# DmitryUlyanov/deep-image-prior

Hardware: NVIDIA H100
Metric: optimisation iterations/sec (512x512 skip-net denoising, sum over independent images) (higher is better)
Workload: dtype fp32 storage; tf32 tensor-core multiplies with fp32 accumulate in the convs (cuDNN's default fp32 mode)

## Files before the change

### deep-image-prior_b200/csrc/conv_tc.cu

```cuda
#include "conv_tc.cuh"
#include "ptx.cuh"
#include "wgmma.cuh"
#include "kernels.cuh"

namespace dip {

static constexpr int kTileM = 128;
static constexpr int kABytes = kTileM * 128;
static constexpr int kChunkBytes = kTileM * 128;
static constexpr int kNumThreads = 256;
static constexpr int kAccStride = kAccS;

struct SmemCtl {
  uint64_t full[8];
  uint64_t empty[8];
  float bias[160];
};

__host__ __device__ constexpr int round32(int n) { return (n + 31) & ~31; }
__host__ __device__ constexpr int round1024(int n) { return (n + 1023) & ~1023; }

template <int NT>
__device__ __forceinline__ void tc_conv_epilogue(const TcConvParams& p, SmemCtl* ctl, uint8_t* staging,
                                                 float (&acc)[2][NT / 2], int x0, int y0, int opx, int opy, int n_off,
                                                 double& stat_s1, double& stat_s2, bool col_halves = false);
__device__ __forceinline__ void tc_conv_stats_flush(const TcConvParams& p, int n_off, double stat_s1, double stat_s2);

template <bool BF16, int NT>
__device__ __forceinline__ void tc_conv_consumer(const TcConvParams& p, SmemCtl* ctl,
                                                 uint8_t* stage_base, int stage_bytes, uint8_t* staging, int n_iters,
                                                 int tile0, int tile_stride, int num_tiles, int tiles_pp, int n_off) {
  const int lane = threadIdx.x & 31;
  float acc[2][NT / 2];
  int stage = 0;
  uint32_t phase = 0;
  double stat_s1 = 0.0, stat_s2 = 0.0;
  const uint32_t base_lo = desc_lo(smem_u32(stage_base));
  const uint32_t stage_step = static_cast<uint32_t>(stage_bytes) >> 4;
  constexpr uint32_t kBOff = static_cast<uint32_t>(kABytes) >> 4;
  constexpr uint32_t kHalfOff = (64u * 128u) >> 4;
  for (int it = 0; it < n_iters; ++it) {
    const int tile = tile0 + it * tile_stride;
    int tx = tile % p.tiles_x, ty = tile / p.tiles_x;
    int opx = 0, opy = 0;
    int kb_per_tile = p.kh * p.kw * p.kblocks;
    if (p.nphase > 0) {
      if (tile >= num_tiles) break;
      const int t = tile % tiles_pp;
      tx = t % p.tiles_x; ty = t / p.tiles_x;
      const TcConvParams::Phase& q = p.phs[tile / tiles_pp];
      opx = q.opx; opy = q.opy;
      kb_per_tile = q.kh * q.kw * p.kblocks;
    }
    const int x0 = tx * p.bw, y0 = ty * p.bh;
#pragma unroll
    for (int i = 0; i < NT / 2; ++i) { acc[0][i] = 0.f; acc[1][i] = 0.f; }
    int prev = -1;
    for (int kbt = 0; kbt < kb_per_tile; ++kbt) {
      mbar_wait(&ctl->full[stage], phase);
      const uint32_t a_lo = base_lo + stage * stage_step;
      const uint32_t b_lo = a_lo + kBOff;
      wgmma_fence();
#pragma unroll
      for (int k = 0; k < 4; ++k) {
        wgmma_ss<NT, BF16>(acc[0], desc_of(a_lo + 2 * k), desc_of(b_lo + 2 * k));
        wgmma_ss<NT, BF16>(acc[1], desc_of(a_lo + kHalfOff + 2 * k), desc_of(b_lo + 2 * k));
      }
      wgmma_commit();
      if (prev >= 0) {
        wgmma_wait<1>();
        if (lane == 0) mbar_arrive(&ctl->empty[prev]);
      }
      prev = stage;
      if (++stage == p.stages) { stage = 0; phase ^= 1; }
    }
    wgmma_wait<0>();
    if (prev >= 0 && lane == 0) mbar_arrive(&ctl->empty[prev]);
    tc_conv_epilogue<NT>(p, ctl, staging, acc, x0, y0, opx, opy, n_off, stat_s1, stat_s2);
  }
  tc_conv_stats_flush(p, n_off, stat_s1, stat_s2);
}

template <int NT>
__device__ __forceinline__ void tc_conv_epilogue(const TcConvParams& p, SmemCtl* ctl, uint8_t* staging,
                                                 float (&acc)[2][NT / 2], int x0, int y0, int opx, int opy, int n_off,
                                                 double& stat_s1, double& stat_s2, bool col_halves) {
  const int et = threadIdx.x - 128;
  const int w = et >> 5, lane = et & 31;
  const int bw_shift = 31 - __clz(p.bw);
  {
    if (et == 0) tma_store_wait_read0();
    named_bar_sync(1, 128);
#pragma unroll
    for (int h = 0; h < 2; ++h) {
#pragma unroll
      for (int j = 0; j < NT / 8; ++j) {
        const int col = 8 * j + 2 * (lane & 3);
        const int chunk = col >> 5;
        if (chunk < p.n_chunks) {
          const int q = (col & 31) >> 2, e = col & 3;
#pragma unroll
          for (int rr = 0; rr < 2; ++rr) {
            const int r64 = 16 * w + (lane >> 2) + 8 * rr;
            const int row = col_halves ? ((r64 >> 3) << 4) + 8 * h + (r64 & 7) : 64 * h + r64;
            float2 o;
            o.x = acc[h][4 * j + 2 * rr] + ctl->bias[col];
            o.y = acc[h][4 * j + 2 * rr + 1] + ctl->bias[col + 1];
            *reinterpret_cast<float2*>(staging + chunk * kChunkBytes + row * 128 + ((q ^ (row & 7)) << 4) + e * 4) = o;
          }
        }
      }
    }
    fence_proxy_async_smem();
    named_bar_sync(1, 128);
    if (et == 0) {
      if (p.nphase > 0)
        for (int j = 0; j < p.n_chunks; ++j) tma_store_5d(&p.tmD, staging + j * kChunkBytes, n_off + j * 32, opx, x0, opy, y0);
      else
        for (int j = 0; j < p.n_chunks; ++j) tma_store_3d(&p.tmD, staging + j * kChunkBytes, n_off + j * 32, x0, y0);
      tma_store_commit();
    }
    if (p.stats != nullptr && et < p.n_mma) {
      const int c = et;
      const int j = c >> 5, q = (c & 31) >> 2, e = c & 3;
      const uint8_t* cb = staging + j * kChunkBytes + e * 4;
      float a0 = 0.f, a1 = 0.f, b0 = 0.f, b1 = 0.f;
      if (x0 + p.bw <= p.out_w && y0 + p.bh <= p.out_h) {
#pragma unroll 8
        for (int m = 0; m < kTileM; m += 2) {
          const float x = *reinterpret_cast<const float*>(cb + m * 128 + ((q ^ (m & 7)) << 4));
          const float y = *reinterpret_cast<const float*>(cb + (m + 1) * 128 + ((q ^ ((m + 1) & 7)) << 4));
          a0 += x; b0 = fmaf(x, x, b0);
          a1 += y; b1 = fmaf(y, y, b1);
        }
      } else {
        for (int m = 0; m < kTileM; ++m) {
          const int py = m >> bw_shift, px = m & (p.bw - 1);
          if (x0 + px < p.out_w && y0 + py < p.out_h) {
            const float x = *reinterpret_cast<const float*>(cb + m * 128 + ((q ^ (m & 7)) << 4));
            a0 += x; b0 = fmaf(x, x, b0);
          }
        }
      }
      stat_s1 += static_cast<double>(a0 + a1);
      stat_s2 += static_cast<double>(b0 + b1);
    }
  }
}

__device__ __forceinline__ void tc_conv_stats_flush(const TcConvParams& p, int n_off, double stat_s1, double stat_s2) {
  const int et = threadIdx.x - 128;
  if (p.stats != nullptr && et < p.n_mma && n_off + et < p.stats_ld) {
    const int rep = (blockIdx.x % kAccR) * kAccLine;
    atomicAdd(&p.stats[(n_off + et) * kAccStride + rep], stat_s1);
    atomicAdd(&p.stats[(p.stats_ld + n_off + et) * kAccStride + rep], stat_s2);
  }
  if (et == 0) tma_store_wait_all0();
}

template <bool BF16>
__device__ __forceinline__ void tc_conv_body(const TcConvParams& p, uint8_t* smem_raw) {
  constexpr int KE = BF16 ? 64 : 32;
  uint8_t* smem = reinterpret_cast<uint8_t*>((reinterpret_cast<uintptr_t>(smem_raw) + 1023) & ~uintptr_t(1023));
  const int nt = round32(p.n_mma);
  const int b_bytes = p.n_mma * 128;
  const int stage_bytes = kABytes + round1024(nt * 128);
  uint8_t* stage_base = smem;
  uint8_t* staging = stage_base + p.stages * stage_bytes;
  SmemCtl* ctl = reinterpret_cast<SmemCtl*>(staging + p.n_chunks * kChunkBytes);

  const int warp = threadIdx.x >> 5;
  const int lane = threadIdx.x & 31;
  const int tiles_pp = p.tiles_x * p.tiles_y;
  const int num_tiles = p.nphase > 0 ? tiles_pp * p.nphase : tiles_pp;
  const int n_split = p.n_split < 1 ? 1 : p.n_split;
  const int n_part = blockIdx.x % n_split;
  const int n_off = n_part * p.n_mma;
  const int n_total = p.n_mma * n_split;
  const int tile_stride = static_cast<int>(gridDim.x) / n_split;
  const int n_iters = (num_tiles + tile_stride - 1) / tile_stride;
  const int tile0 = blockIdx.x / n_split;

  pdl_trigger();
  if (warp == 0 && lane == 0) {
    tma_prefetch_desc(&p.tmA);
    tma_prefetch_desc(&p.tmB);
    tma_prefetch_desc(&p.tmD);
  }
  if (warp == 1 && lane == 0) {
    for (int i = 0; i < p.stages; ++i) {
      mbar_init(&ctl->full[i], 1);
      mbar_init(&ctl->empty[i], 4);
    }
    fence_mbar_init();
  }
  pdl_wait();
  if (warp == 3) {
    for (int i = lane; i < 160; i += 32)
      ctl->bias[i] = (p.bias != nullptr && i < p.n_mma && (p.n_valid == 0 || n_off + i < p.n_valid)) ? p.bias[n_off + i] : 0.f;
  }
  __syncthreads();

  if (warp == 0) {
    int stage = 0;
    uint32_t phase = 0;
    for (int it = 0; it < n_iters; ++it) {
      const int tile = tile0 + it * tile_stride;
      int kh = p.kh, kw = p.kw, offx = p.offx, offy = p.offy, tap0 = 0;
      int x0 = (tile % p.tiles_x) * p.bw, y0 = (tile / p.tiles_x) * p.bh;
      if (p.nphase > 0) {
        if (tile >= num_tiles) break;
        const TcConvParams::Phase& q = p.phs[tile / tiles_pp];
        const int t = tile % tiles_pp;
        kh = q.kh; kw = q.kw; offx = q.offx; offy = q.offy; tap0 = q.tap0;
        x0 = (t % p.tiles_x) * p.bw; y0 = (t / p.tiles_x) * p.bh;
      }
      for (int r = 0; r < kh; ++r) {
        for (int s = 0; s < kw; ++s) {
          const int ix = offx + s, iy = offy + r;
          int cpx, cx, cpy, cy;
          if (p.stride == 1) {
            cpx = 0; cx = x0 + ix; cpy = 0; cy = y0 + iy;
          } else {
            cpx = ix & 1; cx = x0 + (ix >> 1); cpy = iy & 1; cy = y0 + (iy >> 1);
          }
          const int tap = tap0 + r * kw + s;
          for (int kb = 0; kb < p.kblocks; ++kb) {
            mbar_wait(&ctl->empty[stage], phase ^ 1);
            uint8_t* sa = stage_base + stage * stage_bytes;
            if (elect_one()) {
              mbar_expect_tx(&ctl->full[stage], kABytes + b_bytes);
              tma_load_5d(sa, &p.tmA, &ctl->full[stage], kb * KE, cpx, cx, cpy, cy);
              tma_load_2d(sa + kABytes, &p.tmB, &ctl->full[stage], kb * KE, tap * n_total + n_off);
            }
            __syncwarp();
            if (++stage == p.stages) { stage = 0; phase ^= 1; }
          }
        }
      }
    }
  } else if (warp >= 4) {
    switch (nt) {
      case 32: tc_conv_consumer<BF16, 32>(p, ctl, stage_base, stage_bytes, staging, n_iters, tile0, tile_stride, num_tiles, tiles_pp, n_off); break;
      case 64: tc_conv_consumer<BF16, 64>(p, ctl, stage_base, stage_bytes, staging, n_iters, tile0, tile_stride, num_tiles, tiles_pp, n_off); break;
      case 96: tc_conv_consumer<BF16, 96>(p, ctl, stage_base, stage_bytes, staging, n_iters, tile0, tile_stride, num_tiles, tiles_pp, n_off); break;
      case 128: tc_conv_consumer<BF16, 128>(p, ctl, stage_base, stage_bytes, staging, n_iters, tile0, tile_stride, num_tiles, tiles_pp, n_off); break;
      default: tc_conv_consumer<BF16, 160>(p, ctl, stage_base, stage_bytes, staging, n_iters, tile0, tile_stride, num_tiles, tiles_pp, n_off); break;
    }
  }
  __syncthreads();
}
__global__ void __launch_bounds__(kNumThreads, 1) tc_conv_kernel(const __grid_constant__ TcConvParams p) {
  extern __shared__ __align__(1024) uint8_t smem_raw[];
  tc_conv_body<false>(p, smem_raw);
}
__global__ void __launch_bounds__(kNumThreads, 1) tc_conv_kernel_bf16(const __grid_constant__ TcConvParams p) {
  extern __shared__ __align__(1024) uint8_t smem_raw[];
  tc_conv_body<true>(p, smem_raw);
}

__host__ __device__ constexpr int patch_nt(int n_mma) { return n_mma == 144 ? 144 : round32(n_mma); }
struct PatchCtl {
  uint64_t pfull[kPatchMaxKb];
  uint64_t pempty[kPatchMaxKb];
};

struct PatchWork {
  int tile0, tile_stride, n_iters, n_off, n_total;
};
__device__ __forceinline__ PatchWork patch_work(const TcConvParams& p) {
  const int n_split = p.n_split < 1 ? 1 : p.n_split;
  PatchWork w;
  const int num_tiles = p.tiles_x * p.tiles_y;
  w.tile_stride = static_cast<int>(gridDim.x) / n_split;
  w.tile0 = blockIdx.x / n_split;
  w.n_iters = (num_tiles - w.tile0 + w.tile_stride - 1) / w.tile_stride;
  w.n_off = static_cast<int>(blockIdx.x % n_split) * p.n_mma;
  w.n_total = p.n_mma * n_split;
  return w;
}
static constexpr int kPatchTaps = 9;

template <bool BF16, int NT>
__device__ __forceinline__ void tc_conv_patch_consumer(const TcConvParams& p, SmemCtl* ctl, PatchCtl* pc,
                                                       uint8_t* patch_base, uint8_t* b_base, int b_stage_bytes,
                                                       uint8_t* staging, const PatchWork& wk) {
  const int lane = threadIdx.x & 31;
  float acc[2][NT / 2];
  int stage = 0;
  uint32_t phase = 0, pphase = 0;
  double stat_s1 = 0.0, stat_s2 = 0.0;
  const uint32_t patch16 = smem_u32(patch_base) >> 4;
  const uint32_t b_lo0 = desc_lo(smem_u32(b_base));
  const uint32_t b_step = static_cast<uint32_t>(b_stage_bytes) >> 4;
  constexpr uint32_t kPlane16 = kPatchPlane >> 4, kSlot16 = kPatchBytes >> 4;
  const uint32_t row16 = p.bw + 2;
  const uint32_t half16 = p.bw == 8 ? 8 * row16 : 8;
  for (int it = 0; it < wk.n_iters; ++it) {
    const int tile = wk.tile0 + it * wk.tile_stride;
    const int x0 = (tile % p.tiles_x) * p.bw, y0 = (tile / p.tiles_x) * p.bh;
#pragma unroll
    for (int i = 0; i < NT / 2; ++i) { acc[0][i] = 0.f; acc[1][i] = 0.f; }
    int prev = -1;
    int prev_patch = -1;
#pragma unroll 1
    for (int tap = 0; tap < kPatchTaps; ++tap) {
      const int r = tap / 3, s = tap - 3 * (tap / 3);
#pragma unroll 1
      for (int kb = 0; kb < p.kblocks; ++kb) {
        if (tap == 0) mbar_wait(&pc->pfull[kb], pphase);
        mbar_wait(&ctl->full[stage], phase);
        const uint32_t b_lo = b_lo0 + stage * b_step;
        const uint32_t a16 = patch16 + kb * kSlot16 + r * row16 + s;
        wgmma_fence();
#pragma unroll
        for (int k = 0; k < 4; ++k) {
          wgmma_ss<NT, BF16>(acc[0], desc_noswz(a16 + 2 * k * kPlane16, kPlane16, row16), desc_of(b_lo + 2 * k));
          wgmma_ss<NT, BF16>(acc[1], desc_noswz(a16 + half16 + 2 * k * kPlane16, kPlane16, row16), desc_of(b_lo + 2 * k));
        }
        wgmma_commit();
        if (prev >= 0) {
          wgmma_wait<1>();
          if (lane == 0) {
            mbar_arrive(&ctl->empty[prev]);
            if (prev_patch >= 0) mbar_arrive(&pc->pempty[prev_patch]);
          }
        }
        prev = stage;
        prev_patch = tap == kPatchTaps - 1 ? kb : -1;
        if (++stage == p.stages) { stage = 0; phase ^= 1; }
      }
    }
    pphase ^= 1;
    wgmma_wait<0>();
    if (prev >= 0 && lane == 0) {
      mbar_arrive(&ctl->empty[prev]);
      if (prev_patch >= 0) mbar_arrive(&pc->pempty[prev_patch]);
    }
    tc_conv_epilogue<NT>(p, ctl, staging, acc, x0, y0, 0, 0, wk.n_off, stat_s1, stat_s2, p.bw == 16);
  }
  tc_conv_stats_flush(p, wk.n_off, stat_s1, stat_s2);
}

template <bool BF16>
__device__ __forceinline__ void tc_conv_patch_body(const TcConvParams& p, uint8_t* smem_raw) {
  constexpr int KE = BF16 ? 64 : 32;
  constexpr int KG = BF16 ? 8 : 4;
  uint8_t* smem = reinterpret_cast<uint8_t*>((reinterpret_cast<uintptr_t>(smem_raw) + 1023) & ~uintptr_t(1023));
  const int nt = patch_nt(p.n_mma);
  const int b_bytes = p.n_mma * 128;
  const int b_stage_bytes = round1024(nt * 128);
  uint8_t* b_base = smem;
  uint8_t* staging = b_base + p.stages * b_stage_bytes;
  uint8_t* patch_base = staging + p.n_chunks * kChunkBytes;
  SmemCtl* ctl = reinterpret_cast<SmemCtl*>(patch_base + p.kblocks * kPatchBytes);
  PatchCtl* pc = reinterpret_cast<PatchCtl*>(ctl + 1);

  const int warp = threadIdx.x >> 5;
  const int lane = threadIdx.x & 31;
  const PatchWork wk = patch_work(p);

  pdl_trigger();
  if (warp == 0 && lane == 0) {
    tma_prefetch_desc(&p.tmA);
    tma_prefetch_desc(&p.tmB);
    tma_prefetch_desc(&p.tmD);
  }
  if (warp == 1 && lane == 0) {
    for (int i = 0; i < p.stages; ++i) {
      mbar_init(&ctl->full[i], 1);
      mbar_init(&ctl->empty[i], 4);
    }
    for (int i = 0; i < p.kblocks; ++i) {
      mbar_init(&pc->pfull[i], 1);
      mbar_init(&pc->pempty[i], 4);
    }
    fence_mbar_init();
  }
  pdl_wait();
  if (warp == 3) {
    for (int i = lane; i < 160; i += 32)
      ctl->bias[i] = (p.bias != nullptr && i < p.n_mma && (p.n_valid == 0 || wk.n_off + i < p.n_valid)) ? p.bias[wk.n_off + i] : 0.f;
  }
  __syncthreads();

  if (warp == 0) {
    int stage = 0;
    uint32_t phase = 0, pphase = 0;
    for (int it = 0; it < wk.n_iters; ++it) {
      const int tile = wk.tile0 + it * wk.tile_stride;
      const int x0 = (tile % p.tiles_x) * p.bw, y0 = (tile / p.tiles_x) * p.bh;
      for (int tap = 0; tap < kPatchTaps; ++tap) {
        for (int kb = 0; kb < p.kblocks; ++kb) {
          if (tap == 0) {
            mbar_wait(&pc->pempty[kb], pphase ^ 1);
            if (elect_one()) {
              mbar_expect_tx(&pc->pfull[kb], kPatchBytes);
              tma_load_4d(patch_base + kb * kPatchBytes, &p.tmA, &pc->pfull[kb], 0, x0 + p.offx, y0 + p.offy, kb * (KE / KG));
            }
            __syncwarp();
          }
          mbar_wait(&ctl->empty[stage], phase ^ 1);
          if (elect_one()) {
            mbar_expect_tx(&ctl->full[stage], b_bytes);
            tma_load_2d(b_base + stage * b_stage_bytes, &p.tmB, &ctl->full[stage], kb * KE, tap * wk.n_total + wk.n_off);
          }
          __syncwarp();
          if (++stage == p.stages) { stage = 0; phase ^= 1; }
        }
      }
      pphase ^= 1;
    }
  } else if (warp >= 4) {
    switch (nt) {
      case 32: tc_conv_patch_consumer<BF16, 32>(p, ctl, pc, patch_base, b_base, b_stage_bytes, staging, wk); break;
      case 64: tc_conv_patch_consumer<BF16, 64>(p, ctl, pc, patch_base, b_base, b_stage_bytes, staging, wk); break;
      case 96: tc_conv_patch_consumer<BF16, 96>(p, ctl, pc, patch_base, b_base, b_stage_bytes, staging, wk); break;
      case 128: tc_conv_patch_consumer<BF16, 128>(p, ctl, pc, patch_base, b_base, b_stage_bytes, staging, wk); break;
      case 144: tc_conv_patch_consumer<BF16, 144>(p, ctl, pc, patch_base, b_base, b_stage_bytes, staging, wk); break;
      default: tc_conv_patch_consumer<BF16, 160>(p, ctl, pc, patch_base, b_base, b_stage_bytes, staging, wk); break;
    }
  }
  __syncthreads();
}
__global__ void __launch_bounds__(kNumThreads, 1) tc_conv_patch_kernel(const __grid_constant__ TcConvParams p) {
  extern __shared__ __align__(1024) uint8_t smem_raw[];
  tc_conv_patch_body<false>(p, smem_raw);
}
__global__ void __launch_bounds__(kNumThreads, 1) tc_conv_patch_kernel_bf16(const __grid_constant__ TcConvParams p) {
  extern __shared__ __align__(1024) uint8_t smem_raw[];
  tc_conv_patch_body<true>(p, smem_raw);
}

struct SmemCtlW {
  uint64_t full[8];
  uint64_t empty[8];
  uint64_t bt_full[2];
  uint64_t bt_empty[2];
};

__host__ __device__ constexpr int wgrad_tbuf_bytes(bool bf16, int n_cols) {
  return (bf16 ? kTileM * 128 : 0) + round1024(n_cols * 128);
}


template <int NT>
__device__ __forceinline__ void tc_wgrad_transposer(const TcWgradParams& p, SmemCtlW* ctl, uint32_t stage_base, int stage_bytes,
                                                    uint32_t bt_base, int items) {
  constexpr int kBt = wgrad_tbuf_bytes(false, NT);
  constexpr int kUnitsO = ((NT + 31) / 32) * 8;
  constexpr int kIters = (kUnitsO + 11) / 12;
  constexpr int y_bytes = 4 * kWgradKp * 128;
  const int tt = threadIdx.x - 32;
  const int lane = threadIdx.x & 31;
  const int b = tt & 7, b0 = b & 1, b1 = (b >> 1) & 1, b2 = b >> 2;
  uint32_t src[kIters], dst[kIters], sq[kIters], dq[kIters];
  bool ok[kIters];
#pragma unroll
  for (int it = 0; it < kIters; ++it) {
    const int o = (tt >> 3) + 12 * it;
    const int kk = (b1 ^ (o & 1)) | ((b2 ^ ((o >> 1) & 1)) << 1);
    const int c4 = (o >> 3) * 8 + b2 * 4 + b1 * 2 + ((o >> 2) & 1);
    ok[it] = o < kUnitsO && c4 < NT / 4;
    src[it] = y_bytes + (c4 >> 3) * (kWgradKp * 128) + (8 * kk + b0) * 128;
    sq[it] = (c4 & 7) ^ b0;
    dst[it] = c4 * 4 * 128;
    dq[it] = (2 * kk + b0) ^ ((c4 & 1) << 2);
  }
  int stage = 0, tb = 0;
  uint32_t phase = 0, tphase = 0;
  for (int item = blockIdx.x; item < items; item += gridDim.x) {
    const int ks = item % p.ksplits;
    const int blk0 = static_cast<int>((static_cast<long long>(p.px_blocks) * ks) / p.ksplits);
    const int blk1 = static_cast<int>((static_cast<long long>(p.px_blocks) * (ks + 1)) / p.ksplits);
    for (int blk = blk0; blk < blk1; ++blk) {
      mbar_wait(&ctl->full[stage], phase);
      mbar_wait(&ctl->bt_empty[tb], tphase ^ 1);
      const uint32_t sx = stage_base + stage * stage_bytes;
      const uint32_t bt = bt_base + tb * kBt;
#pragma unroll
      for (int it = 0; it < kIters; ++it) {
        if (ok[it]) {
          uint4 v[4];
#pragma unroll
          for (int i = 0; i < 4; ++i) v[i] = lds128(sx + src[it] + 256 * i + ((sq[it] ^ (2 * i)) << 4));
          sts128(bt + dst[it] + ((dq[it] ^ 0) << 4), v[0].x, v[1].x, v[2].x, v[3].x);
          sts128(bt + dst[it] + 128 + ((dq[it] ^ 1) << 4), v[0].y, v[1].y, v[2].y, v[3].y);
          sts128(bt + dst[it] + 256 + ((dq[it] ^ 2) << 4), v[0].z, v[1].z, v[2].z, v[3].z);
          sts128(bt + dst[it] + 384 + ((dq[it] ^ 3) << 4), v[0].w, v[1].w, v[2].w, v[3].w);
        }
      }
      fence_proxy_async_smem();
      mbar_arrive(&ctl->bt_full[tb]);
      __syncwarp();
      if (lane == 0) mbar_arrive(&ctl->empty[stage]);
      if (++stage == p.stages) { stage = 0; phase ^= 1; }
      tb ^= 1;
      if (tb == 0) tphase ^= 1;
    }
  }
}

template <int NT>
__device__ __forceinline__ void tc_wgrad_mma(const TcWgradParams& p, SmemCtlW* ctl, uint32_t stage_base, int stage_bytes,
                                             uint32_t bt_base, int items) {
  constexpr int kBt = wgrad_tbuf_bytes(false, NT);
  constexpr bool kDouble = NT <= 136;
  const int et = threadIdx.x - 128;
  const int w = et >> 5, lane = et & 31, g = lane >> 2, t = lane & 3;
  const int taps = p.kh * p.kw;
  uint32_t aoff[4];
#pragma unroll
  for (int r = 0; r < 4; ++r) {
    const int hi = r & 1, e = r >> 1;
    const int q = 4 * (w & 1) + (g >> 2) + 2 * hi, px = 2 * t + e;
    aoff[r] = (w >> 1) * (kWgradKp * 128) + px * 128 + ((q ^ px) << 4) + (g & 3) * 4;
  }
  auto load_a = [&](uint32_t (&f)[8][4], uint32_t sy) {
#pragma unroll
    for (int h = 0; h < 2; ++h)
#pragma unroll
      for (int kk = 0; kk < 4; ++kk)
#pragma unroll
        for (int r = 0; r < 4; ++r) f[4 * h + kk][r] = lds32(sy + aoff[r] + h * 2 * (kWgradKp * 128) + kk * 1024);
  };
  int stage = 0, tb = 0;
  uint32_t phase = 0, tphase = 0;
  bool pending = false;
  float acc[2][NT / 2];
  uint32_t fa[8][4], fb[8][4];
  auto step = [&](uint32_t (&cur)[8][4], uint32_t (&nxt)[8][4], bool more) {
    mbar_wait(&ctl->bt_full[tb], tphase);
    const uint32_t b_lo = desc_lo(bt_base + tb * kBt);
    wgmma_fence();
#pragma unroll
    for (int kk = 0; kk < 4; ++kk) {
      wgmma_rs<NT>(acc[0], cur[kk], desc_of(b_lo + 2 * kk));
      wgmma_rs<NT>(acc[1], cur[4 + kk], desc_of(b_lo + 2 * kk));
    }
    wgmma_commit();
    __syncwarp();
    if (lane == 0) mbar_arrive(&ctl->empty[stage]);
    if (++stage == p.stages) { stage = 0; phase ^= 1; }
    if constexpr (kDouble) wgmma_wait<1>(); else wgmma_wait<0>();
    if (pending && lane == 0) mbar_arrive(&ctl->bt_empty[tb ^ 1]);
    pending = true;
    tb ^= 1;
    if (tb == 0) tphase ^= 1;
    if (more) {
      mbar_wait(&ctl->full[stage], phase);
      load_a(nxt, stage_base + stage * stage_bytes);
    }
  };
  for (int item = blockIdx.x; item < items; item += gridDim.x) {
    const int tap = item / p.ksplits, ks = item % p.ksplits;
    const int blk0 = static_cast<int>((static_cast<long long>(p.px_blocks) * ks) / p.ksplits);
    const int blk1 = static_cast<int>((static_cast<long long>(p.px_blocks) * (ks + 1)) / p.ksplits);
#pragma unroll
    for (int i = 0; i < NT / 2; ++i) { acc[0][i] = 0.f; acc[1][i] = 0.f; }
    if (blk0 < blk1) {
      mbar_wait(&ctl->full[stage], phase);
      load_a(fa, stage_base + stage * stage_bytes);
    }
    for (int blk = blk0; blk < blk1; blk += 2) {
      step(fa, kDouble ? fb : fa, blk + 1 < blk1);
      if (blk + 1 == blk1) break;
      step(kDouble ? fb : fa, fa, blk + 2 < blk1);
    }
    wgmma_wait<0>();
    if (pending && lane == 0) mbar_arrive(&ctl->bt_empty[tb ^ 1]);
    pending = false;
    float* dst = p.partial + (static_cast<size_t>(ks) * taps + tap) * 128 * NT;
#pragma unroll
    for (int h = 0; h < 2; ++h) {
#pragma unroll
      for (int j = 0; j < NT / 8; ++j) {
        const int col = 8 * j + 2 * t;
#pragma unroll
        for (int rr = 0; rr < 2; ++rr) {
          const int n = 64 * h + 16 * w + g + 8 * rr;
          *reinterpret_cast<float2*>(dst + static_cast<size_t>(n) * NT + col) =
              make_float2(acc[h][4 * j + 2 * rr], acc[h][4 * j + 2 * rr + 1]);
        }
      }
    }
  }
}

template <int NT>
__device__ __forceinline__ void tc_wgrad_consumer_bf16(const TcWgradParams& p, SmemCtlW* ctl, uint8_t* smem, int stage_bytes,
                                                       uint8_t* tbase, int items) {
  constexpr int KE = 64;
  constexpr int E = 2;
  constexpr int kTA = kTileM * 128;
  constexpr int kTBuf = wgrad_tbuf_bytes(true, NT);
  constexpr int kRows = 128 + NT;
  const int et = threadIdx.x - 128;
  const int w = et >> 5, lane = et & 31;
  constexpr int chunk_bytes = kWgradKp * 128;
  constexpr int y_bytes = (128 / KE) * chunk_bytes;
  constexpr int groups = kWgradKp * E / 16;
  constexpr int nk = kWgradKp / 16;
  const int taps = p.kh * p.kw;
  int stage = 0, tb = 0;
  uint32_t phase = 0;
  float acc[2][NT / 2];
  for (int item = blockIdx.x; item < items; item += gridDim.x) {
    const int tap = item / p.ksplits, ks = item % p.ksplits;
    const int blk0 = static_cast<int>((static_cast<long long>(p.px_blocks) * ks) / p.ksplits);
    const int blk1 = static_cast<int>((static_cast<long long>(p.px_blocks) * (ks + 1)) / p.ksplits);
#pragma unroll
    for (int i = 0; i < NT / 2; ++i) { acc[0][i] = 0.f; acc[1][i] = 0.f; }
    for (int blk = blk0; blk < blk1; ++blk) {
      mbar_wait(&ctl->full[stage], phase);
      named_bar_sync(1, 128);
      const uint8_t* sy = smem + stage * stage_bytes;
      const uint8_t* sx = sy + y_bytes;
      uint8_t* ta = tbase + tb * kTBuf;
      uint8_t* tbb = ta + kTA;
      for (int i = et; i < kRows * groups; i += 128) {
        const int g = i / kRows, row = i % kRows;
        const bool is_y = row < 128;
        const int rs = is_y ? row : row - 128;
        const uint8_t* src = (is_y ? sy : sx) + (rs / KE) * chunk_bytes;
        const int cb = (rs % KE) * E;
        uint32_t v[4];
#pragma unroll
        for (int u = 0; u < 4; ++u) {
          const int px = g * 8 + 2 * u;
          const uint32_t lo = *reinterpret_cast<const uint16_t*>(src + px * 128 + ((((cb >> 4) ^ (px & 7)) << 4) | (cb & 15)));
          const uint32_t hi = *reinterpret_cast<const uint16_t*>(src + (px + 1) * 128 + ((((cb >> 4) ^ ((px + 1) & 7)) << 4) | (cb & 15)));
          v[u] = lo | (hi << 16);
        }
        uint8_t* dst = (is_y ? ta : tbb) + rs * 128 + ((g ^ (rs & 7)) << 4);
        *reinterpret_cast<uint4*>(dst) = make_uint4(v[0], v[1], v[2], v[3]);
      }
      fence_proxy_async_smem();
      named_bar_sync(1, 128);
      if (lane == 0) mbar_arrive(&ctl->empty[stage]);
      const uint32_t a_lo = desc_lo(smem_u32(ta)), b_lo = desc_lo(smem_u32(tbb));
      wgmma_fence();
#pragma unroll
      for (int k = 0; k < nk; ++k) {
        wgmma_ss<NT, true>(acc[0], desc_of(a_lo + 2 * k), desc_of(b_lo + 2 * k));
        wgmma_ss<NT, true>(acc[1], desc_of(a_lo + ((64u * 128u) >> 4) + 2 * k), desc_of(b_lo + 2 * k));
      }
      wgmma_commit();
      wgmma_wait<1>();
      tb ^= 1;
      if (++stage == p.stages) { stage = 0; phase ^= 1; }
    }
    wgmma_wait<0>();
    float* dst = p.partial + (static_cast<size_t>(ks) * taps + tap) * 128 * NT;
#pragma unroll
    for (int h = 0; h < 2; ++h) {
#pragma unroll
      for (int j = 0; j < NT / 8; ++j) {
        const int col = 8 * j + 2 * (lane & 3);
#pragma unroll
        for (int rr = 0; rr < 2; ++rr) {
          const int n = 64 * h + 16 * w + (lane >> 2) + 8 * rr;
          *reinterpret_cast<float2*>(dst + static_cast<size_t>(n) * NT + col) =
              make_float2(acc[h][4 * j + 2 * rr], acc[h][4 * j + 2 * rr + 1]);
        }
      }
    }
  }
}

template <bool BF16, int NT>
__device__ __forceinline__ void tc_wgrad_role(const TcWgradParams& p, SmemCtlW* ctl, uint8_t* smem, int stage_bytes,
                                              uint8_t* tbase, int items, int warp) {
  if constexpr (BF16) {
    if (warp >= 4) tc_wgrad_consumer_bf16<NT>(p, ctl, smem, stage_bytes, tbase, items);
  } else {
    if (warp >= 4) tc_wgrad_mma<NT>(p, ctl, smem_u32(smem), stage_bytes, smem_u32(tbase), items);
    else tc_wgrad_transposer<NT>(p, ctl, smem_u32(smem), stage_bytes, smem_u32(tbase), items);
  }
}

template <bool BF16>
__device__ __forceinline__ void tc_wgrad_body(const TcWgradParams& p, uint8_t* smem_raw) {
  uint8_t* smem = reinterpret_cast<uint8_t*>((reinterpret_cast<uintptr_t>(smem_raw) + 1023) & ~uintptr_t(1023));
  constexpr int KE = BF16 ? 64 : 32;
  constexpr int YCH = 128 / KE;
  constexpr int chunk_bytes = kWgradKp * 128;
  const int y_bytes = YCH * chunk_bytes;
  const int x_bytes = p.c_chunks * chunk_bytes;
  const int stage_bytes = y_bytes + x_bytes;
  uint8_t* tbase = smem + p.stages * stage_bytes;
  SmemCtlW* ctl = reinterpret_cast<SmemCtlW*>(tbase + 2 * wgrad_tbuf_bytes(BF16, p.n_cols));
  const int items = p.kh * p.kw * p.ksplits;

  const int warp = threadIdx.x >> 5;
  const int lane = threadIdx.x & 31;
  pdl_trigger();
  if (warp == 0 && lane == 0) {
    tma_prefetch_desc(&p.tmY);
    tma_prefetch_desc(&p.tmX);
  }
  if (warp == 1 && lane == 0) {
    for (int i = 0; i < p.stages; ++i) {
      mbar_init(&ctl->full[i], 1);
      mbar_init(&ctl->empty[i], BF16 ? 4 : 7);
    }
    for (int i = 0; i < 2; ++i) {
      mbar_init(&ctl->bt_full[i], 96);
      mbar_init(&ctl->bt_empty[i], 4);
    }
    fence_mbar_init();
  }
  pdl_wait();
  __syncthreads();

  if (warp == 0) {
    int stage = 0;
    uint32_t phase = 0;
    for (int item = blockIdx.x; item < items; item += gridDim.x) {
      const int tap = item / p.ksplits, ks = item % p.ksplits;
      const int r = tap / p.kw, s = tap % p.kw;
      const int blk0 = static_cast<int>((static_cast<long long>(p.px_blocks) * ks) / p.ksplits);
      const int blk1 = static_cast<int>((static_cast<long long>(p.px_blocks) * (ks + 1)) / p.ksplits);
      const int ix = p.offx + s, iy = p.offy + r;
      for (int blk = blk0; blk < blk1; ++blk) {
        const int y = blk / p.px_blocks_x;
        const int x0 = (blk % p.px_blocks_x) * kWgradKp;
        int cpx, cx, cpy, cy;
        if (p.stride == 1) {
          cpx = 0; cx = x0 + ix; cpy = 0; cy = y + iy;
        } else {
          cpx = ix & 1; cx = x0 + (ix >> 1); cpy = iy & 1; cy = y + (iy >> 1);
        }
        mbar_wait(&ctl->empty[stage], phase ^ 1);
        uint8_t* sy = smem + stage * stage_bytes;
        if (elect_one()) {
          mbar_expect_tx(&ctl->full[stage], stage_bytes);
          for (int j = 0; j < YCH; ++j) tma_load_3d(sy + j * chunk_bytes, &p.tmY, &ctl->full[stage], j * KE, x0, y);
          for (int j = 0; j < p.c_chunks; ++j)
            tma_load_5d(sy + y_bytes + j * chunk_bytes, &p.tmX, &ctl->full[stage], j * KE, cpx, cx, cpy, cy);
        }
        __syncwarp();
        if (++stage == p.stages) { stage = 0; phase ^= 1; }
      }
    }
  } else {
    switch (p.n_cols) {
      case 32: tc_wgrad_role<BF16, 32>(p, ctl, smem, stage_bytes, tbase, items, warp); break;
      case 64: tc_wgrad_role<BF16, 64>(p, ctl, smem, stage_bytes, tbase, items, warp); break;
      case 96: tc_wgrad_role<BF16, 96>(p, ctl, smem, stage_bytes, tbase, items, warp); break;
      case 128: tc_wgrad_role<BF16, 128>(p, ctl, smem, stage_bytes, tbase, items, warp); break;
      case 136: tc_wgrad_role<BF16, 136>(p, ctl, smem, stage_bytes, tbase, items, warp); break;
      default: tc_wgrad_role<BF16, 160>(p, ctl, smem, stage_bytes, tbase, items, warp); break;
    }
  }
  __syncthreads();
}
__global__ void __launch_bounds__(kNumThreads, 1) tc_wgrad_kernel(const __grid_constant__ TcWgradParams p) {
  extern __shared__ __align__(1024) uint8_t smem_raw[];
  tc_wgrad_body<false>(p, smem_raw);
}
__global__ void __launch_bounds__(kNumThreads, 1) tc_wgrad_kernel_bf16(const __grid_constant__ TcWgradParams p) {
  extern __shared__ __align__(1024) uint8_t smem_raw[];
  tc_wgrad_body<true>(p, smem_raw);
}

static constexpr size_t kMaxSmem = 232448;

size_t tc_conv_smem_bytes(const TcConvParams& p) {
  const size_t b_bytes = round1024((p.patch ? patch_nt(p.n_mma) : round32(p.n_mma)) * 128);
  if (p.patch)
    return 1024 + p.stages * b_bytes + static_cast<size_t>(p.n_chunks) * kChunkBytes +
           static_cast<size_t>(p.kblocks) * kPatchBytes + sizeof(SmemCtl) + sizeof(PatchCtl);
  return 1024 + p.stages * (kABytes + b_bytes) + static_cast<size_t>(p.n_chunks) * kChunkBytes + sizeof(SmemCtl);
}
size_t tc_wgrad_smem_bytes(const TcWgradParams& p) {
  const size_t chunk = static_cast<size_t>(kWgradKp) * 128;
  const size_t tbuf = wgrad_tbuf_bytes(p.bf16 != 0, p.n_cols);
  return 1024 + p.stages * ((p.bf16 ? 2 : 4) * chunk + static_cast<size_t>(p.c_chunks) * chunk) + 2 * tbuf + sizeof(SmemCtlW);
}

cudaError_t tc_kernels_init() {
  cudaError_t e = cudaFuncSetAttribute(tc_conv_kernel, cudaFuncAttributeMaxDynamicSharedMemorySize, (int)kMaxSmem);
  if (e != cudaSuccess) return e;
  e = cudaFuncSetAttribute(tc_conv_kernel_bf16, cudaFuncAttributeMaxDynamicSharedMemorySize, (int)kMaxSmem);
  if (e != cudaSuccess) return e;
  e = cudaFuncSetAttribute(tc_conv_patch_kernel, cudaFuncAttributeMaxDynamicSharedMemorySize, (int)kMaxSmem);
  if (e != cudaSuccess) return e;
  e = cudaFuncSetAttribute(tc_conv_patch_kernel_bf16, cudaFuncAttributeMaxDynamicSharedMemorySize, (int)kMaxSmem);
  if (e != cudaSuccess) return e;
  e = cudaFuncSetAttribute(tc_wgrad_kernel_bf16, cudaFuncAttributeMaxDynamicSharedMemorySize, (int)kMaxSmem);
  if (e != cudaSuccess) return e;
  return cudaFuncSetAttribute(tc_wgrad_kernel, cudaFuncAttributeMaxDynamicSharedMemorySize, (int)kMaxSmem);
}

static bool conv_params_ok(const TcConvParams& p) {
  return p.n_mma >= 1 && p.n_mma <= 160 && p.n_chunks == (p.n_mma + 31) / 32 && p.stages >= 1 && p.stages <= 8 &&
         p.kblocks >= 1 && p.nphase >= 0 && p.nphase <= 4 &&
         (p.bw & (p.bw - 1)) == 0 && p.bw * p.bh == kTileM &&
         (!p.patch || (((p.bw == 8 && p.bh == 16) || (p.bw == 16 && p.bh == 8)) && p.kblocks <= kPatchMaxKb && p.kh == 3 && p.kw == 3 && p.stride == 1 && p.nphase == 0));
}

cudaError_t tc_conv_launch(const TcConvParams& p, int num_sms, cudaStream_t s) {
  if (!conv_params_ok(p)) return cudaErrorInvalidValue;
  const int tiles = p.tiles_x * p.tiles_y * (p.nphase > 0 ? p.nphase : 1);
  int grid = tiles < num_sms ? tiles : num_sms;
  if (p.n_split > 1) {
    if (tiles * p.n_split > num_sms) return cudaErrorInvalidValue;
    grid = tiles * p.n_split;
  }
  const size_t smem = tc_conv_smem_bytes(p);
  if (smem > kMaxSmem) return cudaErrorInvalidValue;
  if (p.patch)
    return launch_k(p.bf16 ? tc_conv_patch_kernel_bf16 : tc_conv_patch_kernel, dim3(grid), dim3(kNumThreads), smem, s, 1, p);
  return launch_k(p.bf16 ? tc_conv_kernel_bf16 : tc_conv_kernel, dim3(grid), dim3(kNumThreads), smem, s, 1, p);
}

cudaError_t tc_wgrad_launch(const TcWgradParams& p, cudaStream_t s) {
  const size_t smem = tc_wgrad_smem_bytes(p);
  const bool cols_ok = p.n_cols == 32 || p.n_cols == 64 || p.n_cols == 96 || p.n_cols == 128 || p.n_cols == 136 ||
                       p.n_cols == 160;
  if (smem > kMaxSmem || !cols_ok || p.n_cols > p.c_chunks * (p.bf16 ? 64 : 32) || p.stages < 1 || p.stages > 8)
    return cudaErrorInvalidValue;
  return launch_k(p.bf16 ? tc_wgrad_kernel_bf16 : tc_wgrad_kernel, dim3(p.kh * p.kw * p.ksplits), dim3(kNumThreads), smem, s, 1, p);
}

}
```

### deep-image-prior_b200/csrc/conv_tc.cuh

```cuda
#pragma once
#include <cuda.h>
#include <cuda_runtime.h>
#include <stdint.h>

namespace dip {

struct TcConvParams {
  CUtensorMap tmA;
  CUtensorMap tmB;
  CUtensorMap tmD;
  int tiles_x, tiles_y;
  int bw, bh;
  int out_w, out_h;
  int kh, kw;
  int stride;
  int offx, offy;
  int bf16;
  int kblocks;
  int n_mma;
  int n_chunks;
  int stages;
  int n_split;
  int nphase;
  struct Phase { int kh, kw, offx, offy, tap0, opx, opy; } phs[4];
  int n_valid;
  const float* bias;
  double* stats;
  int stats_ld;
  int patch;
};
static constexpr int kPatchPlane = 180 * 16;
static constexpr int kPatchMaxKb = 8;
static constexpr int kPatchBytes = 8 * kPatchPlane;

static constexpr int kWgradKp = 32;
struct TcWgradParams {
  CUtensorMap tmY;
  CUtensorMap tmX;
  float* partial;
  int kh, kw, stride, offx, offy;
  int px_blocks_x;
  int px_blocks;
  int bf16;
  int c_chunks;
  int n_cols;
  int ksplits;
  int stages;
};

size_t tc_conv_smem_bytes(const TcConvParams& p);
size_t tc_wgrad_smem_bytes(const TcWgradParams& p);
cudaError_t tc_conv_launch(const TcConvParams& p, int num_sms, cudaStream_t s);
cudaError_t tc_wgrad_launch(const TcWgradParams& p, cudaStream_t s);
cudaError_t tc_kernels_init();

}
```

### deep-image-prior_b200/csrc/engine.cu

```cuda
#include <cuda.h>
#include <cuda_bf16.h>
#include <cuda_runtime.h>
#include <math.h>
#include <stdio.h>
#include <stdlib.h>
#include <string.h>

#include <initializer_list>
#include <map>
#include <string>
#include <vector>

#include "../../include/dip.h"
#include "conv_tc.cuh"
#include "kernels.cuh"

namespace dip {

static thread_local std::string g_err;
static int fail(const std::string& m) {
  g_err = m;
  return -1;
}
#define DIP_CUDA(expr)                                                                                   \
  do {                                                                                                   \
    cudaError_t _e = (expr);                                                                             \
    if (_e != cudaSuccess) return fail(std::string(#expr) + ": " + cudaGetErrorString(_e));              \
  } while (0)
#define DIP_CHECK(expr)        \
  do {                         \
    int _r = (expr);           \
    if (_r != 0) return _r;    \
  } while (0)

typedef CUresult (*PFN_encodeTiled)(CUtensorMap*, CUtensorMapDataType, cuuint32_t, void*, const cuuint64_t*,
                                    const cuuint64_t*, const cuuint32_t*, const cuuint32_t*, CUtensorMapInterleave,
                                    CUtensorMapSwizzle, CUtensorMapL2promotion, CUtensorMapFloatOOBfill);
static PFN_encodeTiled g_encode = nullptr;
static int g_num_sms = 0;
static unsigned long long g_inited_mask = 0;

static int engine_init() {
  int dev = 0;
  DIP_CUDA(cudaGetDevice(&dev));
  if (dev >= 64) return fail("dip: device ordinal >= 64 not supported");
  if (g_inited_mask & (1ull << dev)) return 0;
  cudaDeviceProp prop;
  DIP_CUDA(cudaGetDeviceProperties(&prop, dev));
  if (prop.major != 9 || prop.minor != 0)
    return fail("dip requires an sm_90 (H100) device; found sm_" + std::to_string(prop.major * 10 + prop.minor));
  g_num_sms = prop.multiProcessorCount;
  void* fn = nullptr;
  cudaDriverEntryPointQueryResult q;
  DIP_CUDA(cudaGetDriverEntryPoint("cuTensorMapEncodeTiled", &fn, cudaEnableDefault, &q));
  if (fn == nullptr || q != cudaDriverEntryPointSuccess) return fail("cuTensorMapEncodeTiled not available from the driver");
  g_encode = reinterpret_cast<PFN_encodeTiled>(fn);
  DIP_CUDA(tc_kernels_init());
  DIP_CUDA(down_kernels_init());
  g_inited_mask |= 1ull << dev;
  return 0;
}

static bool is_tc(int prec) { return prec == DIP_PRECISION_TF32 || prec == DIP_PRECISION_BF16; }

static int encode_map(CUtensorMap* m, const void* base, int rank, const cuuint64_t* dims, const cuuint64_t* strides_b,
                      const cuuint32_t* box, bool bf16 = false, bool swizzle = true) {
  cuuint32_t estr[5] = {1, 1, 1, 1, 1};
  CUresult r = g_encode(m, bf16 ? CU_TENSOR_MAP_DATA_TYPE_BFLOAT16 : CU_TENSOR_MAP_DATA_TYPE_FLOAT32, rank, const_cast<void*>(base), dims, strides_b, box, estr,
                        CU_TENSOR_MAP_INTERLEAVE_NONE, swizzle ? CU_TENSOR_MAP_SWIZZLE_128B : CU_TENSOR_MAP_SWIZZLE_NONE,
                        CU_TENSOR_MAP_L2_PROMOTION_L2_128B,
                        CU_TENSOR_MAP_FLOAT_OOB_FILL_NONE);
  if (r != CUDA_SUCCESS) {
    char buf[256];
    snprintf(buf, sizeof buf, "cuTensorMapEncodeTiled failed (%d): rank %d dims %llu %llu %llu box %u %u %u", (int)r, rank,
             (unsigned long long)dims[0], (unsigned long long)dims[1], (unsigned long long)(rank > 2 ? dims[2] : 0), box[0],
             box[1], rank > 2 ? box[2] : 0);
    return fail(buf);
  }
  return 0;
}
static int map_act5(CUtensorMap* m, const void* base, int rows, int cols, int ld, int c, int stride, int bw, int bh,
                    bool bf16 = false) {
  const cuuint64_t e = bf16 ? 2 : sizeof(float);
  cuuint64_t dims[5], str[4];
  if (stride == 1) {
    dims[0] = c; dims[1] = 1; dims[2] = cols; dims[3] = 1; dims[4] = rows;
    str[0] = ld * e; str[1] = ld * e; str[2] = (cuuint64_t)cols * ld * e; str[3] = (cuuint64_t)cols * ld * e;
  } else {
    dims[0] = c; dims[1] = 2; dims[2] = cols / 2; dims[3] = 2; dims[4] = rows / 2;
    str[0] = ld * e; str[1] = 2 * ld * e; str[2] = (cuuint64_t)cols * ld * e; str[3] = 2 * (cuuint64_t)cols * ld * e;
  }
  cuuint32_t box[5] = {bf16 ? 64u : 32u, 1, (cuuint32_t)bw, 1, (cuuint32_t)bh};
  return encode_map(m, base, 5, dims, str, box, bf16);
}
static int map_act3(CUtensorMap* m, const void* base, int rows, int cols, int ld, int c, int bw, int bh, bool bf16 = false) {
  const cuuint64_t e = bf16 ? 2 : sizeof(float);
  cuuint64_t dims[3] = {(cuuint64_t)c, (cuuint64_t)cols, (cuuint64_t)rows};
  cuuint64_t str[2] = {ld * e, (cuuint64_t)cols * ld * e};
  cuuint32_t box[3] = {bf16 ? 64u : 32u, (cuuint32_t)bw, (cuuint32_t)bh};
  return encode_map(m, base, 3, dims, str, box, bf16);
}
static int map_patch(CUtensorMap* m, const void* base, int rows, int cols, int ld, int c, int bw, int bh, bool bf16) {
  const cuuint64_t e = bf16 ? 2 : sizeof(float);
  const cuuint64_t g = 16 / e;
  cuuint64_t dims[4] = {g, (cuuint64_t)cols, (cuuint64_t)rows, (cuuint64_t)c / g};
  cuuint64_t str[3] = {ld * e, (cuuint64_t)cols * ld * e, 16};
  cuuint32_t box[4] = {(cuuint32_t)g, (cuuint32_t)bw + 2, (cuuint32_t)bh + 2, 8};
  return encode_map(m, base, 4, dims, str, box, bf16, false);
}
static int map_w2(CUtensorMap* m, const void* base, int rows_total, int kcols, int box_rows, bool bf16 = false) {
  const cuuint64_t e = bf16 ? 2 : sizeof(float);
  cuuint64_t dims[2] = {(cuuint64_t)kcols, (cuuint64_t)rows_total};
  cuuint64_t str[1] = {kcols * e};
  cuuint32_t box[2] = {bf16 ? 64u : 32u, (cuuint32_t)box_rows};
  return encode_map(m, base, 2, dims, str, box, bf16);
}

static void pick_tile(int w, int h, int* bw, int* bh) {
  const int cand[5][2] = {{128, 1}, {64, 2}, {32, 4}, {16, 8}, {8, 16}};
  long long best = -1;
  for (int i = 0; i < 5; ++i) {
    const long long cw = (w + cand[i][0] - 1) / cand[i][0] * cand[i][0];
    const long long ch = (h + cand[i][1] - 1) / cand[i][1] * cand[i][1];
    const long long cost = cw * ch * 64 + (cand[i][0] + cand[i][1]);
    if (best < 0 || cost < best) { best = cost; *bw = cand[i][0]; *bh = cand[i][1]; }
  }
}
static int round_up(int x, int m) { return (x + m - 1) / m * m; }
struct Timer {
  bool on = false;
  std::vector<cudaEvent_t> pool;
  size_t used = 0;
  struct Rec { int cls; double flops; size_t e0, e1; };
  std::vector<Rec> recs;
  size_t get(cudaStream_t s) {
    if (used == pool.size()) { cudaEvent_t e; cudaEventCreate(&e); pool.push_back(e); }
    cudaEventRecord(pool[used], s);
    return used++;
  }
  void reset() { used = 0; recs.clear(); }
};
struct Recorder {
  Timer* timer = nullptr;
  int n = 0;
};
enum HbmId { H_INPUT_PAD = 0, H_NOISE, H_SKINNY_FWD, H_BN_ACT_WRITE, H_BN_ACT_HEAD, H_CAT_STATS, H_CAT_WRITE, H_BN_BWD_REDUCE,
             H_BN_BWD_APPLY, H_CAT_BWD_REDUCE, H_CAT_BWD_APPLY, H_UPADJ, H_SKINNY_BWD, H_MSE, H_ADAM, H_HEAD_DLOGIT, H_DOWN_FWD,
             H_DOWN_BWD, H_PACK, H_WGRAD_REDUCE, H_TRACK_OUT, H_TRACK_DECIDE, H_ADAM_TRACK };
static constexpr int kUntimed = -1;
static int hbm(HbmId id, int sub) { return 16 + 8 * (int)id + sub; }
struct EnqScope {
  Timer* t; int cls; double flops; size_t e0 = 0; cudaStream_t s;
  EnqScope(Recorder* r, int cls_, double flops_, cudaStream_t s_)
      : t(r != nullptr && cls_ != kUntimed && r->timer->on ? r->timer : nullptr), cls(cls_), flops(flops_), s(s_) {
    if (r != nullptr) r->n++;
    if (t) e0 = t->get(s);
  }
  ~EnqScope() { if (t) { size_t e1 = t->get(s); t->recs.push_back({cls, flops, e0, e1}); } }
};
#define ENQ(rec, cls, flops, s, stmt)                                 \
  do {                                                                \
    EnqScope _es((rec), (cls), (double)(flops), (s));                 \
    stmt;                                                             \
  } while (0)

struct PackEntry {
  const float* w; float* dst_f; float* dst_d;
  int N, C, k, rot, n_rows, c_pad, c_rows;
  int Ctot, coff;
  int s2;
  int bf16;
  int c_pad16;
  int n_pad;
};
__constant__ int kS2Taps[9] = {2 * 3 + 2, 2 * 3 + 0, 0 * 3 + 2, 0 * 3 + 0,
                               2 * 3 + 1, 0 * 3 + 1,
                               1 * 3 + 2, 1 * 3 + 0,
                               1 * 3 + 1};
__global__ void k_pack_table(const PackEntry* __restrict__ tab) {
  pdl_enter();
  const PackEntry e = tab[blockIdx.y];
  const int taps = e.k * e.k;
  const int c_pad = e.bf16 ? e.c_pad16 : e.c_pad;
  __nv_bfloat16* const f16 = reinterpret_cast<__nv_bfloat16*>(e.dst_f);
  __nv_bfloat16* const d16 = reinterpret_cast<__nv_bfloat16*>(e.dst_d);
  const long long nf = e.dst_f != nullptr ? (long long)taps * e.n_rows * c_pad : 0;
  const long long nd = e.dst_d != nullptr ? (long long)taps * e.c_rows * e.n_pad : 0;
  for (long long i = (long long)blockIdx.x * blockDim.x + threadIdx.x; i < nf + nd; i += (long long)gridDim.x * blockDim.x) {
    if (i < nf) {
      const int c = (int)(i % c_pad), n = (int)((i / c_pad) % e.n_rows), tap = (int)(i / ((long long)c_pad * e.n_rows));
      float v = 0.f;
      if (n < e.N && c < e.C) v = e.w[((long long)n * e.Ctot + (c + e.coff + e.rot) % e.Ctot) * taps + tap];
      if (e.bf16) f16[i] = __float2bfloat16_rn(v); else e.dst_f[i] = v;
    } else {
      const long long j = i - nf;
      const int n = (int)(j % e.n_pad), c = (int)((j / e.n_pad) % e.c_rows), tapf = (int)(j / ((long long)e.n_pad * e.c_rows));
      const int tap = e.s2 ? kS2Taps[tapf] : taps - 1 - tapf;
      float v = 0.f;
      if (n < e.N && c < e.C) v = e.w[((long long)n * e.Ctot + (c + e.coff + e.rot) % e.Ctot) * taps + tap];
      if (e.bf16) d16[j] = __float2bfloat16_rn(v); else e.dst_d[j] = v;
    }
  }
}
struct UnpackEntry {
  const float* acc; float* dw;
  int N, C, taps, rot, cols, Ctot, coff, ks;
};
__global__ void k_wgrad_unpack_table(const UnpackEntry* __restrict__ tab) {
  pdl_enter();
  const UnpackEntry e = tab[blockIdx.y];
  const int total = e.N * e.C * e.taps;
  for (int i = blockIdx.x * blockDim.x + threadIdx.x; i < total; i += gridDim.x * blockDim.x) {
    const int tap = i % e.taps, c = (i / e.taps) % e.C, n = i / (e.taps * e.C);
    const size_t split = (size_t)e.taps * 128 * e.cols;
    const float* src = e.acc + ((size_t)tap * 128 + n) * e.cols + c;
    float v = 0.f;
    for (int k = 0; k < e.ks; ++k) v += src[k * split];
    e.dw[((size_t)n * e.Ctot + (c + e.coff + e.rot) % e.Ctot) * e.taps + tap] = v;
  }
}
static int pick_nsplit(int tiles, int n_rows) {
  int sp = 1;
  while (sp * 2 <= 4 && tiles * sp * 2 <= g_num_sms && n_rows % (32 * sp * 2) == 0) sp *= 2;
  return sp;
}
static void fit_stages(TcConvParams& p) {
  p.stages = p.patch ? 8 : 6;
  while (tc_conv_smem_bytes(p) > 232448 && p.stages > 2) p.stages--;
}
struct ConvOp {
  Recorder* rec = nullptr;
  double alg_flops() const { return 2.0 * out_h * out_w * (double)N * C * k * k; }
  int N = 128, C = 0, k = 1, stride = 1, rot = 0;
  int Np = 128;
  int n_pad = 128;
  int n_pad16 = 128;
  int Ctot = 0, coff = 0;
  bool do_fprop = true, do_wgrad = true;
  int dg_ld = 0;
  int c_pad = 0;
  int crows = 0;
  bool bf16 = false;
  int c_pad16 = 0;
  const uint16_t* in16 = nullptr; int in_ld16 = 0;
  const uint16_t* dy16 = nullptr;
  const float* in = nullptr; int in_rows = 0, in_cols = 0, in_ld = 0; int offx = 0, offy = 0;
  float* out = nullptr; int out_h = 0, out_w = 0;
  double* stats = nullptr;
  float* wp_f = nullptr; float* wp_d = nullptr;
  const float* dy = nullptr;
  bool has_dgrad = false;
  bool dg_s2 = false;
  float* dg_out = nullptr; int dg_out_h = 0, dg_out_w = 0; int dg_off = 0;
  float* partial = nullptr;
  const UnpackEntry* unpack = nullptr;
  int p_w = -1, p_b = -1;
  TcConvParams fp{}, dg{};
  TcWgradParams wg{};

  void set_shapes() {
    c_pad = round_up(C, 32);
    c_pad16 = round_up(C, 64);
    crows = round_up(C, 16);
    Np = round_up(N, 16); n_pad = round_up(N, 32); n_pad16 = round_up(N, 64);
    if (Ctot == 0) Ctot = C;
    if (dg_ld == 0) dg_ld = C;
  }
  size_t wp_f_elems() const { return (size_t)k * k * Np * c_pad; }
  size_t wp_d_elems() const { return (size_t)k * k * crows * n_pad; }
  int wg_cols() const { return C > 128 && C <= 136 ? 136 : c_pad; }
  int tc_ksplits() const {
    const int blocks = out_h * ((out_w + kWgradKp - 1) / kWgradKp);
    int ks = static_cast<int>(kNumSms) / (k * k);
    if (ks > blocks) ks = blocks;
    return ks < 1 ? 1 : ks;
  }
  int simt_ksplits() const { return out_h < 64 ? out_h : 64; }
  int part_ks(int prec) const { return is_tc(prec) ? tc_ksplits() : simt_ksplits(); }
  int part_cols(int prec) const { return is_tc(prec) ? wg_cols() : c_pad; }
  size_t partial_elems(int prec) const { return (size_t)part_ks(prec) * k * k * 128 * part_cols(prec); }
  PackEntry pack_entry(int prec, const float* w) const {
    PackEntry e{};
    e.w = w; e.dst_f = do_fprop ? wp_f : nullptr; e.dst_d = has_dgrad ? wp_d : nullptr;
    e.N = N; e.C = C; e.k = k; e.rot = rot; e.n_rows = Np; e.c_pad = c_pad; e.c_rows = crows;
    e.Ctot = Ctot; e.coff = coff; e.s2 = dg_s2 && is_tc(prec) ? 1 : 0;
    e.bf16 = bf16 ? 1 : 0; e.c_pad16 = c_pad16; e.n_pad = bf16 ? n_pad16 : n_pad;
    return e;
  }
  UnpackEntry unpack_entry(int prec, float* dw) const {
    return UnpackEntry{partial, dw, N, C, k * k, rot, part_cols(prec), Ctot, coff, part_ks(prec)};
  }

  int patch_form(TcConvParams& g, const void* act, int rows, int cols, int ld, int kc) {
    if ((g.bw != 8 && g.bw != 16) || kc % (bf16 ? 8 : 4) != 0 || g.kblocks > kPatchMaxKb) return 0;
    TcConvParams t = g;
    t.patch = 1;
    fit_stages(t);
    if (tc_conv_smem_bytes(t) > 232448) return 0;
    DIP_CHECK(map_patch(&t.tmA, act, rows, cols, ld, kc, g.bw, g.bh, bf16));
    g = t;
    return 0;
  }
  int build_tc() {
    int bw, bh;
    fp = TcConvParams{};
    if (do_fprop) {
      pick_tile(out_w, out_h, &bw, &bh);
      DIP_CHECK(bf16 ? map_act5(&fp.tmA, in16, in_rows, in_cols, in_ld16, C, stride, bw, bh, true)
                     : map_act5(&fp.tmA, in, in_rows, in_cols, in_ld, C, stride, bw, bh));
      fp.n_split = pick_nsplit(((out_w + bw - 1) / bw) * ((out_h + bh - 1) / bh), Np);
      DIP_CHECK(map_w2(&fp.tmB, wp_f, k * k * Np, bf16 ? c_pad16 : c_pad, Np / fp.n_split, bf16));
      DIP_CHECK(map_act3(&fp.tmD, out, out_h, out_w, N, N, bw, bh));
      fp.tiles_x = (out_w + bw - 1) / bw; fp.tiles_y = (out_h + bh - 1) / bh;
      fp.bw = bw; fp.bh = bh; fp.out_w = out_w; fp.out_h = out_h;
      fp.kh = fp.kw = k; fp.stride = stride; fp.offx = offx; fp.offy = offy;
      fp.bf16 = bf16 ? 1 : 0;
      fp.kblocks = bf16 ? c_pad16 / 64 : c_pad / 32;
      fp.n_mma = Np / fp.n_split; fp.n_chunks = (fp.n_mma + 31) / 32;
      fp.n_valid = N;
      fp.bias = nullptr; fp.stats = stats; fp.stats_ld = N;
      fit_stages(fp);
      if (k == 3 && stride == 1)
        DIP_CHECK(bf16 ? patch_form(fp, in16, in_rows, in_cols, in_ld16, C) : patch_form(fp, in, in_rows, in_cols, in_ld, C));
    }
    dg = TcConvParams{};
    if (has_dgrad) {
      const int gh = dg_s2 ? dg_out_h / 2 : dg_out_h, gw = dg_s2 ? dg_out_w / 2 : dg_out_w;
      pick_tile(gw, gh, &bw, &bh);
      DIP_CHECK(bf16 ? map_act5(&dg.tmA, dy16, out_h, out_w, N, N, 1, bw, bh, true)
                     : map_act5(&dg.tmA, dy, out_h, out_w, N, N, 1, bw, bh));
      dg.tiles_x = (gw + bw - 1) / bw; dg.tiles_y = (gh + bh - 1) / bh;
      dg.n_split = pick_nsplit((dg_s2 ? 4 : 1) * dg.tiles_x * dg.tiles_y, crows);
      DIP_CHECK(map_w2(&dg.tmB, wp_d, k * k * crows, bf16 ? n_pad16 : n_pad, crows / dg.n_split, bf16));
      DIP_CHECK(dg_s2 ? map_act5(&dg.tmD, dg_out, dg_out_h, dg_out_w, dg_ld, C, 2, bw, bh)
                      : map_act3(&dg.tmD, dg_out, dg_out_h, dg_out_w, dg_ld, C, bw, bh));
      dg.bw = bw; dg.bh = bh; dg.out_w = gw; dg.out_h = gh;
      dg.stride = 1;
      if (dg_s2) {
        dg.kh = dg.kw = 2; dg.offx = dg.offy = -1;
        dg.nphase = 4;
        int t0 = 0;
        for (int a = 0; a < 2; ++a)
          for (int b = 0; b < 2; ++b) {
            TcConvParams::Phase& q = dg.phs[a * 2 + b];
            q.kh = 2 - a; q.kw = 2 - b; q.offy = a == 0 ? -1 : 0; q.offx = b == 0 ? -1 : 0; q.tap0 = t0; q.opx = b; q.opy = a;
            t0 += q.kh * q.kw;
          }
      } else {
        dg.kh = dg.kw = k; dg.offx = dg.offy = dg_off;
      }
      dg.bf16 = bf16 ? 1 : 0;
      dg.kblocks = bf16 ? n_pad16 / 64 : n_pad / 32;
      dg.n_mma = crows / dg.n_split; dg.n_chunks = (dg.n_mma + 31) / 32;
      fit_stages(dg);
      if (!dg_s2 && k == 3)
        DIP_CHECK(bf16 ? patch_form(dg, dy16, out_h, out_w, N, N) : patch_form(dg, dy, out_h, out_w, N, N));
    }
    wg = TcWgradParams{};
    if (!do_wgrad) return 0;
    wg.bf16 = bf16 ? 1 : 0;
    DIP_CHECK(bf16 ? map_act3(&wg.tmY, dy16, out_h, out_w, N, N, kWgradKp, 1, true)
                   : map_act3(&wg.tmY, dy, out_h, out_w, N, N, kWgradKp, 1));
    DIP_CHECK(bf16 ? map_act5(&wg.tmX, in16, in_rows, in_cols, in_ld16, C, stride, kWgradKp, 1, true)
                   : map_act5(&wg.tmX, in, in_rows, in_cols, in_ld, C, stride, kWgradKp, 1));
    wg.partial = partial;
    wg.kh = wg.kw = k; wg.stride = stride; wg.offx = offx; wg.offy = offy;
    wg.px_blocks_x = (out_w + kWgradKp - 1) / kWgradKp;
    wg.px_blocks = out_h * wg.px_blocks_x;
    wg.c_chunks = bf16 ? c_pad16 / 64 : c_pad / 32;
    wg.n_cols = wg_cols();
    wg.ksplits = tc_ksplits();
    wg.stages = 6;
    while (tc_wgrad_smem_bytes(wg) > 232448 && wg.stages > 1) wg.stages--;
    if (tc_wgrad_smem_bytes(wg) > 232448) return fail("wgrad stage does not fit in shared memory");
    return 0;
  }

  int run_fprop(int prec, const float* bias, cudaStream_t s) {
    if (is_tc(prec)) {
      TcConvParams p = fp;
      p.bias = bias;
      ENQ(rec, 0, alg_flops(), s, DIP_CUDA(tc_conv_launch(p, g_num_sms, s)));
    } else {
      SimtConvArgs a{};
      a.A = in; a.a_h = in_rows; a.a_w = in_cols; a.a_ld = in_ld; a.a_c = C;
      a.Wp = wp_f; a.n_rows = Np; a.c_pad = c_pad;
      a.D = out; a.d_h = out_h; a.d_w = out_w; a.d_ld = N; a.d_c = N;
      a.kh = a.kw = k; a.stride = stride; a.offx = offx; a.offy = offy; a.bias = bias;
      ENQ(rec, kUntimed, 0, s, launch_simt_conv(a, s));
      if (stats != nullptr) ENQ(rec, kUntimed, 0, s, launch_channel_stats(out, N, N, out_h * out_w, stats, s));
      DIP_CUDA(cudaGetLastError());
    }
    return 0;
  }
  int run_dgrad(int prec, cudaStream_t s) {
    if (is_tc(prec)) {
      ENQ(rec, 1, alg_flops(), s, DIP_CUDA(tc_conv_launch(dg, g_num_sms, s)));
    } else {
      SimtConvArgs a{};
      a.A = dy; a.a_h = out_h; a.a_w = out_w; a.a_ld = N; a.a_c = N; a.dil = dg_s2 ? 2 : 1;
      a.Wp = wp_d; a.n_rows = crows; a.c_pad = n_pad;
      a.D = dg_out; a.d_h = dg_out_h; a.d_w = dg_out_w; a.d_ld = dg_ld; a.d_c = C;
      a.kh = a.kw = k; a.stride = 1; a.offx = a.offy = dg_off; a.bias = nullptr;
      ENQ(rec, kUntimed, 0, s, launch_simt_conv(a, s));
      DIP_CUDA(cudaGetLastError());
    }
    return 0;
  }
  int run_wgrad(int prec, cudaStream_t s) {
    static const bool dbg_skip = getenv("DIP_DBG_SKIP_WGRAD") != nullptr;
    if (dbg_skip) return 0;
    if (is_tc(prec)) {
      ENQ(rec, 2, alg_flops(), s, DIP_CUDA(tc_wgrad_launch(wg, s)));
    } else {
      SimtWgradArgs a{};
      a.dY = dy; a.h = out_h; a.w = out_w; a.dy_ld = N; a.n = N;
      a.X = in; a.x_h = in_rows; a.x_w = in_cols; a.x_ld = in_ld; a.x_c = C;
      a.kh = a.kw = k; a.stride = stride; a.offx = offx; a.offy = offy;
      a.partial = partial; a.c_pad = c_pad; a.ksplits = simt_ksplits();
      ENQ(rec, kUntimed, 0, s, launch_simt_wgrad(a, s));
    }
    if (unpack != nullptr)
      ENQ(rec, hbm(H_WGRAD_REDUCE, 0), ((double)part_ks(prec) + 1.0) * k * k * 128.0 * part_cols(prec) * sizeof(float), s,
          launch_k(k_wgrad_unpack_table, dim3(64, 1), dim3(256), 0, s, 1, unpack));
    DIP_CUDA(cudaGetLastError());
    return 0;
  }
};

struct CvtEntry {
  const double* src; float* dst; int n, rot;
  int row, row_ld;
};
__global__ void k_cvt_table(const CvtEntry* __restrict__ tab) {
  pdl_enter();
  const CvtEntry e = tab[blockIdx.x];
  for (int i = threadIdx.x; i < e.n; i += blockDim.x) {
    const int si = e.row > 0 ? (i / e.row) * e.row_ld + i % e.row : i;
    e.dst[(i + e.rot) % e.n] = (float)acc_get(e.src + (size_t)si * kAccS);
  }
}
struct RunEntry {
  const double* fwd; float* rm; float* rv; void* nb; int C, rot; float n; int nb_is_float;
};
__global__ void k_running_table(const RunEntry* __restrict__ tab) {
  pdl_enter();
  const RunEntry e = tab[blockIdx.x];
  if (e.rm == nullptr) return;
  for (int c = threadIdx.x; c < e.C; c += blockDim.x) {
    const int ct = (c + e.rot) % e.C;
    const double m = acc_get(e.fwd + c * kAccS) / e.n;
    double var = acc_get(e.fwd + (e.C + c) * kAccS) / e.n - m * m;
    if (var < 0) var = 0;
    const double unb = e.n > 1.f ? var * e.n / (e.n - 1.0) : var;
    e.rm[ct] = 0.9f * e.rm[ct] + 0.1f * (float)m;
    e.rv[ct] = 0.9f * e.rv[ct] + 0.1f * (float)unb;
  }
  if (threadIdx.x == 0 && e.nb != nullptr) {
    if (e.nb_is_float) *reinterpret_cast<float*>(e.nb) += 1.f; else *reinterpret_cast<long long*>(e.nb) += 1;
  }
}

struct Arena {
  uint8_t* base;
  size_t off = 0;
  template <typename T>
  T* get(size_t n) {
    off = (off + 255) & ~size_t(255);
    T* p = base ? reinterpret_cast<T*>(base + off) : nullptr;
    off += n * sizeof(T);
    return p;
  }
};
struct BufInfo {
  void* ptr; int rows, cols, ld, c;
};
struct BnLayer {
  int C = 0, rot = 0; float n = 1.f;
  double* fwd = nullptr; double* bwd = nullptr; double* dbias = nullptr;
  int p_gamma = -1, p_beta = -1, p_bias = -1, idx = -1;
};
struct Level {
  int H, W, h, w, Cin;
  int Cin_act;
  int bilinear;
  int nd = 128, nu = 128, ns = 0, cu = 128;
  float *rawF = nullptr, *dRawF = nullptr;
  uint16_t* dRawF16 = nullptr;
  float *Pin, *raw_s, *raw_d1, *P_d1, *raw_d2, *P_d2, *P_cat, *raw_u, *A_u, *raw_v, *U;
  uint16_t *Pin16 = nullptr, *P_d1_16 = nullptr, *P_d2_16 = nullptr, *P_cat16 = nullptr, *A_u16 = nullptr;
  uint16_t *dRaw_v16 = nullptr, *dRaw_u16 = nullptr, *dRaw_d2_16 = nullptr, *dRaw_d1_16 = nullptr, *dRaw_s16 = nullptr;
  int Pin_ld16 = 0, cat_ld16 = 0;
  float *dUp;
  float *dS;
  float *dRaw_v, *dA_u, *dRaw_u, *dP_cat, *dCat, *dRaw_s, *dRaw_d2, *dP_d1, *dRaw_d1, *dPin;
  BnLayer bn_s, bn_d1, bn_d2, bn_cat, bn_u, bn_v;
  int p_skip_w, p_skip_b;
  double* dw_s;
  ConvOp d1, d2, up, c11;
  ConvOp sk, up_a, up_b;
};

}

using namespace dip;

struct dip_plan {
  dip_net_desc desc;
  int H, W;
  int zero_pad = 0;
  int act_fun = DIP_ACT_LEAKY_RELU;
  bool dry = false;
  uint8_t* ws = nullptr;
  size_t ws_bytes = 0;
  std::vector<Level> lv;
  std::vector<long long> numel;
  std::vector<float*> params, grads;
  std::vector<void*> running;
  std::vector<BnLayer*> bns;
  std::vector<ConvOp*> convs;
  std::map<std::string, BufInfo> bufs;
  int p_head_w = -1, p_head_b = -1;
  double* dw_head = nullptr; double* db_head = nullptr; double* db_scratch = nullptr;
  float* out_saved = nullptr;
  double* acc_fwd = nullptr; size_t acc_fwd_n = 0;
  double* acc_bwd = nullptr; size_t acc_bwd_n = 0;
  float* partial = nullptr;
  float* zbuf = nullptr; float* dout = nullptr; float* dl4 = nullptr;
  static constexpr int kDownMaxK = 64;
  float* ds_kern = nullptr;
  float* ds_y = nullptr;
  float* ds_dy = nullptr;
  int ds_K = 0, ds_f = 1, ds_pad = 0, ds_Ho = 0, ds_Wo = 0;
  static constexpr int kLossRing = 65536;
  double* loss_ring = nullptr;
  int* it_dev = nullptr;
  struct GraphKey {
    const void *z0 = nullptr, *target = nullptr, *mask = nullptr, *out = nullptr, *slots = nullptr;
    unsigned long long adam_id = 0, adam_bind = 0;
    float sigma = 0.f; uint64_t seed = 0; double lr = 0.0;
    dip_track track{};
    bool operator==(const GraphKey& o) const {
      const dip_track &a = track, &b = o.track;
      return z0 == o.z0 && target == o.target && mask == o.mask && out == o.out && slots == o.slots && adam_id == o.adam_id &&
             adam_bind == o.adam_bind && sigma == o.sigma && seed == o.seed && lr == o.lr && a.gt == b.gt &&
             a.out_avg == b.out_avg && a.snapshot == b.snapshot && a.state == b.state && a.records == b.records &&
             a.exp_weight == b.exp_weight && a.show_every == b.show_every && a.backtrack_db == b.backtrack_db;
    }
  };
  GraphKey gkey{};
  cudaGraphExec_t gexec = nullptr;
  cudaGraphExec_t gfwd = nullptr, gbwd = nullptr;
  cudaStream_t gstream = nullptr;
  cudaEvent_t gev_in = nullptr, gev_out = nullptr;
  cudaStream_t wstream = nullptr;
  cudaStream_t sstream = nullptr;
  std::vector<cudaEvent_t> wev;
  size_t wev_used = 0;
  bool side_on = false;
  std::vector<dip::ConvOp*> deferred;
  struct { bool on = false; const float* z0 = nullptr; float sigma = 0.f; uint64_t seed = 0, offset = 0; const int* it_dev = nullptr; } fnoise;
  bool prepacked = false;
  PackEntry* d_pack = nullptr; CvtEntry* d_cvt = nullptr; RunEntry* d_run = nullptr; UnpackEntry* d_unpack = nullptr;
  int n_pack = 0, n_cvt = 0, n_run = 0, n_unpack = 0;
  float* wacc_base = nullptr; size_t wacc_bytes = 0;
  long long pack_max = 0;
  bool bound = false;
  int nbt_is_float = 0;
  int launches_fwd = 0, launches_bwd = 0;
  Timer timer;
  Recorder rec{&timer};
};

namespace dip {

static BnRef bn_ref(const dip_plan* P, const BnLayer& b) {
  BnRef r;
  r.fwd = b.fwd; r.gamma = P->params[b.p_gamma]; r.beta = P->params[b.p_beta];
  r.C = b.C; r.rot = b.rot; r.inv_n = 1.f / b.n;
  return r;
}

static int build_plan(dip_plan* P, Arena& A) {
  const dip_net_desc& d = P->desc;
  const int L = d.num_scales;
  if (L < 1 || L > 8) return fail("dip-b200: 1..8 scales supported");
  std::vector<int> ND(L), NU(L), NS(L);
  for (int l = 0; l < L; ++l) {
    ND[l] = d.channels > 0 ? d.channels : d.channels_down[l];
    NU[l] = d.channels > 0 ? d.channels : d.channels_up[l];
    NS[l] = d.channels > 0 ? d.skip_channels : d.channels_skip[l];
    for (int w : {ND[l], NU[l]})
      if (w < 8 || w > 128 || w % 8 != 0)
        return fail("dip-b200: num_channels_down / num_channels_up must be multiples of 8 in [8, 128] (128 in the BASELINE configurations)");
  }
  bool wide = true, uniform = true;
  for (int l = 0; l < L; ++l) {
    wide = wide && NS[l] == 128 && ND[l] == 128 && NU[l] == 128;
    uniform = uniform && ND[l] == 128 && NU[l] == 128 && NS[l] == NS[0];
  }
  for (int l = 0; l < L; ++l)
    if (!(wide || NS[l] == 0 || NS[l] == 4))
      return fail("dip-b200: num_channels_skip must be 0 or 4 per scale, or 128 at every scale of a 128-wide network");
  const int CS = NS[0];
  if (d.downsample_mode != 0 && d.downsample_mode != 1) return fail("dip-b200: downsample_mode must be 'stride' (0) or 'avg' (1)");
  const bool avg = d.downsample_mode == 1;
  auto psl = [&](int l) { return NS[l] > 0 ? 4 : 0; };
  if (d.in_channels < 1 || d.in_channels > 128) return fail("dip-b200: input depth must be in [1,128]");
  int cin_eng = 4;
  while (cin_eng < d.in_channels) cin_eng *= 2;
  if (d.out_channels < 1 || d.out_channels > 4) return fail("dip-b200: num_output_channels must be <= 4");
  if (P->H % (1 << L) || P->W % (1 << L)) return fail("dip-b200: H and W must be divisible by 2^num_scales");
  if ((P->H >> L) < 2 || (P->W >> L) < 2)
    return fail("dip-b200: H and W must be at least 2 * 2^num_scales (ReflectionPad2d(1) in front of the deepest 3x3 conv needs 2 "
                "pixels per side: torch raises for the reference's network as well)");
  const int prec = d.precision;
  if (prec != DIP_PRECISION_TF32 && prec != DIP_PRECISION_FP32 && prec != DIP_PRECISION_BF16) return fail("dip-b200: unknown precision");
  const bool bf = prec == DIP_PRECISION_BF16;
  P->lv.resize(L);
  int pidx = 0;
  std::vector<int> pre(L), post(L);
  {
    int idx = 0;
    for (int l = 0; l < L; ++l) { pre[l] = idx; idx += 8 + psl(l); }
    for (int l = L - 1; l >= 0; --l) { post[l] = idx; idx += 10; }
    P->p_head_w = idx; P->p_head_b = idx + 1;
    pidx = idx + 2;
  }
  P->numel.assign(pidx, 0);
  P->bns.clear(); P->convs.clear();
  size_t acc_f = 0, acc_b = 0;
  auto bn_init = [&](BnLayer& b, int C, int rot, int n, int pg, int pbias) {
    b.C = C; b.rot = rot; b.n = (float)n; b.p_gamma = pg; b.p_beta = pg + 1; b.p_bias = pbias;
    P->numel[pg] = C; P->numel[pg + 1] = C;
    acc_f += 2 * C; acc_b += 3 * C;
  };
  for (int l = 0; l < L; ++l) {
    Level& v = P->lv[l];
    v.H = P->H >> l; v.W = P->W >> l; v.h = v.H / 2; v.w = v.W / 2;
    v.nd = ND[l]; v.nu = NU[l]; v.ns = NS[l]; v.cu = l == L - 1 ? ND[l] : NU[l + 1];
    const int CS = v.ns, ps = psl(l);
    v.Cin = l == 0 ? cin_eng : ND[l - 1];
    v.Cin_act = l == 0 ? d.in_channels : ND[l - 1];
    v.bilinear = d.upsample_bilinear < 0 ? (d.upsample_mask >> l) & 1 : (d.upsample_bilinear != 0);
    const int b0 = pre[l], b1 = post[l];
    if (CS > 0) {
      v.p_skip_w = b0; v.p_skip_b = b0 + 1;
      P->numel[b0] = (long long)CS * v.Cin_act; P->numel[b0 + 1] = CS;
      bn_init(v.bn_s, CS, 0, v.H * v.W, b0 + 2, b0 + 1);
    } else {
      v.p_skip_w = v.p_skip_b = -1;
      v.bn_s = BnLayer{};
    }
    v.d1.N = v.nd; v.d1.C = v.Cin_act; v.d1.k = 3; v.d1.stride = 2; v.d1.p_w = b0 + ps; v.d1.p_b = b0 + ps + 1;
    P->numel[b0 + ps] = (long long)v.nd * v.Cin_act * 9; P->numel[b0 + ps + 1] = v.nd;
    bn_init(v.bn_d1, v.nd, 0, v.h * v.w, b0 + ps + 2, b0 + ps + 1);
    v.d2.N = v.nd; v.d2.C = v.nd; v.d2.k = 3; v.d2.stride = 1; v.d2.p_w = b0 + ps + 4; v.d2.p_b = b0 + ps + 5;
    P->numel[b0 + ps + 4] = (long long)v.nd * v.nd * 9; P->numel[b0 + ps + 5] = v.nd;
    bn_init(v.bn_d2, v.nd, 0, v.h * v.w, b0 + ps + 6, b0 + ps + 5);
    bn_init(v.bn_cat, v.cu + CS, CS, v.H * v.W, b1 + 0, -1);
    v.up.N = v.nu; v.up.C = v.cu + CS; v.up.k = 3; v.up.stride = 1; v.up.rot = CS; v.up.p_w = b1 + 2; v.up.p_b = b1 + 3;
    if (wide) {
      v.up.do_wgrad = false;
      v.sk.C = v.Cin_act; v.sk.k = 1; v.sk.stride = 1; v.sk.p_w = b0; v.sk.p_b = b0 + 1;
      for (ConvOp* h : {&v.up_a, &v.up_b}) {
        h->C = 128; h->Ctot = 128 + CS; h->k = 3; h->stride = 1; h->rot = CS; h->p_w = b1 + 2; h->p_b = b1 + 3;
        h->do_fprop = false; h->dg_ld = 128 + CS;
      }
      v.up_b.coff = 128;
    }
    P->numel[b1 + 2] = (long long)v.nu * (v.cu + CS) * 9; P->numel[b1 + 3] = v.nu;
    bn_init(v.bn_u, v.nu, 0, v.H * v.W, b1 + 4, b1 + 3);
    v.c11.N = v.nu; v.c11.C = v.nu; v.c11.k = 1; v.c11.stride = 1; v.c11.p_w = b1 + 6; v.c11.p_b = b1 + 7;
    P->numel[b1 + 6] = (long long)v.nu * v.nu; P->numel[b1 + 7] = v.nu;
    bn_init(v.bn_v, v.nu, 0, v.H * v.W, b1 + 8, b1 + 7);
  }
  const int NH = NU[0];
  P->numel[P->p_head_w] = (long long)d.out_channels * NH;
  P->numel[P->p_head_b] = d.out_channels;
  {
    std::vector<BnLayer*> a, b;
    for (int l = 0; l < L; ++l) { if (NS[l] > 0) a.push_back(&P->lv[l].bn_s); a.push_back(&P->lv[l].bn_d1); a.push_back(&P->lv[l].bn_d2); }
    for (int l = L - 1; l >= 0; --l) { a.push_back(&P->lv[l].bn_cat); a.push_back(&P->lv[l].bn_u); a.push_back(&P->lv[l].bn_v); }
    P->bns = a;
    for (size_t i = 0; i < P->bns.size(); ++i) P->bns[i]->idx = (int)i;
  }
  size_t skinny_acc = 0;
  for (int l = 0; l < L; ++l) skinny_acc += (size_t)NS[l] * P->lv[l].Cin;
  skinny_acc += (size_t)d.out_channels * NH + 8;
  P->acc_fwd_n = acc_f * kAccS;
  P->acc_bwd_n = (acc_b + skinny_acc) * kAccS;
  P->acc_fwd = A.get<double>(P->acc_fwd_n);
  P->acc_bwd = A.get<double>(P->acc_bwd_n);
  {
    double* f = P->acc_fwd; double* b = P->acc_bwd;
    for (BnLayer* bn : P->bns) {
      bn->fwd = f; f = f ? f + 2 * bn->C * kAccS : nullptr;
      bn->bwd = b; bn->dbias = b ? b + 2 * bn->C * kAccS : nullptr; b = b ? b + 3 * bn->C * kAccS : nullptr;
    }
    for (int l = 0; l < L; ++l) { P->lv[l].dw_s = b; b = b ? b + (size_t)NS[l] * P->lv[l].Cin * kAccS : nullptr; }
    P->dw_head = b; b = b ? b + (size_t)d.out_channels * NH * kAccS : nullptr;
    P->db_head = b;
    P->db_scratch = b ? b + 4 * kAccS : nullptr;
  }
  auto reg = [&](const std::string& name, void* p, int rows, int cols, int ld, int c) { P->bufs[name] = BufInfo{p, rows, cols, ld, c}; };
  for (int l = 0; l < L; ++l) {
    Level& v = P->lv[l];
    const std::string pf = "L" + std::to_string(l) + ".";
    auto f32 = [&](const char* name, int rows, int cols, int ld, int c) {
      float* p = A.get<float>((size_t)rows * cols * ld);
      reg(pf + name, p, rows, cols, ld, c);
      return p;
    };
    auto b16 = [&](const char* name, int rows, int cols, int ld, int c) {
      uint16_t* p = A.get<uint16_t>((size_t)rows * cols * ld);
      reg(pf + name, p, rows, cols, ld, c);
      return p;
    };
    const bool last = l == L - 1;
    const int CS = v.ns, nd = v.nd, nu = v.nu, CC = v.cu + v.ns;
    const bool d1_dgrad = l > 0 || d.input_grad != 0;
    if (l == 0) v.Pin = f32("Pin", v.H + 2, v.W + 2, v.Cin, v.Cin);
    else reg(pf + "Pin", v.Pin = P->lv[l - 1].P_d2, v.H + 2, v.W + 2, v.Cin, v.Cin);
    v.raw_s = f32("raw_s", v.H, v.W, CS, CS);
    v.raw_d1 = f32("raw_d1", v.h, v.w, nd, nd);
    v.P_d1 = f32("P_d1", v.h + 2, v.w + 2, nd, nd);
    v.raw_d2 = f32("raw_d2", v.h, v.w, nd, nd);
    v.P_d2 = last ? f32("P_d2", v.h, v.w, nd, nd) : f32("P_d2", v.h + 2, v.w + 2, nd, nd);
    v.P_cat = f32("P_cat", v.H + 2, v.W + 2, CC, CC);
    v.raw_u = f32("raw_u", v.H, v.W, nu, nu);
    v.A_u = f32("A_u", v.H, v.W, nu, nu);
    v.raw_v = f32("raw_v", v.H, v.W, nu, nu);
    v.U = (l > 0 || nu != 128) ? f32("U", v.H, v.W, nu, nu) : nullptr;
    v.dRaw_v = f32("dRaw_v", v.H, v.W, nu, nu);
    v.dA_u = f32("dA_u", v.H, v.W, nu, nu);
    v.dRaw_u = f32("dRaw_u", v.H, v.W, nu, nu);
    v.dP_cat = f32("dP_cat", v.H + 2, v.W + 2, CC, CC);
    v.dCat = f32("dCat", v.H, v.W, CC, CC);
    v.dRaw_s = f32("dRaw_s", v.H, v.W, CS, CS);
    v.dUp = f32("dUp", v.h, v.w, v.cu, v.cu);
    v.dRaw_d2 = f32("dRaw_d2", v.h, v.w, nd, nd);
    v.dP_d1 = f32("dP_d1", v.h + 2, v.w + 2, nd, nd);
    v.dRaw_d1 = f32("dRaw_d1", v.h, v.w, nd, nd);
    if (avg) {
      v.rawF = f32("rawF", v.H, v.W, nd, nd);
      if (bf) v.dRawF16 = b16("dRawF16", v.H, v.W, nd, nd);
      else v.dRawF = f32("dRawF", v.H, v.W, nd, nd);
    }
    v.dS = (CS > 0 && (l > 0 ? wide : d.input_grad != 0)) ? f32("dS", v.H, v.W, v.Cin, v.Cin) : nullptr;
    v.dPin = d1_dgrad ? f32("dPin", v.H + 2, v.W + 2, v.Cin, v.Cin_act) : nullptr;
    if (bf) {
      v.Pin_ld16 = round_up(v.Cin, 8); v.cat_ld16 = round_up(CC, 8);
      if (l == 0) v.Pin16 = b16("Pin16", v.H + 2, v.W + 2, v.Pin_ld16, v.Cin);
      else reg(pf + "Pin16", v.Pin16 = P->lv[l - 1].P_d2_16, v.H + 2, v.W + 2, v.Pin_ld16, v.Cin);
      v.P_d1_16 = b16("P_d1_16", v.h + 2, v.w + 2, nd, nd);
      v.P_d2_16 = last ? nullptr : b16("P_d2_16", v.h + 2, v.w + 2, nd, nd);
      v.P_cat16 = b16("P_cat16", v.H + 2, v.W + 2, v.cat_ld16, CC);
      v.A_u16 = b16("A_u16", v.H, v.W, nu, nu);
      v.dRaw_v16 = b16("dRaw_v16", v.H, v.W, nu, nu);
      v.dRaw_u16 = b16("dRaw_u16", v.H, v.W, nu, nu);
      v.dRaw_d2_16 = b16("dRaw_d2_16", v.h, v.w, nd, nd);
      v.dRaw_d1_16 = avg ? nullptr : b16("dRaw_d1_16", v.h, v.w, nd, nd);
      v.dRaw_s16 = wide ? b16("dRaw_s16", v.H, v.W, 128, 128) : nullptr;
    }
  }
  P->out_saved = A.get<float>((size_t)P->H * P->W * d.out_channels);
  P->zbuf = A.get<float>((size_t)P->H * P->W * d.in_channels);
  P->dout = A.get<float>((size_t)P->H * P->W * d.out_channels);
  P->dl4 = A.get<float>((size_t)P->H * P->W * 4);
  P->ds_kern = A.get<float>(dip_plan::kDownMaxK * dip_plan::kDownMaxK);
  P->ds_y = A.get<float>((size_t)P->H * P->W * d.out_channels);
  P->ds_dy = A.get<float>((size_t)P->H * P->W * d.out_channels);
  P->loss_ring = A.get<double>(dip_plan::kLossRing);
  P->it_dev = A.get<int>(4);
  size_t partial_max = 0;
  for (int l = 0; l < L; ++l) {
    Level& v = P->lv[l];
    ConvOp& a = v.d1;
    a.set_shapes();
    a.in = v.Pin; a.in_rows = v.H + 2; a.in_cols = v.W + 2; a.in_ld = v.Cin; a.offx = a.offy = 0;
    a.out = v.raw_d1; a.out_h = v.h; a.out_w = v.w; a.stats = v.bn_d1.fwd;
    a.has_dgrad = l > 0 || d.input_grad != 0;
    a.dg_ld = v.Cin;
    a.dg_s2 = true;
    a.dy = v.dRaw_d1; a.dy16 = v.dRaw_d1_16;
    a.dg_out = v.dPin; a.dg_out_h = v.H + 2; a.dg_out_w = v.W + 2; a.dg_off = -2;
    a.in16 = v.Pin16; a.in_ld16 = v.Pin_ld16;
    if (avg) {
      a.stride = 1; a.out = v.rawF; a.out_h = v.H; a.out_w = v.W; a.stats = nullptr;
      a.dg_s2 = false; a.dy = v.dRawF; a.dy16 = v.dRawF16;
    }
    ConvOp& b = v.d2;
    b.set_shapes();
    b.in = v.P_d1; b.in_rows = v.h + 2; b.in_cols = v.w + 2; b.in_ld = v.nd; b.offx = b.offy = 0;
    b.out = v.raw_d2; b.out_h = v.h; b.out_w = v.w; b.stats = v.bn_d2.fwd;
    b.has_dgrad = true;
    b.dy = v.dRaw_d2; b.dy16 = v.dRaw_d2_16;
    b.dg_out = v.dP_d1; b.dg_out_h = v.h + 2; b.dg_out_w = v.w + 2; b.dg_off = -2;
    b.in16 = v.P_d1_16; b.in_ld16 = v.nd;
    ConvOp& c = v.up;
    c.set_shapes();
    c.in = v.P_cat; c.in_rows = v.H + 2; c.in_cols = v.W + 2; c.in_ld = v.cu + v.ns; c.offx = c.offy = 0;
    c.out = v.raw_u; c.out_h = v.H; c.out_w = v.W; c.stats = v.bn_u.fwd;
    c.has_dgrad = !wide;
    c.dy = v.dRaw_u; c.dy16 = v.dRaw_u16;
    c.dg_out = v.dP_cat; c.dg_out_h = v.H + 2; c.dg_out_w = v.W + 2; c.dg_off = -2;
    c.in16 = v.P_cat16; c.in_ld16 = v.cat_ld16;
    ConvOp& e = v.c11;
    e.set_shapes();
    e.in = v.A_u; e.in_rows = v.H; e.in_cols = v.W; e.in_ld = v.nu; e.offx = e.offy = 0;
    e.out = v.raw_v; e.out_h = v.H; e.out_w = v.W; e.stats = v.bn_v.fwd;
    e.has_dgrad = true;
    e.dy = v.dRaw_v; e.dy16 = v.dRaw_v16;
    e.dg_out = v.dA_u; e.dg_out_h = v.H; e.dg_out_w = v.W; e.dg_off = 0;
    e.in16 = v.A_u16; e.in_ld16 = v.nu;
    std::vector<ConvOp*> ops = {&a, &b, &c, &e};
    if (wide) {
      ConvOp& k1 = v.sk;
      k1.set_shapes();
      k1.in = v.Pin; k1.in_rows = v.H + 2; k1.in_cols = v.W + 2; k1.in_ld = v.Cin; k1.offx = k1.offy = 1;
      k1.out = v.raw_s; k1.out_h = v.H; k1.out_w = v.W; k1.stats = v.bn_s.fwd;
      k1.has_dgrad = l > 0 || d.input_grad != 0;
      k1.dg_ld = v.Cin;
      k1.dy = v.dRaw_s; k1.dy16 = v.dRaw_s16;
      k1.dg_out = v.dS; k1.dg_out_h = v.H; k1.dg_out_w = v.W; k1.dg_off = 0;
      k1.in16 = v.Pin16; k1.in_ld16 = v.Pin_ld16;
      ops.push_back(&k1);
      for (ConvOp* h : {&v.up_a, &v.up_b}) {
        h->set_shapes();
        h->in = v.P_cat + h->coff; h->in_rows = v.H + 2; h->in_cols = v.W + 2; h->in_ld = 128 + CS; h->offx = h->offy = 0;
        h->out = v.raw_u; h->out_h = v.H; h->out_w = v.W; h->stats = nullptr;
        h->has_dgrad = true;
        h->dy = v.dRaw_u; h->dy16 = v.dRaw_u16;
        h->dg_out = v.dP_cat + h->coff; h->dg_out_h = v.H + 2; h->dg_out_w = v.W + 2; h->dg_off = -2;
        h->in16 = v.P_cat16 != nullptr ? v.P_cat16 + h->coff : nullptr; h->in_ld16 = v.cat_ld16;
        ops.push_back(h);
      }
    }
    for (ConvOp* op : ops) {
      op->wp_f = op->do_fprop ? A.get<float>(op->wp_f_elems()) : nullptr;
      op->wp_d = op->has_dgrad ? A.get<float>(op->wp_d_elems()) : nullptr;
      op->bf16 = bf;
      op->rec = &P->rec;
      const size_t pe = op->do_wgrad ? op->partial_elems(prec) : 0;
      if (pe > partial_max) partial_max = pe;
      P->convs.push_back(op);
    }
  }
  P->partial = is_tc(prec) ? nullptr : A.get<float>(partial_max);
  P->n_unpack = 0;
  for (ConvOp* op : P->convs) if (op->do_wgrad) P->n_unpack++;
  if (is_tc(prec)) {
    size_t tot = 0;
    for (ConvOp* op : P->convs) if (op->do_wgrad) tot += (op->partial_elems(prec) + 63) & ~size_t(63);
    P->wacc_base = A.get<float>(tot);
    P->wacc_bytes = tot * sizeof(float);
    if (P->wacc_base != nullptr) reg("wacc", P->wacc_base, 1, 1, (int)tot, (int)tot);
    size_t off = 0;
    for (ConvOp* op : P->convs) if (op->do_wgrad) { op->partial = P->wacc_base ? P->wacc_base + off : nullptr; off += (op->partial_elems(prec) + 63) & ~size_t(63); }
  }
  P->d_unpack = A.get<UnpackEntry>(P->n_unpack > 0 ? P->n_unpack : 1);
  if (!is_tc(prec) && !P->dry) {
    int i = 0;
    for (ConvOp* op : P->convs) if (op->do_wgrad) { op->partial = P->partial; op->unpack = P->d_unpack + i++; }
  }
  P->n_pack = (int)P->convs.size();
  P->n_cvt = (int)P->bns.size() * 3 + L + 2;
  P->n_run = (int)P->bns.size();
  P->d_pack = A.get<PackEntry>(P->n_pack);
  P->d_cvt = A.get<CvtEntry>(P->n_cvt);
  P->d_run = A.get<RunEntry>(P->n_run);
  if (P->dry) return 0;
  {
    int lo = 0, hi = 0;
    DIP_CUDA(cudaDeviceGetStreamPriorityRange(&lo, &hi));
    if (getenv("DIP_NO_PRIO") != nullptr) lo = hi = 0;
    DIP_CUDA(cudaStreamCreateWithPriority(&P->wstream, cudaStreamNonBlocking, lo));
    DIP_CUDA(cudaStreamCreateWithPriority(&P->sstream, cudaStreamNonBlocking, lo));
  }
  if (is_tc(prec))
    for (ConvOp* op : P->convs) DIP_CHECK(op->build_tc());
  P->pack_max = 0;
  for (ConvOp* op : P->convs) {
    const long long n = (op->do_fprop ? (long long)op->wp_f_elems() : 0) + (op->has_dgrad ? (long long)op->wp_d_elems() : 0);
    if (n > P->pack_max) P->pack_max = n;
  }
  return 0;
}

static int upload_tables(dip_plan* P) {
  std::vector<PackEntry> pk;
  for (ConvOp* op : P->convs) pk.push_back(op->pack_entry(P->desc.precision, P->params[op->p_w]));
  DIP_CUDA(cudaMemcpy(P->d_pack, pk.data(), pk.size() * sizeof(PackEntry), cudaMemcpyHostToDevice));
  if (P->n_unpack > 0) {
    std::vector<UnpackEntry> up;
    for (ConvOp* op : P->convs)
      if (op->do_wgrad) up.push_back(op->unpack_entry(P->desc.precision, P->grads[op->p_w]));
    if ((int)up.size() != P->n_unpack) return fail("internal: unpack table size mismatch");
    DIP_CUDA(cudaMemcpy(P->d_unpack, up.data(), up.size() * sizeof(UnpackEntry), cudaMemcpyHostToDevice));
  }
  std::vector<CvtEntry> cv;
  for (BnLayer* b : P->bns) {
    cv.push_back(CvtEntry{b->bwd + b->C * kAccS, P->grads[b->p_gamma], b->C, b->rot});
    cv.push_back(CvtEntry{b->bwd, P->grads[b->p_beta], b->C, b->rot});
    if (b->p_bias >= 0) cv.push_back(CvtEntry{b->dbias, P->grads[b->p_bias], b->C, 0});
    else cv.push_back(CvtEntry{b->dbias, nullptr, 0, 0});
  }
  for (size_t l = 0; l < P->lv.size(); ++l) {
    if (P->lv[l].ns == 128 || P->lv[l].ns == 0) cv.push_back(CvtEntry{P->lv[l].dw_s, nullptr, 0, 0});
    else cv.push_back(CvtEntry{P->lv[l].dw_s, P->grads[P->lv[l].p_skip_w], (int)P->numel[P->lv[l].p_skip_w], 0,
                               P->lv[l].Cin_act, P->lv[l].Cin});
  }
  cv.push_back(CvtEntry{P->dw_head, P->grads[P->p_head_w], (int)P->numel[P->p_head_w], 0});
  cv.push_back(CvtEntry{P->db_head, P->grads[P->p_head_b], (int)P->numel[P->p_head_b], 0});
  if ((int)cv.size() != P->n_cvt) return fail("internal: cvt table size mismatch");
  DIP_CUDA(cudaMemcpy(P->d_cvt, cv.data(), cv.size() * sizeof(CvtEntry), cudaMemcpyHostToDevice));
  std::vector<RunEntry> rn;
  for (BnLayer* b : P->bns) {
    RunEntry e{};
    e.fwd = b->fwd; e.C = b->C; e.rot = b->rot; e.n = b->n;
    if (!P->running.empty()) {
      e.rm = (float*)P->running[3 * b->idx]; e.rv = (float*)P->running[3 * b->idx + 1]; e.nb = P->running[3 * b->idx + 2];
      e.nb_is_float = P->nbt_is_float;
    }
    rn.push_back(e);
  }
  DIP_CUDA(cudaMemcpy(P->d_run, rn.data(), rn.size() * sizeof(RunEntry), cudaMemcpyHostToDevice));
  return 0;
}

static void stream_edge(dip_plan* P, cudaStream_t from, cudaStream_t to) {
  if (P->wev_used == P->wev.size()) {
    cudaEvent_t e;
    cudaEventCreateWithFlags(&e, cudaEventDisableTiming);
    P->wev.push_back(e);
  }
  cudaEvent_t e = P->wev[P->wev_used++];
  cudaEventRecord(e, from);
  cudaStreamWaitEvent(to, e, 0);
}
static cudaStream_t fork_side(dip_plan* P, cudaStream_t s) {
  if (!P->side_on) return s;
  stream_edge(P, s, P->wstream);
  return P->wstream;
}
static void join_side(dip_plan* P, cudaStream_t s) {
  if (P->side_on) stream_edge(P, P->wstream, s);
}
static bool skip_stream_on(const dip_plan* P) {
  static const bool off = getenv("DIP_NO_SKIPSTREAM") != nullptr;
  return P->side_on && !off;
}
static cudaStream_t fork_skip(dip_plan* P, cudaStream_t s) {
  if (!skip_stream_on(P)) return s;
  stream_edge(P, s, P->sstream);
  return P->sstream;
}
static void join_skip(dip_plan* P, cudaStream_t s) {
  if (skip_stream_on(P)) stream_edge(P, P->sstream, s);
}

static CatArgs cat_args(const dip_plan* P, const Level& v, const float* Usrc) {
  CatArgs a;
  a.U = Usrc; a.raw_s = v.raw_s;
  if (v.ns > 0) a.bn_s = bn_ref(P, v.bn_s);
  else a.bn_s = BnRef{nullptr, nullptr, nullptr, 0, 0, 0.f};
  a.Cu = v.cu; a.Cs = v.ns; a.H = v.H; a.W = v.W; a.bilinear = v.bilinear;
  return a;
}
static const float* level_usrc(const dip_plan* P, int l) {
  const int L = (int)P->lv.size();
  return l == L - 1 ? P->lv[l].P_d2 : P->lv[l + 1].U;
}

static int fwd_level(dip_plan* P, int l, cudaStream_t s) {
  Level& v = P->lv[l];
  const int prec = P->desc.precision;
  const int CS = v.ns, nd = v.nd, nu = v.nu;
  const bool last = l == (int)P->lv.size() - 1;
  const float* pin_interior = v.Pin + ((size_t)(v.W + 2) + 1) * v.Cin;
  const bool bf = prec == DIP_PRECISION_BF16;
  if (CS > 0) {
    cudaStream_t ks = fork_skip(P, s);
    if (CS == 128)
      DIP_CHECK(v.sk.run_fprop(prec, P->params[v.p_skip_b], ks));
    else
      ENQ(&P->rec, hbm(H_SKINNY_FWD, 0), (double)v.H * v.W * (v.Cin_act + CS) * sizeof(float), ks,
          launch_skinny_fwd(pin_interior, v.Cin, v.W + 2, P->params[v.p_skip_w], P->params[v.p_skip_b], v.Cin, CS, v.H, v.W, v.raw_s, 0,
                            v.bn_s.fwd, ks, v.Cin_act));
  }
  DIP_CHECK(v.d1.run_fprop(prec, P->params[v.d1.p_b], s));
  if (v.rawF != nullptr) {
    ENQ(&P->rec, kUntimed, 0, s, launch_avgpool2(v.rawF, v.h, v.w, nd, v.raw_d1, s));
    ENQ(&P->rec, kUntimed, 0, s, launch_channel_stats(v.raw_d1, nd, nd, v.h * v.w, v.bn_d1.fwd, s));
  }
  ENQ(&P->rec, hbm(H_BN_ACT_WRITE, 1), (double)nd * ((double)v.h * v.w + (double)(v.h + 2) * (v.w + 2)) * sizeof(float), s,
      launch_bn_act_write(v.raw_d1, nd, bn_ref(P, v.bn_d1), v.h, v.w, bf ? nullptr : v.P_d1, nd, 1, 1, P->act_fun, s, Twin{v.P_d1_16, nd},
                          P->zero_pad));
  DIP_CHECK(v.d2.run_fprop(prec, P->params[v.d2.p_b], s));
  ENQ(&P->rec, hbm(H_BN_ACT_WRITE, last ? 0 : 1),
      (double)nd * ((double)v.h * v.w + (last ? (double)v.h * v.w : (double)(v.h + 2) * (v.w + 2))) * sizeof(float), s,
      launch_bn_act_write(v.raw_d2, nd, bn_ref(P, v.bn_d2), v.h, v.w, (bf && !last && P->lv[l + 1].ns != 4) ? nullptr : v.P_d2, nd, last ? 0 : 1, 1, P->act_fun, s,
                          Twin{last ? nullptr : v.P_d2_16, nd}, P->zero_pad));
  if (!last) DIP_CHECK(fwd_level(P, l + 1, s));
  if (CS > 0) join_skip(P, s);
  CatArgs ca = cat_args(P, v, level_usrc(P, l));
  const double cat_in = ((double)v.cu * v.h * v.w + (double)CS * v.H * v.W) * sizeof(float);
  ENQ(&P->rec, hbm(H_CAT_STATS, v.bilinear), cat_in, s, launch_cat_stats(ca, v.bn_cat.fwd, P->act_fun, s));
  ENQ(&P->rec, hbm(H_CAT_WRITE, v.bilinear), cat_in + ((double)v.cu + CS) * (v.H + 2) * (v.W + 2) * sizeof(float), s,
      launch_cat_write(ca, bn_ref(P, v.bn_cat), v.P_cat, P->act_fun, s, Twin{v.P_cat16, v.cat_ld16}, P->zero_pad));
  DIP_CHECK(v.up.run_fprop(prec, P->params[v.up.p_b], s));
  ENQ(&P->rec, hbm(H_BN_ACT_WRITE, 0), 2.0 * nu * v.H * v.W * sizeof(float), s,
      launch_bn_act_write(v.raw_u, nu, bn_ref(P, v.bn_u), v.H, v.W, bf ? nullptr : v.A_u, nu, 0, 1, P->act_fun, s, Twin{v.A_u16, nu}));
  DIP_CHECK(v.c11.run_fprop(prec, P->params[v.c11.p_b], s));
  if (l > 0 || nu != 128) {
    ENQ(&P->rec, hbm(H_BN_ACT_WRITE, 0), 2.0 * nu * v.H * v.W * sizeof(float), s,
        launch_bn_act_write(v.raw_v, nu, bn_ref(P, v.bn_v), v.H, v.W, v.U, nu, 0, 1, P->act_fun, s));
    if (l == 0) {
      ENQ(&P->rec, hbm(H_SKINNY_FWD, 1), ((double)nu + P->desc.out_channels) * v.H * v.W * sizeof(float), s,
          launch_skinny_fwd(v.U, nu, v.W, P->params[P->p_head_w], P->params[P->p_head_b], nu, P->desc.out_channels, v.H, v.W,
                            P->out_saved, P->desc.need_sigmoid != 0 ? 1 : 2, nullptr, s));
    }
  } else {
    HeadRef hd{P->params[P->p_head_w], P->params[P->p_head_b], P->desc.out_channels, P->out_saved, P->desc.need_sigmoid != 0};
    ENQ(&P->rec, hbm(H_BN_ACT_HEAD, 0), (128.0 + P->desc.out_channels) * v.H * v.W * sizeof(float), s,
        launch_bn_act_head(v.raw_v, bn_ref(P, v.bn_v), v.H, v.W, hd, P->act_fun, s));
  }
  DIP_CUDA(cudaGetLastError());
  return 0;
}

static void plan_pack(dip_plan* P, cudaStream_t s) {
  dim3 grid((unsigned)((P->pack_max + 255) / 256 < 64 ? (P->pack_max + 255) / 256 : 64), P->n_pack);
  double bytes = 0;
  for (ConvOp* op : P->convs)
    bytes += ((double)op->N * op->C * op->k * op->k + (op->do_fprop ? (double)op->wp_f_elems() : 0.0) + (op->has_dgrad ? (double)op->wp_d_elems() : 0.0)) * sizeof(float);
  ENQ(&P->rec, hbm(H_PACK, 0), bytes, s, launch_k(k_pack_table, dim3(grid), dim3(256), 0, s, 1, P->d_pack));
}

static int plan_forward(dip_plan* P, const float* z, const float* noise, float sigma, float* out, cudaStream_t s) {
  if (!P->bound) return fail("dip_forward: parameters not bound (call dip_plan_bind)");
  P->side_on = getenv("DIP_NO_SIDE") == nullptr;
  if (!P->prepacked) { P->wev_used = 0; P->rec.n = 0; }
  ENQ(&P->rec, kUntimed, 0, s, DIP_CUDA(cudaMemsetAsync(P->acc_fwd, 0, P->acc_fwd_n * sizeof(double), s)));
  if (!P->prepacked) plan_pack(P, fork_side(P, s));
  P->prepacked = false;
  Level& v0 = P->lv[0];
  if (P->fnoise.on)
    ENQ(&P->rec, hbm(H_NOISE, 1), ((double)v0.Cin_act * v0.H * v0.W + (double)v0.Cin * (v0.H + 2) * (v0.W + 2)) * sizeof(float), s,
        launch_noise_pad(P->fnoise.z0, P->fnoise.sigma, P->fnoise.seed, P->fnoise.offset, P->fnoise.it_dev, v0.Pin, v0.Cin,
                         v0.H, v0.W, v0.Cin_act, s, Twin{v0.Pin16, v0.Pin_ld16}, P->zero_pad));
  else
    ENQ(&P->rec, hbm(H_INPUT_PAD, noise != nullptr),
        ((noise != nullptr ? 2.0 : 1.0) * v0.Cin_act * v0.H * v0.W + (double)v0.Cin * (v0.H + 2) * (v0.W + 2)) * sizeof(float), s,
        launch_input_pad(z, noise, sigma, v0.Pin, v0.Cin, v0.H, v0.W, s, v0.Cin_act, Twin{v0.Pin16, v0.Pin_ld16}, P->zero_pad));
  join_side(P, s);
  DIP_CHECK(fwd_level(P, 0, s));
  if (out != nullptr && out != P->out_saved)
    ENQ(&P->rec, kUntimed, 0, s,
        DIP_CUDA(cudaMemcpyAsync(out, P->out_saved, (size_t)v0.H * v0.W * P->desc.out_channels * sizeof(float), cudaMemcpyDeviceToDevice, s)));
  ENQ(&P->rec, kUntimed, 0, s, launch_k(k_running_table, dim3(P->n_run), dim3(160), 0, s, 1, P->d_run));
  DIP_CUDA(cudaGetLastError());
  P->launches_fwd = P->rec.n;
  return 0;
}

static int bn_bwd(dip_plan* P, const float* raw, int ld_raw, BnLayer& b, int act, GradSrc src, int H, int W, float* draw,
                  cudaStream_t s, uint16_t* draw16 = nullptr) {
  if (draw16 != nullptr) draw = nullptr;
  if (src.kind == 1) src.zero_pad = P->zero_pad;
  BnRef r = bn_ref(P, b);
  const double px = (double)H * W, C4 = b.C * sizeof(float);
  double gsrc = px * C4;
  if (src.kind == 1) gsrc = (src.zero_pad ? px : (double)(H + 2) * (W + 2)) * C4 + (src.ds != nullptr ? px * 4 * sizeof(float) : 0.0) + (src.add != nullptr ? px * C4 : 0.0);
  else if (src.kind == 2) gsrc = 4.0 * px * C4;
  else if (src.kind == 3) gsrc = px * 4 * sizeof(float);
  ENQ(&P->rec, hbm(H_BN_BWD_REDUCE, src.kind), px * C4 + gsrc, s, launch_bn_bwd_reduce(raw, ld_raw, r, act, P->act_fun, src, H, W, b.bwd, s));
  ENQ(&P->rec, hbm(H_BN_BWD_APPLY, src.kind), px * C4 + gsrc + px * C4, s,
      launch_bn_bwd_apply(raw, ld_raw, r, act, P->act_fun, src, H, W, b.bwd, draw, b.dbias, s, Twin{draw16, b.C}));
  return 0;
}
static GradSrc src_plain(const float* g, int ld, int coff) { GradSrc s{}; s.kind = 0; s.g = g; s.ld = ld; s.coff = coff; return s; }
static GradSrc src_fold(const float* gp, int ld, const float* ds, const float* w2, int n2) {
  GradSrc s{}; s.kind = 1; s.g = gp; s.ld = ld; s.coff = 0; s.ds = ds; s.w2 = w2; s.n2 = n2; return s;
}
static GradSrc src_upadj(const float* d, int ld, int bilinear) { GradSrc s{}; s.kind = 2; s.g = d; s.ld = ld; s.coff = 0; s.bilinear = bilinear; return s; }

static constexpr int kDeferLevel = 2;
static int flush_deferred(dip_plan* P, int prec, cudaStream_t s) {
  if (P->deferred.empty()) return 0;
  cudaStream_t ws = fork_side(P, s);
  for (ConvOp* op : P->deferred) DIP_CHECK(op->run_wgrad(prec, ws));
  P->deferred.clear();
  return 0;
}
static int conv_backward(dip_plan* P, ConvOp& op, bool dgrad, int prec, cudaStream_t s, int level = 99) {
  if (P->side_on && level < kDeferLevel && (int)P->lv.size() > kDeferLevel) {
    if (dgrad) DIP_CHECK(op.run_dgrad(prec, s));
    P->deferred.push_back(&op);
    return 0;
  }
  cudaStream_t ws = fork_side(P, s);
  if (dgrad) DIP_CHECK(op.run_dgrad(prec, s));
  return op.run_wgrad(prec, ws);
}

static int bwd_level(dip_plan* P, int l, GradSrc src_v, cudaStream_t s) {
  Level& v = P->lv[l];
  const int prec = P->desc.precision;
  const int CS = v.ns, nd = v.nd, nu = v.nu;
  const int CC = v.cu + CS;
  const bool last = l == (int)P->lv.size() - 1;
  DIP_CHECK(bn_bwd(P, v.raw_v, nu, v.bn_v, 1, src_v, v.H, v.W, v.dRaw_v, s, v.dRaw_v16));
  if (l == kDeferLevel) DIP_CHECK(flush_deferred(P, prec, s));
  DIP_CHECK(conv_backward(P, v.c11, true, prec, s, l));
  DIP_CHECK(bn_bwd(P, v.raw_u, nu, v.bn_u, 1, src_plain(v.dA_u, nu, 0), v.H, v.W, v.dRaw_u, s, v.dRaw_u16));
  if (CS == 128) {
    cudaStream_t ws = fork_side(P, s);
    DIP_CHECK(v.up_a.run_dgrad(prec, s));
    DIP_CHECK(v.up_b.run_dgrad(prec, s));
    DIP_CHECK(v.up_a.run_wgrad(prec, ws));
    DIP_CHECK(v.up_b.run_wgrad(prec, ws));
  } else {
    DIP_CHECK(conv_backward(P, v.up, true, prec, s, l));
  }
  BnRef rc = bn_ref(P, v.bn_cat);
  const double catb = ((double)v.H * v.W + (P->zero_pad ? (double)v.H * v.W : (double)(v.H + 2) * (v.W + 2))) * CC * sizeof(float);
  ENQ(&P->rec, hbm(H_CAT_BWD_REDUCE, 0), catb, s, launch_cat_bwd_reduce(v.P_cat, rc, v.dP_cat, CC, v.H, v.W, v.bn_cat.bwd, s, P->zero_pad));
  ENQ(&P->rec, hbm(H_CAT_BWD_APPLY, 0), catb + (double)v.H * v.W * CC * sizeof(float), s,
      launch_cat_bwd_apply(v.P_cat, rc, v.dP_cat, CC, v.H, v.W, v.bn_cat.bwd, v.dCat, s, P->zero_pad));
  cudaStream_t ks = fork_skip(P, s);
  ENQ(&P->rec, hbm(H_UPADJ, v.bilinear), (double)v.cu * ((double)v.H * v.W + (double)v.h * v.w) * sizeof(float), s,
      launch_upadj(v.dCat, CC, 0, v.h, v.w, v.cu, v.bilinear, v.dUp, s));
  if (CS > 0) DIP_CHECK(bn_bwd(P, v.raw_s, CS, v.bn_s, 1, src_plain(v.dCat, CC, v.cu), v.H, v.W, v.dRaw_s, ks, v.dRaw_s16));
  if (CS == 0) {
  } else if (CS == 128) {
    DIP_CHECK(v.sk.run_wgrad(prec, fork_side(P, ks)));
    if (l > 0 || P->desc.input_grad) DIP_CHECK(v.sk.run_dgrad(prec, ks));
  } else {
    const float* pin_interior = v.Pin + ((size_t)(v.W + 2) + 1) * v.Cin;
    ENQ(&P->rec, hbm(H_SKINNY_BWD, 0), (double)v.H * v.W * (v.Cin_act + CS) * sizeof(float), ks,
        launch_skinny_bwd(pin_interior, v.Cin, v.W + 2, P->params[v.p_skip_w], v.Cin, CS, v.H, v.W, v.dRaw_s, nullptr, 0,
                          (l == 0 && P->desc.input_grad) ? v.dS : nullptr, v.dw_s, nullptr , ks, v.Cin_act));
  }
  GradSrc src_d2;
  if (!last) {
    DIP_CHECK(bwd_level(P, l + 1, src_plain(v.dUp, v.cu, 0), s));
    join_skip(P, s);
    Level& n = P->lv[l + 1];
    if (n.ns == 128) { src_d2 = src_fold(n.dPin, nd, nullptr, nullptr, 0); src_d2.add = n.dS; src_d2.ld_add = nd; }
    else if (n.ns == 0) src_d2 = src_fold(n.dPin, nd, nullptr, nullptr, 0);
    else src_d2 = src_fold(n.dPin, nd, n.dRaw_s, P->params[n.p_skip_w], n.ns);
  } else {
    src_d2 = src_plain(v.dUp, v.cu, 0);
  }
  DIP_CHECK(bn_bwd(P, v.raw_d2, nd, v.bn_d2, 1, src_d2, v.h, v.w, v.dRaw_d2, s, v.dRaw_d2_16));
  DIP_CHECK(conv_backward(P, v.d2, true, prec, s));
  const bool d1_dgrad = l > 0 || P->desc.input_grad != 0;
  const bool avg = v.rawF != nullptr;
  DIP_CHECK(bn_bwd(P, v.raw_d1, nd, v.bn_d1, 1, src_fold(v.dP_d1, nd, nullptr, nullptr, 0), v.h, v.w, v.dRaw_d1, s,
                   avg ? nullptr : v.dRaw_d1_16));
  if (avg)
    ENQ(&P->rec, kUntimed, 0, s,
        launch_avgpool2_bwd(v.dRaw_d1, v.h, v.w, nd, prec == DIP_PRECISION_BF16 ? nullptr : v.dRawF, s, Twin{v.dRawF16, nd}));
  DIP_CHECK(conv_backward(P, v.d1, d1_dgrad, prec, s));
  DIP_CUDA(cudaGetLastError());
  return 0;
}

static int plan_backward(dip_plan* P, const float* dout, cudaStream_t s) {
  if (!P->bound) return fail("dip_backward: parameters not bound");
  P->rec.n = 0;
  P->deferred.clear();
  ENQ(&P->rec, kUntimed, 0, s, DIP_CUDA(cudaMemsetAsync(P->acc_bwd, 0, P->acc_bwd_n * sizeof(double), s)));
  P->side_on = getenv("DIP_NO_SIDE") == nullptr;
  Level& v0 = P->lv[0];
  GradSrc sh{};
  ENQ(&P->rec, hbm(H_HEAD_DLOGIT, 0), (2.0 * P->desc.out_channels + 4.0) * P->H * P->W * sizeof(float), s,
      launch_head_dlogit(dout, P->out_saved, P->desc.out_channels, P->H * P->W, P->dl4, s, P->desc.need_sigmoid != 0));
  sh.kind = 3; sh.dl4 = P->dl4; sh.wh = P->params[P->p_head_w]; sh.nh = P->desc.out_channels;
  sh.dwh = P->dw_head; sh.dbh = P->db_head;
  DIP_CHECK(bwd_level(P, 0, sh, s));
  DIP_CHECK(flush_deferred(P, P->desc.precision, s));
  join_side(P, s);
  join_skip(P, s);
  ENQ(&P->rec, kUntimed, 0, s, launch_k(k_cvt_table, dim3(P->n_cvt), dim3(128), 0, s, 1, P->d_cvt));
  if (is_tc(P->desc.precision) && P->n_unpack > 0)
    ENQ(&P->rec, hbm(H_WGRAD_REDUCE, 1), 2.0 * (double)P->wacc_bytes, s,
        launch_k(k_wgrad_unpack_table, dim3(64, P->n_unpack), dim3(256), 0, s, 1, P->d_unpack));
  DIP_CUDA(cudaGetLastError());
  P->launches_bwd = P->rec.n;
  return 0;
}

}

struct dip_adam {
  int n = 0;
  std::vector<long long> numel;
  int nblocks = 0;
  float** d_p = nullptr; const float** d_g = nullptr; float** d_m = nullptr; float** d_v = nullptr;
  int* d_blk_tensor = nullptr; int* d_blk_start = nullptr; int* d_numel = nullptr;
  long long* d_off = nullptr;
  bool bound = false;
  unsigned long long id = 0;
  unsigned long long bind_gen = 0;
};
static unsigned long long g_adam_serial = 0;

static void drop_graphs(dip_plan* P) {
  for (cudaGraphExec_t* g : {&P->gexec, &P->gfwd, &P->gbwd})
    if (*g != nullptr) { cudaGraphExecDestroy(*g); *g = nullptr; }
}
static bool graphs_enabled(const dip_plan* P) { return !P->timer.on && getenv("DIP_NO_GRAPH") == nullptr; }
static int ensure_gstream(dip_plan* P) {
  if (P->gstream == nullptr) {
    int lo = 0, hi = 0;
    DIP_CUDA(cudaDeviceGetStreamPriorityRange(&lo, &hi));
    if (getenv("DIP_NO_PRIO") != nullptr) hi = 0;
    DIP_CUDA(cudaStreamCreateWithPriority(&P->gstream, cudaStreamNonBlocking, hi));
    DIP_CUDA(cudaEventCreateWithFlags(&P->gev_in, cudaEventDisableTiming));
    DIP_CUDA(cudaEventCreateWithFlags(&P->gev_out, cudaEventDisableTiming));
  }
  return 0;
}
template <class Body>
static int capture_graph(cudaStream_t gs, cudaGraphExec_t* exec, Body body) {
  cudaGraph_t graph = nullptr;
  DIP_CUDA(cudaStreamBeginCapture(gs, cudaStreamCaptureModeThreadLocal));
  const int rc = body(gs);
  cudaError_t ce = cudaStreamEndCapture(gs, &graph);
  if (rc != 0) { if (graph) cudaGraphDestroy(graph); return rc; }
  if (ce != cudaSuccess) return fail(std::string("cudaStreamEndCapture: ") + cudaGetErrorString(ce));
  ce = cudaGraphInstantiate(exec, graph, 0);
  cudaGraphDestroy(graph);
  if (ce != cudaSuccess) { *exec = nullptr; return fail(std::string("cudaGraphInstantiate: ") + cudaGetErrorString(ce)); }
  return 0;
}
template <class Body>
static int replay_graph(dip_plan* P, cudaGraphExec_t* exec, cudaStream_t s, Body body) {
  DIP_CHECK(ensure_gstream(P));
  cudaStream_t gs = P->gstream;
  DIP_CUDA(cudaEventRecord(P->gev_in, s));
  DIP_CUDA(cudaStreamWaitEvent(gs, P->gev_in, 0));
  if (*exec == nullptr) DIP_CHECK(capture_graph(gs, exec, body));
  DIP_CUDA(cudaGraphLaunch(*exec, gs));
  DIP_CUDA(cudaEventRecord(P->gev_out, gs));
  DIP_CUDA(cudaStreamWaitEvent(s, P->gev_out, 0));
  return 0;
}

extern "C" {

const char* dip_last_error(void) { return g_err.c_str(); }
int dip_version(void) { return 100; }

static_assert(DIP_ACT_LEAKY_RELU == kActLeakyRelu && DIP_ACT_SWISH == kActSwish && DIP_ACT_ELU == kActElu &&
                  DIP_ACT_NONE == kActNone, "the plan's act_fun is passed to the kernels as their kAct* kind");
static int apply_opts(dip_plan* P, const dip_plan_opts* opts) {
  const int pad = opts != nullptr ? opts->pad_mode : DIP_PAD_REFLECTION;
  if (pad != DIP_PAD_REFLECTION && pad != DIP_PAD_ZERO)
    return fail("dip-b200: pad_mode must be DIP_PAD_REFLECTION (0) or DIP_PAD_ZERO (1), got " + std::to_string(pad));
  const int act = opts != nullptr ? opts->act_fun : DIP_ACT_LEAKY_RELU;
  if (act < DIP_ACT_LEAKY_RELU || act > DIP_ACT_NONE)
    return fail("dip-b200: act_fun must be DIP_ACT_LEAKY_RELU (0), DIP_ACT_SWISH (1), DIP_ACT_ELU (2) or DIP_ACT_NONE (3), got " +
                std::to_string(act));
  P->zero_pad = pad == DIP_PAD_ZERO;
  P->act_fun = act;
  return 0;
}

size_t dip_plan_workspace_bytes_opts(const dip_net_desc* desc, int H, int W, const dip_plan_opts* opts) {
  dip_plan P;
  P.desc = *desc; P.H = H; P.W = W; P.dry = true;
  if (apply_opts(&P, opts) != 0) return 0;
  Arena A{nullptr};
  if (build_plan(&P, A) != 0) return 0;
  return A.off + 4096;
}
size_t dip_plan_workspace_bytes(const dip_net_desc* desc, int H, int W) { return dip_plan_workspace_bytes_opts(desc, H, W, nullptr); }

int dip_plan_create_opts(const dip_net_desc* desc, int H, int W, const dip_plan_opts* opts, void* workspace,
                         size_t workspace_bytes, dip_plan** out) {
  DIP_CHECK(engine_init());
  const size_t need = dip_plan_workspace_bytes_opts(desc, H, W, opts);
  if (need == 0) return -1;
  if (workspace == nullptr || workspace_bytes < need) return fail("dip_plan_create: workspace too small");
  if (reinterpret_cast<uintptr_t>(workspace) % 256 != 0) return fail("dip_plan_create: workspace must be 256-byte aligned");
  dip_plan* P = new dip_plan();
  P->desc = *desc; P->H = H; P->W = W; P->ws = (uint8_t*)workspace; P->ws_bytes = workspace_bytes;
  apply_opts(P, opts);
  Arena A{(uint8_t*)workspace};
  if (build_plan(P, A) != 0) { delete P; return -1; }
  *out = P;
  return 0;
}
int dip_plan_create(const dip_net_desc* desc, int H, int W, void* workspace, size_t workspace_bytes, dip_plan** out) {
  return dip_plan_create_opts(desc, H, W, nullptr, workspace, workspace_bytes, out);
}
void dip_plan_destroy(dip_plan* plan) {
  if (plan == nullptr) return;
  if (plan->gexec) cudaGraphExecDestroy(plan->gexec);
  if (plan->gfwd) cudaGraphExecDestroy(plan->gfwd);
  if (plan->gbwd) cudaGraphExecDestroy(plan->gbwd);
  if (plan->gstream) cudaStreamDestroy(plan->gstream);
  if (plan->gev_in) cudaEventDestroy(plan->gev_in);
  if (plan->gev_out) cudaEventDestroy(plan->gev_out);
  for (cudaEvent_t e : plan->timer.pool) cudaEventDestroy(e);
  for (cudaEvent_t e : plan->wev) cudaEventDestroy(e);
  if (plan->wstream) cudaStreamDestroy(plan->wstream);
  if (plan->sstream) cudaStreamDestroy(plan->sstream);
  delete plan;
}
int dip_plan_num_params(const dip_plan* plan) { return (int)plan->numel.size(); }
int dip_plan_num_bn(const dip_plan* plan) { return (int)plan->bns.size(); }
long long dip_plan_param_numel(const dip_plan* plan, int index) {
  if (index < 0 || index >= (int)plan->numel.size()) return -1;
  return plan->numel[index];
}
int dip_plan_bind(dip_plan* P, void* const* params, void* const* grads, void* const* bn_running, int nbt_is_float) {
  drop_graphs(P);
  P->nbt_is_float = nbt_is_float;
  const int n = (int)P->numel.size();
  P->params.resize(n); P->grads.resize(n);
  for (int i = 0; i < n; ++i) {
    if (params[i] == nullptr || grads[i] == nullptr) return fail("dip_plan_bind: null parameter/gradient pointer");
    P->params[i] = (float*)params[i]; P->grads[i] = (float*)grads[i];
  }
  P->running.clear();
  if (bn_running != nullptr) P->running.assign(bn_running, bn_running + 3 * P->bns.size());
  DIP_CHECK(upload_tables(P));
  P->bound = true;
  return 0;
}
int dip_forward(dip_plan* P, const void* z, const void* noise, float sigma, void* out, dip_stream_t stream) {
  cudaStream_t s = (cudaStream_t)stream;
  if (!P->bound) return fail("dip_forward: parameters not bound (call dip_plan_bind)");
  if (noise != nullptr || !graphs_enabled(P))
    return plan_forward(P, (const float*)z, (const float*)noise, sigma, (float*)out, s);
  const size_t nz = (size_t)P->H * P->W * P->desc.in_channels * sizeof(float);
  DIP_CUDA(cudaMemcpyAsync(P->zbuf, z, nz, cudaMemcpyDeviceToDevice, s));
  DIP_CHECK(replay_graph(P, &P->gfwd, s, [&](cudaStream_t gs) { return plan_forward(P, P->zbuf, nullptr, 0.f, nullptr, gs); }));
  if (out != nullptr && out != P->out_saved)
    DIP_CUDA(cudaMemcpyAsync(out, P->out_saved, (size_t)P->H * P->W * P->desc.out_channels * sizeof(float), cudaMemcpyDeviceToDevice, s));
  return 0;
}
int dip_backward(dip_plan* P, const void* dout, dip_stream_t stream) {
  cudaStream_t s = (cudaStream_t)stream;
  if (!P->bound) return fail("dip_backward: parameters not bound");
  if (!graphs_enabled(P)) return plan_backward(P, (const float*)dout, s);
  if (dout != P->dout)
    DIP_CUDA(cudaMemcpyAsync(P->dout, dout, (size_t)P->H * P->W * P->desc.out_channels * sizeof(float), cudaMemcpyDeviceToDevice, s));
  return replay_graph(P, &P->gbwd, s, [&](cudaStream_t gs) { return plan_backward(P, P->dout, gs); });
}
int dip_loss_mse(const void* out, const void* target, const void* mask, int channels, int hw, double* loss, void* dout,
                 dip_stream_t stream) {
  launch_mse((const float*)out, (const float*)target, (const float*)mask, channels, hw, loss, (float*)dout, nullptr, (cudaStream_t)stream);
  DIP_CUDA(cudaGetLastError());
  return 0;
}
int dip_noise_perturb(const void* z0, void* z, float sigma, uint64_t seed, uint64_t offset, size_t n, dip_stream_t stream) {
  if (n % 4 != 0) return fail("dip_noise_perturb: n must be a multiple of 4");
  launch_noise((const float*)z0, (float*)z, sigma, seed, offset, nullptr, n, (cudaStream_t)stream);
  DIP_CUDA(cudaGetLastError());
  return 0;
}

int dip_lanczos_down_fwd(const void* x, int C, int H, int W, const void* kern, int K, int factor, int pad, void* y,
                         dip_stream_t stream) {
  DIP_CHECK(engine_init());
  if (K < 1 || factor < 1 || pad < 0) return fail("dip_lanczos_down_fwd: bad K / factor / pad");
  if (down_out_size(H, K, factor, pad) < 1 || down_out_size(W, K, factor, pad) < 1)
    return fail("dip_lanczos_down_fwd: image smaller than the filter");
  DIP_CUDA(launch_down_fwd((const float*)x, C, H, W, (const float*)kern, K, factor, pad, (float*)y, (cudaStream_t)stream));
  return 0;
}
int dip_lanczos_down_bwd(const void* dy, int C, int H, int W, const void* kern, int K, int factor, int pad, void* dx,
                         dip_stream_t stream) {
  DIP_CHECK(engine_init());
  if (K < 1 || factor < 1 || pad < 0) return fail("dip_lanczos_down_bwd: bad K / factor / pad");
  if (down_out_size(H, K, factor, pad) < 1 || down_out_size(W, K, factor, pad) < 1)
    return fail("dip_lanczos_down_bwd: image smaller than the filter");
  DIP_CUDA(launch_down_bwd((const float*)dy, C, H, W, (const float*)kern, K, factor, pad, (float*)dx, (cudaStream_t)stream));
  return 0;
}
int dip_lanczos_down_out_size(int n, int K, int factor, int pad) { return down_out_size(n, K, factor, pad); }

int dip_plan_set_downsampler(dip_plan* P, const float* kern_host, int K, int factor, int pad) {
  if (P->gexec != nullptr) { cudaGraphExecDestroy(P->gexec); P->gexec = nullptr; }
  if (kern_host == nullptr || K == 0) { P->ds_K = 0; return 0; }
  if (K < 1 || K > dip_plan::kDownMaxK || factor < 1 || pad < 0) return fail("dip_plan_set_downsampler: bad K / factor / pad");
  const int Ho = down_out_size(P->H, K, factor, pad), Wo = down_out_size(P->W, K, factor, pad);
  if (Ho < 1 || Wo < 1 || Ho > P->H || Wo > P->W) return fail("dip_plan_set_downsampler: unsupported output size");
  DIP_CUDA(cudaMemcpy(P->ds_kern, kern_host, (size_t)K * K * sizeof(float), cudaMemcpyHostToDevice));
  P->ds_K = K; P->ds_f = factor; P->ds_pad = pad; P->ds_Ho = Ho; P->ds_Wo = Wo;
  return 0;
}

int dip_adam_create(int ntensors, const long long* numel, dip_adam** out) {
  dip_adam* a = new dip_adam();
  a->id = ++g_adam_serial;
  a->n = ntensors;
  a->numel.assign(numel, numel + ntensors);
  std::vector<int> bt, bs, ne;
  std::vector<long long> off;
  const int chunk = adam_chunk();
  for (int t = 0; t < ntensors; ++t) {
    off.push_back(t == 0 ? 0 : off.back() + numel[t - 1]);
    ne.push_back((int)numel[t]);
    for (long long st = 0; st < numel[t]; st += chunk) { bt.push_back(t); bs.push_back((int)st); }
  }
  a->nblocks = (int)bt.size();
  DIP_CUDA(cudaMalloc(&a->d_p, ntensors * sizeof(void*)));
  DIP_CUDA(cudaMalloc(&a->d_g, ntensors * sizeof(void*)));
  DIP_CUDA(cudaMalloc(&a->d_m, ntensors * sizeof(void*)));
  DIP_CUDA(cudaMalloc(&a->d_v, ntensors * sizeof(void*)));
  DIP_CUDA(cudaMalloc(&a->d_blk_tensor, bt.size() * sizeof(int)));
  DIP_CUDA(cudaMalloc(&a->d_blk_start, bs.size() * sizeof(int)));
  DIP_CUDA(cudaMalloc(&a->d_numel, ne.size() * sizeof(int)));
  DIP_CUDA(cudaMalloc(&a->d_off, off.size() * sizeof(long long)));
  DIP_CUDA(cudaMemcpy(a->d_blk_tensor, bt.data(), bt.size() * sizeof(int), cudaMemcpyHostToDevice));
  DIP_CUDA(cudaMemcpy(a->d_blk_start, bs.data(), bs.size() * sizeof(int), cudaMemcpyHostToDevice));
  DIP_CUDA(cudaMemcpy(a->d_numel, ne.data(), ne.size() * sizeof(int), cudaMemcpyHostToDevice));
  DIP_CUDA(cudaMemcpy(a->d_off, off.data(), off.size() * sizeof(long long), cudaMemcpyHostToDevice));
  *out = a;
  return 0;
}
void dip_adam_destroy(dip_adam* a) {
  if (!a) return;
  cudaFree(a->d_p); cudaFree(a->d_g); cudaFree(a->d_m); cudaFree(a->d_v);
  cudaFree(a->d_blk_tensor); cudaFree(a->d_blk_start); cudaFree(a->d_numel); cudaFree(a->d_off);
  delete a;
}
int dip_adam_bind(dip_adam* a, void* const* p, void* const* g, void* const* m, void* const* v) {
  DIP_CUDA(cudaMemcpy(a->d_p, p, a->n * sizeof(void*), cudaMemcpyHostToDevice));
  DIP_CUDA(cudaMemcpy(a->d_g, g, a->n * sizeof(void*), cudaMemcpyHostToDevice));
  DIP_CUDA(cudaMemcpy(a->d_m, m, a->n * sizeof(void*), cudaMemcpyHostToDevice));
  DIP_CUDA(cudaMemcpy(a->d_v, v, a->n * sizeof(void*), cudaMemcpyHostToDevice));
  a->bound = true;
  a->bind_gen++;
  return 0;
}
int dip_adam_step(dip_adam* a, double lr, double beta1, double beta2, double eps, int step, dip_stream_t stream) {
  if (!a->bound) return fail("dip_adam_step: not bound");
  if (step < 1) return fail("dip_adam_step: step must be >= 1");
  AdamTable t{a->d_p, a->d_g, a->d_m, a->d_v, a->d_blk_tensor, a->d_blk_start, a->d_numel, a->nblocks};
  launch_adam(t, lr, beta1, beta2, eps, step, nullptr, (cudaStream_t)stream);
  DIP_CUDA(cudaGetLastError());
  return 0;
}

static int run_body(dip_plan* P, dip_adam* adam, const float* z0, const float* target, const float* mask, float sigma,
                    uint64_t seed, int step_base, double lr, float* out, double* loss_slot, const dip_track* track, int* it_dev,
                    cudaStream_t s) {
  const size_t nz = (size_t)P->H * P->W * P->desc.in_channels;
  const int hw = P->H * P->W;
  const float* zin = z0;
  Recorder runner{&P->timer};
  P->side_on = getenv("DIP_NO_SIDE") == nullptr;
  P->wev_used = 0;
  if (P->side_on && P->bound) {
    P->rec.n = 0;
    plan_pack(P, fork_side(P, s));
    P->prepacked = true;
  }
  if (sigma > 0.f && P->W % 4 != 0) {
    ENQ(&runner, hbm(H_NOISE, 0), 2.0 * nz * sizeof(float), s, launch_noise(z0, P->zbuf, sigma, seed, (uint64_t)step_base, it_dev, nz, s));
    zin = P->zbuf;
  } else if (sigma > 0.f) {
    P->fnoise.on = true; P->fnoise.z0 = z0; P->fnoise.sigma = sigma; P->fnoise.seed = seed; P->fnoise.offset = (uint64_t)step_base;
    P->fnoise.it_dev = it_dev;
  }
  const int frc = plan_forward(P, zin, nullptr, 0.f, out, s);
  P->fnoise.on = false;
  DIP_CHECK(frc);
  const int* slot_idx = it_dev != nullptr ? it_dev + 1 : nullptr;
  if (P->ds_K > 0) {
    const int co = P->desc.out_channels;
    ENQ(&runner, hbm(H_DOWN_FWD, 0), (double)co * ((double)P->H * P->W + (double)P->ds_Ho * P->ds_Wo) * sizeof(float), s,
        DIP_CUDA(launch_down_fwd(P->out_saved, co, P->H, P->W, P->ds_kern, P->ds_K, P->ds_f, P->ds_pad, P->ds_y, s)));
    launch_mse(P->ds_y, target, mask, co, P->ds_Ho * P->ds_Wo, loss_slot, P->ds_dy, slot_idx, s);
    ENQ(&runner, hbm(H_DOWN_BWD, 0), (double)co * ((double)P->H * P->W + (double)P->ds_Ho * P->ds_Wo) * sizeof(float), s,
        DIP_CUDA(launch_down_bwd(P->ds_dy, co, P->H, P->W, P->ds_kern, P->ds_K, P->ds_f, P->ds_pad, P->dout, s)));
  } else {
    ENQ(&runner, hbm(H_MSE, mask != nullptr), (3.0 * P->desc.out_channels + (mask != nullptr ? 1.0 : 0.0)) * hw * sizeof(float), s,
        launch_mse(P->out_saved, target, mask, P->desc.out_channels, hw, loss_slot, P->dout, slot_idx, s));
  }
  TrackState* tstate = track != nullptr ? (TrackState*)track->state : nullptr;
  if (track != nullptr) {
    const int n = P->desc.out_channels * hw;
    const bool gt = track->gt != nullptr;
    ENQ(&runner, hbm(H_TRACK_OUT, gt), (gt ? 4.0 : 3.0) * n * sizeof(float), s,
        launch_track_out(P->out_saved, (const float*)track->gt, (float*)track->out_avg, tstate, (float)track->exp_weight,
                         (float)(1.0 - track->exp_weight), n, track->records, slot_idx, s));
    ENQ(&runner, hbm(H_TRACK_DECIDE, 0), (kTrackRecord + 1.0) * sizeof(double) + 2.0 * sizeof(TrackState), s,
        launch_track_decide(loss_slot, track->records, tstate, track->show_every, track->backtrack_db, gt, slot_idx, s));
  }
  DIP_CHECK(plan_backward(P, P->dout, s));
  if (!adam->bound) return fail("dip_run_iterations: adam not bound");
  AdamTable t{adam->d_p, adam->d_g, adam->d_m, adam->d_v, adam->d_blk_tensor, adam->d_blk_start, adam->d_numel, adam->nblocks};
  {
    double np_ = 0; for (long long n : adam->numel) np_ += (double)n;
    if (track == nullptr)
      ENQ(&runner, hbm(H_ADAM, 0), 7.0 * np_ * sizeof(float), s, launch_adam(t, lr, 0.9, 0.999, 1e-8, step_base + 1, it_dev, s));
    else
      ENQ(&runner, hbm(H_ADAM_TRACK, 0), 8.0 * np_ * sizeof(float), s,
          launch_adam_track(t, lr, 0.9, 0.999, 1e-8, step_base + 1, it_dev, AdamTrack{tstate, (float*)track->snapshot, adam->d_off}, s));
  }
  if (it_dev != nullptr) launch_advance(it_dev, s);
  DIP_CUDA(cudaGetLastError());
  return 0;
}

size_t dip_track_state_bytes(void) { return sizeof(TrackState); }

static int check_track(const dip_track* t) {
  if (!(t->exp_weight >= 0.0 && t->exp_weight < 1.0))
    return fail("dip_run_iterations_tracked: exp_weight must be in [0, 1), got " + std::to_string(t->exp_weight));
  if (t->show_every < 0) return fail("dip_run_iterations_tracked: show_every must be >= 0, got " + std::to_string(t->show_every));
  if (t->backtrack_db != t->backtrack_db) return fail("dip_run_iterations_tracked: backtrack_db is NaN");
  if (t->out_avg == nullptr) return fail("dip_run_iterations_tracked: out_avg is NULL");
  if (t->snapshot == nullptr) return fail("dip_run_iterations_tracked: snapshot is NULL");
  if (t->state == nullptr) return fail("dip_run_iterations_tracked: state is NULL");
  if (t->records == nullptr) return fail("dip_run_iterations_tracked: records is NULL");
  return 0;
}

int dip_run_iterations_tracked(dip_plan* P, dip_adam* adam, const void* z0, const void* target, const void* mask, float sigma,
                               uint64_t seed, int step0, int iters, double lr, void* out, double* loss_hist,
                               const dip_track* track, dip_stream_t stream) {
  cudaStream_t s = (cudaStream_t)stream;
  if (track != nullptr) DIP_CHECK(check_track(track));
  if (iters <= 0) return 0;
  const bool use_graph = !P->timer.on && getenv("DIP_NO_GRAPH") == nullptr;
  if (!use_graph) {
    for (int i = 0; i < iters; ++i) {
      double* lp = loss_hist != nullptr ? loss_hist + i : P->loss_ring;
      DIP_CUDA(cudaMemsetAsync(lp, 0, sizeof(double), s));
      dip_track ti;
      if (track != nullptr) {
        ti = *track;
        ti.records = track->records + (size_t)kTrackRecord * i;
        DIP_CUDA(cudaMemsetAsync(ti.records, 0, kTrackRecord * sizeof(double), s));
      }
      DIP_CHECK(run_body(P, adam, (const float*)z0, (const float*)target, (const float*)mask, sigma, seed, step0 + i, lr,
                         (float*)out, lp, track != nullptr ? &ti : nullptr, nullptr, s));
    }
    return 0;
  }
  if (loss_hist == nullptr && iters > dip_plan::kLossRing) {
    for (int done = 0; done < iters; done += dip_plan::kLossRing) {
      const int n = iters - done < dip_plan::kLossRing ? iters - done : dip_plan::kLossRing;
      dip_track tc;
      if (track != nullptr) { tc = *track; tc.records = track->records + (size_t)kTrackRecord * done; }
      DIP_CHECK(dip_run_iterations_tracked(P, adam, z0, target, mask, sigma, seed, step0 + done, n, lr, out, nullptr,
                                           track != nullptr ? &tc : nullptr, stream));
    }
    return 0;
  }
  DIP_CHECK(ensure_gstream(P));
  cudaStream_t gs = P->gstream;
  DIP_CUDA(cudaEventRecord(P->gev_in, s));
  DIP_CUDA(cudaStreamWaitEvent(gs, P->gev_in, 0));
  double* slots = loss_hist != nullptr ? loss_hist : P->loss_ring;
  dip_plan::GraphKey key;
  key.z0 = z0; key.target = target; key.mask = mask; key.out = out; key.slots = slots;
  key.adam_id = adam->id; key.adam_bind = adam->bind_gen; key.sigma = sigma; key.seed = seed; key.lr = lr;
  if (track != nullptr) key.track = *track;
  if (P->gexec == nullptr || !(key == P->gkey)) {
    if (P->gexec != nullptr) { cudaGraphExecDestroy(P->gexec); P->gexec = nullptr; }
    DIP_CHECK(capture_graph(gs, &P->gexec, [&](cudaStream_t cs) {
      return run_body(P, adam, (const float*)z0, (const float*)target, (const float*)mask, sigma, seed, 0, lr, (float*)out, slots,
                      track, P->it_dev, cs);
    }));
    P->gkey = key;
  }
  const int init[2] = {step0, 0};
  DIP_CUDA(cudaMemcpyAsync(P->it_dev, init, sizeof init, cudaMemcpyHostToDevice, gs));
  DIP_CUDA(cudaMemsetAsync(slots, 0, (size_t)iters * sizeof(double), gs));
  if (track != nullptr) DIP_CUDA(cudaMemsetAsync(track->records, 0, (size_t)iters * kTrackRecord * sizeof(double), gs));
  for (int i = 0; i < iters; ++i) DIP_CUDA(cudaGraphLaunch(P->gexec, gs));
  DIP_CUDA(cudaEventRecord(P->gev_out, gs));
  DIP_CUDA(cudaStreamWaitEvent(s, P->gev_out, 0));
  return 0;
}

int dip_run_iterations(dip_plan* P, dip_adam* adam, const void* z0, const void* target, const void* mask, float sigma,
                       uint64_t seed, int step0, int iters, double lr, void* out, double* loss_hist, dip_stream_t stream) {
  return dip_run_iterations_tracked(P, adam, z0, target, mask, sigma, seed, step0, iters, lr, out, loss_hist, nullptr, stream);
}

int dip_input_grad(dip_plan* P, void* dz, dip_stream_t stream) {
  if (!P->desc.input_grad) return fail("dip_input_grad: the plan was created without input_grad");
  Level& v = P->lv[0];
  launch_input_grad(v.dPin, v.ns > 0 ? v.dS : nullptr, v.Cin, v.Cin_act, v.H, v.W, (float*)dz, (cudaStream_t)stream, P->zero_pad);
  DIP_CUDA(cudaGetLastError());
  return 0;
}

int dip_plan_buffer(const dip_plan* plan, const char* name, void** ptr, int* dims4) {
  auto it = plan->bufs.find(name);
  if (it == plan->bufs.end()) return fail(std::string("dip_plan_buffer: unknown buffer ") + name);
  *ptr = it->second.ptr;
  dims4[0] = it->second.rows; dims4[1] = it->second.cols; dims4[2] = it->second.ld; dims4[3] = it->second.c;
  return 0;
}
int dip_plan_set_timing(dip_plan* plan, int enable) {
  plan->timer.on = enable != 0;
  plan->timer.reset();
  return 0;
}
int dip_plan_get_timing(dip_plan* plan, double* ms3, double* flops3, int* launches3) {
  for (int i = 0; i < 3; ++i) { ms3[i] = 0; flops3[i] = 0; launches3[i] = 0; }
  for (const Timer::Rec& r : plan->timer.recs) {
    DIP_CUDA(cudaEventSynchronize(plan->timer.pool[r.e1]));
    float ms = 0.f;
    DIP_CUDA(cudaEventElapsedTime(&ms, plan->timer.pool[r.e0], plan->timer.pool[r.e1]));
    if (r.cls > 2) continue;
    ms3[r.cls] += ms; flops3[r.cls] += r.flops; launches3[r.cls] += 1;
  }
  plan->timer.reset();
  return 0;
}
int dip_plan_get_timing_records(dip_plan* plan, int max_records, int* cls, double* flops, double* ms) {
  int n = 0;
  for (const Timer::Rec& r : plan->timer.recs) {
    if (n >= max_records) break;
    DIP_CUDA(cudaEventSynchronize(plan->timer.pool[r.e1]));
    float t = 0.f;
    DIP_CUDA(cudaEventElapsedTime(&t, plan->timer.pool[r.e0], plan->timer.pool[r.e1]));
    cls[n] = r.cls; flops[n] = r.flops; ms[n] = t;
    ++n;
  }
  plan->timer.reset();
  return n;
}
int dip_plan_num_launches(const dip_plan* plan, int* fwd, int* bwd) {
  *fwd = plan->launches_fwd; *bwd = plan->launches_bwd;
  return 0;
}

size_t dip_op_scratch_bytes(void) { return (size_t)96 << 20; }

static int op_setup(const char* name, ConvOp& op, int prec, const float* w, float* dw, void* scratch, cudaStream_t s) {
  DIP_CHECK(engine_init());
  const int max_c = op.do_fprop ? 256 : 160;
  if (op.N != 128) return fail(std::string(name) + ": N must be 128");
  if (op.C % 4 != 0 || op.C > max_c)
    return fail(std::string(name) + ": C must be a multiple of 4 and <= " + std::to_string(max_c));
  op.bf16 = prec == DIP_PRECISION_BF16;
  op.set_shapes();
  const bool pack = op.do_fprop || op.has_dgrad;
  const bool cast_dy = op.bf16 && (op.has_dgrad || op.do_wgrad), cast_in = op.bf16 && (op.do_fprop || op.do_wgrad);
  if (cast_in) op.in_ld16 = round_up(op.in_ld, 8);
  Arena A{(uint8_t*)scratch};
  op.wp_f = op.do_fprop ? A.get<float>(op.wp_f_elems()) : nullptr;
  op.wp_d = op.has_dgrad ? A.get<float>(op.wp_d_elems()) : nullptr;
  PackEntry* d_pack = pack ? A.get<PackEntry>(1) : nullptr;
  UnpackEntry* d_unpack = op.do_wgrad ? A.get<UnpackEntry>(1) : nullptr;
  op.partial = op.do_wgrad ? A.get<float>(op.partial_elems(prec)) : nullptr;
  const long long dy_px = (long long)op.out_h * op.out_w, in_px = (long long)op.in_rows * op.in_cols;
  uint16_t* dy16 = cast_dy ? A.get<uint16_t>(dy_px * op.N) : nullptr;
  uint16_t* in16 = cast_in ? A.get<uint16_t>(in_px * op.in_ld16) : nullptr;
  if (A.off > dip_op_scratch_bytes())
    return fail(std::string(name) + ": the operands need " + std::to_string((A.off + (1 << 20) - 1) >> 20) +
                " MB of scratch, more than dip_op_scratch_bytes() = " + std::to_string(dip_op_scratch_bytes() >> 20) + " MB");
  if (pack) {
    const PackEntry e = op.pack_entry(prec, w);
    DIP_CUDA(cudaMemcpyAsync(d_pack, &e, sizeof e, cudaMemcpyHostToDevice, s));
    launch_k(k_pack_table, dim3(64, 1), dim3(256), 0, s, 1, (const PackEntry*)d_pack);
  }
  if (op.do_wgrad) {
    const UnpackEntry e = op.unpack_entry(prec, dw);
    DIP_CUDA(cudaMemcpyAsync(d_unpack, &e, sizeof e, cudaMemcpyHostToDevice, s));
    op.unpack = d_unpack;
  }
  if (cast_dy) launch_cast_bf16(op.dy, op.N, op.N, dy_px, Twin{dy16, op.N}, s);
  if (cast_in) launch_cast_bf16(op.in, op.in_ld, op.in_ld, in_px, Twin{in16, op.in_ld16}, s);
  op.dy16 = dy16; op.in16 = in16;
  DIP_CUDA(cudaGetLastError());
  return is_tc(prec) ? op.build_tc() : 0;
}

int dip_op_conv_fprop(const void* a, int a_h, int a_w, int a_c, const void* w, const void* bias, int N, int C, int k, int stride,
                      int offx, int offy, int rot, void* d, int d_h, int d_w, double* stats, int precision, void* scratch,
                      dip_stream_t stream) {
  cudaStream_t s = (cudaStream_t)stream;
  ConvOp op;
  op.N = N; op.C = C; op.k = k; op.stride = stride; op.rot = rot;
  op.do_fprop = true; op.has_dgrad = false; op.do_wgrad = false;
  op.in = (const float*)a; op.in_rows = a_h; op.in_cols = a_w; op.in_ld = a_c; op.offx = offx; op.offy = offy;
  op.out = (float*)d; op.out_h = d_h; op.out_w = d_w; op.stats = stats;
  DIP_CHECK(op_setup("dip_op_conv_fprop", op, precision, (const float*)w, nullptr, scratch, s));
  return op.run_fprop(precision, (const float*)bias, s);
}
int dip_op_conv_dgrad(const void* dy, int dy_h, int dy_w, const void* w, int N, int C, int k, int rot, void* dx, int dx_h, int dx_w,
                      int precision, void* scratch, dip_stream_t stream) {
  cudaStream_t s = (cudaStream_t)stream;
  ConvOp op;
  op.N = N; op.C = C; op.k = k; op.rot = rot;
  op.do_fprop = false; op.has_dgrad = true; op.do_wgrad = false;
  op.dy = (const float*)dy; op.out_h = dy_h; op.out_w = dy_w;
  op.dg_out = (float*)dx; op.dg_out_h = dx_h; op.dg_out_w = dx_w; op.dg_off = -(k - 1);
  DIP_CHECK(op_setup("dip_op_conv_dgrad", op, precision, (const float*)w, nullptr, scratch, s));
  return op.run_dgrad(precision, s);
}
int dip_op_conv_dgrad_s2(const void* dy, int dy_h, int dy_w, const void* w, int N, int C, int rot, void* dx, int precision,
                         void* scratch, dip_stream_t stream) {
  cudaStream_t s = (cudaStream_t)stream;
  ConvOp op;
  op.N = N; op.C = C; op.k = 3; op.stride = 2; op.rot = rot;
  op.do_fprop = false; op.has_dgrad = true; op.do_wgrad = false;
  op.dg_s2 = true;
  op.dy = (const float*)dy; op.out_h = dy_h; op.out_w = dy_w;
  op.dg_out = (float*)dx; op.dg_out_h = 2 * dy_h + 2; op.dg_out_w = 2 * dy_w + 2; op.dg_off = -2;
  DIP_CHECK(op_setup("dip_op_conv_dgrad_s2", op, precision, (const float*)w, nullptr, scratch, s));
  return op.run_dgrad(precision, s);
}
int dip_op_conv_wgrad(const void* dy, int dy_h, int dy_w, const void* a, int a_h, int a_w, int a_c, int N, int C, int k, int stride,
                      int offx, int offy, int rot, void* dw, int precision, void* scratch, dip_stream_t stream) {
  cudaStream_t s = (cudaStream_t)stream;
  ConvOp op;
  op.N = N; op.C = C; op.k = k; op.stride = stride; op.rot = rot;
  op.do_fprop = false; op.has_dgrad = false; op.do_wgrad = true;
  op.in = (const float*)a; op.in_rows = a_h; op.in_cols = a_w; op.in_ld = a_c; op.offx = offx; op.offy = offy;
  op.dy = (const float*)dy; op.out_h = dy_h; op.out_w = dy_w;
  DIP_CHECK(op_setup("dip_op_conv_wgrad", op, precision, nullptr, (float*)dw, scratch, s));
  return op.run_wgrad(precision, s);
}

}
```

### deep-image-prior_b200/csrc/wgmma.cuh

```cuda
#pragma once
#include <stdint.h>

namespace dip {

__device__ __forceinline__ void wgmma_tf32_n32(float (&d)[16], uint64_t a, uint64_t b) {
  asm volatile("{\n\t.reg .pred p;\n\tsetp.ne.b32 p, %18, 0;\n\t"
               "wgmma.mma_async.sync.aligned.m64n32k8.f32.tf32.tf32 {%0, %1, %2, %3, %4, %5, %6, %7, %8, %9, %10, %11, %12, %13, %14, %15}, %16, %17, p, 1, 1;\n\t}\n"
               : "+f"(d[0]), "+f"(d[1]), "+f"(d[2]), "+f"(d[3]), "+f"(d[4]), "+f"(d[5]), "+f"(d[6]), "+f"(d[7]), "+f"(d[8]), "+f"(d[9]), "+f"(d[10]), "+f"(d[11]), "+f"(d[12]), "+f"(d[13]), "+f"(d[14]), "+f"(d[15])
               : "l"(a), "l"(b), "r"(1) : "memory");
}
__device__ __forceinline__ void wgmma_tf32_n64(float (&d)[32], uint64_t a, uint64_t b) {
  asm volatile("{\n\t.reg .pred p;\n\tsetp.ne.b32 p, %34, 0;\n\t"
               "wgmma.mma_async.sync.aligned.m64n64k8.f32.tf32.tf32 {%0, %1, %2, %3, %4, %5, %6, %7, %8, %9, %10, %11, %12, %13, %14, %15, %16, %17, %18, %19, %20, %21, %22, %23, %24, %25, %26, %27, %28, %29, %30, %31}, %32, %33, p, 1, 1;\n\t}\n"
               : "+f"(d[0]), "+f"(d[1]), "+f"(d[2]), "+f"(d[3]), "+f"(d[4]), "+f"(d[5]), "+f"(d[6]), "+f"(d[7]), "+f"(d[8]), "+f"(d[9]), "+f"(d[10]), "+f"(d[11]), "+f"(d[12]), "+f"(d[13]), "+f"(d[14]), "+f"(d[15]), "+f"(d[16]), "+f"(d[17]), "+f"(d[18]), "+f"(d[19]), "+f"(d[20]), "+f"(d[21]), "+f"(d[22]), "+f"(d[23]), "+f"(d[24]), "+f"(d[25]), "+f"(d[26]), "+f"(d[27]), "+f"(d[28]), "+f"(d[29]), "+f"(d[30]), "+f"(d[31])
               : "l"(a), "l"(b), "r"(1) : "memory");
}
__device__ __forceinline__ void wgmma_tf32_n96(float (&d)[48], uint64_t a, uint64_t b) {
  asm volatile("{\n\t.reg .pred p;\n\tsetp.ne.b32 p, %50, 0;\n\t"
               "wgmma.mma_async.sync.aligned.m64n96k8.f32.tf32.tf32 {%0, %1, %2, %3, %4, %5, %6, %7, %8, %9, %10, %11, %12, %13, %14, %15, %16, %17, %18, %19, %20, %21, %22, %23, %24, %25, %26, %27, %28, %29, %30, %31, %32, %33, %34, %35, %36, %37, %38, %39, %40, %41, %42, %43, %44, %45, %46, %47}, %48, %49, p, 1, 1;\n\t}\n"
               : "+f"(d[0]), "+f"(d[1]), "+f"(d[2]), "+f"(d[3]), "+f"(d[4]), "+f"(d[5]), "+f"(d[6]), "+f"(d[7]), "+f"(d[8]), "+f"(d[9]), "+f"(d[10]), "+f"(d[11]), "+f"(d[12]), "+f"(d[13]), "+f"(d[14]), "+f"(d[15]), "+f"(d[16]), "+f"(d[17]), "+f"(d[18]), "+f"(d[19]), "+f"(d[20]), "+f"(d[21]), "+f"(d[22]), "+f"(d[23]), "+f"(d[24]), "+f"(d[25]), "+f"(d[26]), "+f"(d[27]), "+f"(d[28]), "+f"(d[29]), "+f"(d[30]), "+f"(d[31]), "+f"(d[32]), "+f"(d[33]), "+f"(d[34]), "+f"(d[35]), "+f"(d[36]), "+f"(d[37]), "+f"(d[38]), "+f"(d[39]), "+f"(d[40]), "+f"(d[41]), "+f"(d[42]), "+f"(d[43]), "+f"(d[44]), "+f"(d[45]), "+f"(d[46]), "+f"(d[47])
               : "l"(a), "l"(b), "r"(1) : "memory");
}
__device__ __forceinline__ void wgmma_tf32_n128(float (&d)[64], uint64_t a, uint64_t b) {
  asm volatile("{\n\t.reg .pred p;\n\tsetp.ne.b32 p, %66, 0;\n\t"
               "wgmma.mma_async.sync.aligned.m64n128k8.f32.tf32.tf32 {%0, %1, %2, %3, %4, %5, %6, %7, %8, %9, %10, %11, %12, %13, %14, %15, %16, %17, %18, %19, %20, %21, %22, %23, %24, %25, %26, %27, %28, %29, %30, %31, %32, %33, %34, %35, %36, %37, %38, %39, %40, %41, %42, %43, %44, %45, %46, %47, %48, %49, %50, %51, %52, %53, %54, %55, %56, %57, %58, %59, %60, %61, %62, %63}, %64, %65, p, 1, 1;\n\t}\n"
               : "+f"(d[0]), "+f"(d[1]), "+f"(d[2]), "+f"(d[3]), "+f"(d[4]), "+f"(d[5]), "+f"(d[6]), "+f"(d[7]), "+f"(d[8]), "+f"(d[9]), "+f"(d[10]), "+f"(d[11]), "+f"(d[12]), "+f"(d[13]), "+f"(d[14]), "+f"(d[15]), "+f"(d[16]), "+f"(d[17]), "+f"(d[18]), "+f"(d[19]), "+f"(d[20]), "+f"(d[21]), "+f"(d[22]), "+f"(d[23]), "+f"(d[24]), "+f"(d[25]), "+f"(d[26]), "+f"(d[27]), "+f"(d[28]), "+f"(d[29]), "+f"(d[30]), "+f"(d[31]), "+f"(d[32]), "+f"(d[33]), "+f"(d[34]), "+f"(d[35]), "+f"(d[36]), "+f"(d[37]), "+f"(d[38]), "+f"(d[39]), "+f"(d[40]), "+f"(d[41]), "+f"(d[42]), "+f"(d[43]), "+f"(d[44]), "+f"(d[45]), "+f"(d[46]), "+f"(d[47]), "+f"(d[48]), "+f"(d[49]), "+f"(d[50]), "+f"(d[51]), "+f"(d[52]), "+f"(d[53]), "+f"(d[54]), "+f"(d[55]), "+f"(d[56]), "+f"(d[57]), "+f"(d[58]), "+f"(d[59]), "+f"(d[60]), "+f"(d[61]), "+f"(d[62]), "+f"(d[63])
               : "l"(a), "l"(b), "r"(1) : "memory");
}
__device__ __forceinline__ void wgmma_tf32_n144(float (&d)[72], uint64_t a, uint64_t b) {
  asm volatile("{\n\t.reg .pred p;\n\tsetp.ne.b32 p, %74, 0;\n\t"
               "wgmma.mma_async.sync.aligned.m64n144k8.f32.tf32.tf32 {%0, %1, %2, %3, %4, %5, %6, %7, %8, %9, %10, %11, %12, %13, %14, %15, %16, %17, %18, %19, %20, %21, %22, %23, %24, %25, %26, %27, %28, %29, %30, %31, %32, %33, %34, %35, %36, %37, %38, %39, %40, %41, %42, %43, %44, %45, %46, %47, %48, %49, %50, %51, %52, %53, %54, %55, %56, %57, %58, %59, %60, %61, %62, %63, %64, %65, %66, %67, %68, %69, %70, %71}, %72, %73, p, 1, 1;\n\t}\n"
               : "+f"(d[0]), "+f"(d[1]), "+f"(d[2]), "+f"(d[3]), "+f"(d[4]), "+f"(d[5]), "+f"(d[6]), "+f"(d[7]), "+f"(d[8]), "+f"(d[9]), "+f"(d[10]), "+f"(d[11]), "+f"(d[12]), "+f"(d[13]), "+f"(d[14]), "+f"(d[15]), "+f"(d[16]), "+f"(d[17]), "+f"(d[18]), "+f"(d[19]), "+f"(d[20]), "+f"(d[21]), "+f"(d[22]), "+f"(d[23]), "+f"(d[24]), "+f"(d[25]), "+f"(d[26]), "+f"(d[27]), "+f"(d[28]), "+f"(d[29]), "+f"(d[30]), "+f"(d[31]), "+f"(d[32]), "+f"(d[33]), "+f"(d[34]), "+f"(d[35]), "+f"(d[36]), "+f"(d[37]), "+f"(d[38]), "+f"(d[39]), "+f"(d[40]), "+f"(d[41]), "+f"(d[42]), "+f"(d[43]), "+f"(d[44]), "+f"(d[45]), "+f"(d[46]), "+f"(d[47]), "+f"(d[48]), "+f"(d[49]), "+f"(d[50]), "+f"(d[51]), "+f"(d[52]), "+f"(d[53]), "+f"(d[54]), "+f"(d[55]), "+f"(d[56]), "+f"(d[57]), "+f"(d[58]), "+f"(d[59]), "+f"(d[60]), "+f"(d[61]), "+f"(d[62]), "+f"(d[63]), "+f"(d[64]), "+f"(d[65]), "+f"(d[66]), "+f"(d[67]), "+f"(d[68]), "+f"(d[69]), "+f"(d[70]), "+f"(d[71])
               : "l"(a), "l"(b), "r"(1) : "memory");
}
__device__ __forceinline__ void wgmma_tf32_n160(float (&d)[80], uint64_t a, uint64_t b) {
  asm volatile("{\n\t.reg .pred p;\n\tsetp.ne.b32 p, %82, 0;\n\t"
               "wgmma.mma_async.sync.aligned.m64n160k8.f32.tf32.tf32 {%0, %1, %2, %3, %4, %5, %6, %7, %8, %9, %10, %11, %12, %13, %14, %15, %16, %17, %18, %19, %20, %21, %22, %23, %24, %25, %26, %27, %28, %29, %30, %31, %32, %33, %34, %35, %36, %37, %38, %39, %40, %41, %42, %43, %44, %45, %46, %47, %48, %49, %50, %51, %52, %53, %54, %55, %56, %57, %58, %59, %60, %61, %62, %63, %64, %65, %66, %67, %68, %69, %70, %71, %72, %73, %74, %75, %76, %77, %78, %79}, %80, %81, p, 1, 1;\n\t}\n"
               : "+f"(d[0]), "+f"(d[1]), "+f"(d[2]), "+f"(d[3]), "+f"(d[4]), "+f"(d[5]), "+f"(d[6]), "+f"(d[7]), "+f"(d[8]), "+f"(d[9]), "+f"(d[10]), "+f"(d[11]), "+f"(d[12]), "+f"(d[13]), "+f"(d[14]), "+f"(d[15]), "+f"(d[16]), "+f"(d[17]), "+f"(d[18]), "+f"(d[19]), "+f"(d[20]), "+f"(d[21]), "+f"(d[22]), "+f"(d[23]), "+f"(d[24]), "+f"(d[25]), "+f"(d[26]), "+f"(d[27]), "+f"(d[28]), "+f"(d[29]), "+f"(d[30]), "+f"(d[31]), "+f"(d[32]), "+f"(d[33]), "+f"(d[34]), "+f"(d[35]), "+f"(d[36]), "+f"(d[37]), "+f"(d[38]), "+f"(d[39]), "+f"(d[40]), "+f"(d[41]), "+f"(d[42]), "+f"(d[43]), "+f"(d[44]), "+f"(d[45]), "+f"(d[46]), "+f"(d[47]), "+f"(d[48]), "+f"(d[49]), "+f"(d[50]), "+f"(d[51]), "+f"(d[52]), "+f"(d[53]), "+f"(d[54]), "+f"(d[55]), "+f"(d[56]), "+f"(d[57]), "+f"(d[58]), "+f"(d[59]), "+f"(d[60]), "+f"(d[61]), "+f"(d[62]), "+f"(d[63]), "+f"(d[64]), "+f"(d[65]), "+f"(d[66]), "+f"(d[67]), "+f"(d[68]), "+f"(d[69]), "+f"(d[70]), "+f"(d[71]), "+f"(d[72]), "+f"(d[73]), "+f"(d[74]), "+f"(d[75]), "+f"(d[76]), "+f"(d[77]), "+f"(d[78]), "+f"(d[79])
               : "l"(a), "l"(b), "r"(1) : "memory");
}
__device__ __forceinline__ void wgmma_bf16_n32(float (&d)[16], uint64_t a, uint64_t b) {
  asm volatile("{\n\t.reg .pred p;\n\tsetp.ne.b32 p, %18, 0;\n\t"
               "wgmma.mma_async.sync.aligned.m64n32k16.f32.bf16.bf16 {%0, %1, %2, %3, %4, %5, %6, %7, %8, %9, %10, %11, %12, %13, %14, %15}, %16, %17, p, 1, 1, 0, 0;\n\t}\n"
               : "+f"(d[0]), "+f"(d[1]), "+f"(d[2]), "+f"(d[3]), "+f"(d[4]), "+f"(d[5]), "+f"(d[6]), "+f"(d[7]), "+f"(d[8]), "+f"(d[9]), "+f"(d[10]), "+f"(d[11]), "+f"(d[12]), "+f"(d[13]), "+f"(d[14]), "+f"(d[15])
               : "l"(a), "l"(b), "r"(1) : "memory");
}
__device__ __forceinline__ void wgmma_bf16_n64(float (&d)[32], uint64_t a, uint64_t b) {
  asm volatile("{\n\t.reg .pred p;\n\tsetp.ne.b32 p, %34, 0;\n\t"
               "wgmma.mma_async.sync.aligned.m64n64k16.f32.bf16.bf16 {%0, %1, %2, %3, %4, %5, %6, %7, %8, %9, %10, %11, %12, %13, %14, %15, %16, %17, %18, %19, %20, %21, %22, %23, %24, %25, %26, %27, %28, %29, %30, %31}, %32, %33, p, 1, 1, 0, 0;\n\t}\n"
               : "+f"(d[0]), "+f"(d[1]), "+f"(d[2]), "+f"(d[3]), "+f"(d[4]), "+f"(d[5]), "+f"(d[6]), "+f"(d[7]), "+f"(d[8]), "+f"(d[9]), "+f"(d[10]), "+f"(d[11]), "+f"(d[12]), "+f"(d[13]), "+f"(d[14]), "+f"(d[15]), "+f"(d[16]), "+f"(d[17]), "+f"(d[18]), "+f"(d[19]), "+f"(d[20]), "+f"(d[21]), "+f"(d[22]), "+f"(d[23]), "+f"(d[24]), "+f"(d[25]), "+f"(d[26]), "+f"(d[27]), "+f"(d[28]), "+f"(d[29]), "+f"(d[30]), "+f"(d[31])
               : "l"(a), "l"(b), "r"(1) : "memory");
}
__device__ __forceinline__ void wgmma_bf16_n96(float (&d)[48], uint64_t a, uint64_t b) {
  asm volatile("{\n\t.reg .pred p;\n\tsetp.ne.b32 p, %50, 0;\n\t"
               "wgmma.mma_async.sync.aligned.m64n96k16.f32.bf16.bf16 {%0, %1, %2, %3, %4, %5, %6, %7, %8, %9, %10, %11, %12, %13, %14, %15, %16, %17, %18, %19, %20, %21, %22, %23, %24, %25, %26, %27, %28, %29, %30, %31, %32, %33, %34, %35, %36, %37, %38, %39, %40, %41, %42, %43, %44, %45, %46, %47}, %48, %49, p, 1, 1, 0, 0;\n\t}\n"
               : "+f"(d[0]), "+f"(d[1]), "+f"(d[2]), "+f"(d[3]), "+f"(d[4]), "+f"(d[5]), "+f"(d[6]), "+f"(d[7]), "+f"(d[8]), "+f"(d[9]), "+f"(d[10]), "+f"(d[11]), "+f"(d[12]), "+f"(d[13]), "+f"(d[14]), "+f"(d[15]), "+f"(d[16]), "+f"(d[17]), "+f"(d[18]), "+f"(d[19]), "+f"(d[20]), "+f"(d[21]), "+f"(d[22]), "+f"(d[23]), "+f"(d[24]), "+f"(d[25]), "+f"(d[26]), "+f"(d[27]), "+f"(d[28]), "+f"(d[29]), "+f"(d[30]), "+f"(d[31]), "+f"(d[32]), "+f"(d[33]), "+f"(d[34]), "+f"(d[35]), "+f"(d[36]), "+f"(d[37]), "+f"(d[38]), "+f"(d[39]), "+f"(d[40]), "+f"(d[41]), "+f"(d[42]), "+f"(d[43]), "+f"(d[44]), "+f"(d[45]), "+f"(d[46]), "+f"(d[47])
               : "l"(a), "l"(b), "r"(1) : "memory");
}
__device__ __forceinline__ void wgmma_bf16_n128(float (&d)[64], uint64_t a, uint64_t b) {
  asm volatile("{\n\t.reg .pred p;\n\tsetp.ne.b32 p, %66, 0;\n\t"
               "wgmma.mma_async.sync.aligned.m64n128k16.f32.bf16.bf16 {%0, %1, %2, %3, %4, %5, %6, %7, %8, %9, %10, %11, %12, %13, %14, %15, %16, %17, %18, %19, %20, %21, %22, %23, %24, %25, %26, %27, %28, %29, %30, %31, %32, %33, %34, %35, %36, %37, %38, %39, %40, %41, %42, %43, %44, %45, %46, %47, %48, %49, %50, %51, %52, %53, %54, %55, %56, %57, %58, %59, %60, %61, %62, %63}, %64, %65, p, 1, 1, 0, 0;\n\t}\n"
               : "+f"(d[0]), "+f"(d[1]), "+f"(d[2]), "+f"(d[3]), "+f"(d[4]), "+f"(d[5]), "+f"(d[6]), "+f"(d[7]), "+f"(d[8]), "+f"(d[9]), "+f"(d[10]), "+f"(d[11]), "+f"(d[12]), "+f"(d[13]), "+f"(d[14]), "+f"(d[15]), "+f"(d[16]), "+f"(d[17]), "+f"(d[18]), "+f"(d[19]), "+f"(d[20]), "+f"(d[21]), "+f"(d[22]), "+f"(d[23]), "+f"(d[24]), "+f"(d[25]), "+f"(d[26]), "+f"(d[27]), "+f"(d[28]), "+f"(d[29]), "+f"(d[30]), "+f"(d[31]), "+f"(d[32]), "+f"(d[33]), "+f"(d[34]), "+f"(d[35]), "+f"(d[36]), "+f"(d[37]), "+f"(d[38]), "+f"(d[39]), "+f"(d[40]), "+f"(d[41]), "+f"(d[42]), "+f"(d[43]), "+f"(d[44]), "+f"(d[45]), "+f"(d[46]), "+f"(d[47]), "+f"(d[48]), "+f"(d[49]), "+f"(d[50]), "+f"(d[51]), "+f"(d[52]), "+f"(d[53]), "+f"(d[54]), "+f"(d[55]), "+f"(d[56]), "+f"(d[57]), "+f"(d[58]), "+f"(d[59]), "+f"(d[60]), "+f"(d[61]), "+f"(d[62]), "+f"(d[63])
               : "l"(a), "l"(b), "r"(1) : "memory");
}
__device__ __forceinline__ void wgmma_bf16_n136(float (&d)[68], uint64_t a, uint64_t b) {
  asm volatile("{\n\t.reg .pred p;\n\tsetp.ne.b32 p, %70, 0;\n\t"
               "wgmma.mma_async.sync.aligned.m64n136k16.f32.bf16.bf16 {%0, %1, %2, %3, %4, %5, %6, %7, %8, %9, %10, %11, %12, %13, %14, %15, %16, %17, %18, %19, %20, %21, %22, %23, %24, %25, %26, %27, %28, %29, %30, %31, %32, %33, %34, %35, %36, %37, %38, %39, %40, %41, %42, %43, %44, %45, %46, %47, %48, %49, %50, %51, %52, %53, %54, %55, %56, %57, %58, %59, %60, %61, %62, %63, %64, %65, %66, %67}, %68, %69, p, 1, 1, 0, 0;\n\t}\n"
               : "+f"(d[0]), "+f"(d[1]), "+f"(d[2]), "+f"(d[3]), "+f"(d[4]), "+f"(d[5]), "+f"(d[6]), "+f"(d[7]), "+f"(d[8]), "+f"(d[9]), "+f"(d[10]), "+f"(d[11]), "+f"(d[12]), "+f"(d[13]), "+f"(d[14]), "+f"(d[15]), "+f"(d[16]), "+f"(d[17]), "+f"(d[18]), "+f"(d[19]), "+f"(d[20]), "+f"(d[21]), "+f"(d[22]), "+f"(d[23]), "+f"(d[24]), "+f"(d[25]), "+f"(d[26]), "+f"(d[27]), "+f"(d[28]), "+f"(d[29]), "+f"(d[30]), "+f"(d[31]), "+f"(d[32]), "+f"(d[33]), "+f"(d[34]), "+f"(d[35]), "+f"(d[36]), "+f"(d[37]), "+f"(d[38]), "+f"(d[39]), "+f"(d[40]), "+f"(d[41]), "+f"(d[42]), "+f"(d[43]), "+f"(d[44]), "+f"(d[45]), "+f"(d[46]), "+f"(d[47]), "+f"(d[48]), "+f"(d[49]), "+f"(d[50]), "+f"(d[51]), "+f"(d[52]), "+f"(d[53]), "+f"(d[54]), "+f"(d[55]), "+f"(d[56]), "+f"(d[57]), "+f"(d[58]), "+f"(d[59]), "+f"(d[60]), "+f"(d[61]), "+f"(d[62]), "+f"(d[63]), "+f"(d[64]), "+f"(d[65]), "+f"(d[66]), "+f"(d[67])
               : "l"(a), "l"(b), "r"(1) : "memory");
}
__device__ __forceinline__ void wgmma_bf16_n144(float (&d)[72], uint64_t a, uint64_t b) {
  asm volatile("{\n\t.reg .pred p;\n\tsetp.ne.b32 p, %74, 0;\n\t"
               "wgmma.mma_async.sync.aligned.m64n144k16.f32.bf16.bf16 {%0, %1, %2, %3, %4, %5, %6, %7, %8, %9, %10, %11, %12, %13, %14, %15, %16, %17, %18, %19, %20, %21, %22, %23, %24, %25, %26, %27, %28, %29, %30, %31, %32, %33, %34, %35, %36, %37, %38, %39, %40, %41, %42, %43, %44, %45, %46, %47, %48, %49, %50, %51, %52, %53, %54, %55, %56, %57, %58, %59, %60, %61, %62, %63, %64, %65, %66, %67, %68, %69, %70, %71}, %72, %73, p, 1, 1, 0, 0;\n\t}\n"
               : "+f"(d[0]), "+f"(d[1]), "+f"(d[2]), "+f"(d[3]), "+f"(d[4]), "+f"(d[5]), "+f"(d[6]), "+f"(d[7]), "+f"(d[8]), "+f"(d[9]), "+f"(d[10]), "+f"(d[11]), "+f"(d[12]), "+f"(d[13]), "+f"(d[14]), "+f"(d[15]), "+f"(d[16]), "+f"(d[17]), "+f"(d[18]), "+f"(d[19]), "+f"(d[20]), "+f"(d[21]), "+f"(d[22]), "+f"(d[23]), "+f"(d[24]), "+f"(d[25]), "+f"(d[26]), "+f"(d[27]), "+f"(d[28]), "+f"(d[29]), "+f"(d[30]), "+f"(d[31]), "+f"(d[32]), "+f"(d[33]), "+f"(d[34]), "+f"(d[35]), "+f"(d[36]), "+f"(d[37]), "+f"(d[38]), "+f"(d[39]), "+f"(d[40]), "+f"(d[41]), "+f"(d[42]), "+f"(d[43]), "+f"(d[44]), "+f"(d[45]), "+f"(d[46]), "+f"(d[47]), "+f"(d[48]), "+f"(d[49]), "+f"(d[50]), "+f"(d[51]), "+f"(d[52]), "+f"(d[53]), "+f"(d[54]), "+f"(d[55]), "+f"(d[56]), "+f"(d[57]), "+f"(d[58]), "+f"(d[59]), "+f"(d[60]), "+f"(d[61]), "+f"(d[62]), "+f"(d[63]), "+f"(d[64]), "+f"(d[65]), "+f"(d[66]), "+f"(d[67]), "+f"(d[68]), "+f"(d[69]), "+f"(d[70]), "+f"(d[71])
               : "l"(a), "l"(b), "r"(1) : "memory");
}
__device__ __forceinline__ void wgmma_bf16_n160(float (&d)[80], uint64_t a, uint64_t b) {
  asm volatile("{\n\t.reg .pred p;\n\tsetp.ne.b32 p, %82, 0;\n\t"
               "wgmma.mma_async.sync.aligned.m64n160k16.f32.bf16.bf16 {%0, %1, %2, %3, %4, %5, %6, %7, %8, %9, %10, %11, %12, %13, %14, %15, %16, %17, %18, %19, %20, %21, %22, %23, %24, %25, %26, %27, %28, %29, %30, %31, %32, %33, %34, %35, %36, %37, %38, %39, %40, %41, %42, %43, %44, %45, %46, %47, %48, %49, %50, %51, %52, %53, %54, %55, %56, %57, %58, %59, %60, %61, %62, %63, %64, %65, %66, %67, %68, %69, %70, %71, %72, %73, %74, %75, %76, %77, %78, %79}, %80, %81, p, 1, 1, 0, 0;\n\t}\n"
               : "+f"(d[0]), "+f"(d[1]), "+f"(d[2]), "+f"(d[3]), "+f"(d[4]), "+f"(d[5]), "+f"(d[6]), "+f"(d[7]), "+f"(d[8]), "+f"(d[9]), "+f"(d[10]), "+f"(d[11]), "+f"(d[12]), "+f"(d[13]), "+f"(d[14]), "+f"(d[15]), "+f"(d[16]), "+f"(d[17]), "+f"(d[18]), "+f"(d[19]), "+f"(d[20]), "+f"(d[21]), "+f"(d[22]), "+f"(d[23]), "+f"(d[24]), "+f"(d[25]), "+f"(d[26]), "+f"(d[27]), "+f"(d[28]), "+f"(d[29]), "+f"(d[30]), "+f"(d[31]), "+f"(d[32]), "+f"(d[33]), "+f"(d[34]), "+f"(d[35]), "+f"(d[36]), "+f"(d[37]), "+f"(d[38]), "+f"(d[39]), "+f"(d[40]), "+f"(d[41]), "+f"(d[42]), "+f"(d[43]), "+f"(d[44]), "+f"(d[45]), "+f"(d[46]), "+f"(d[47]), "+f"(d[48]), "+f"(d[49]), "+f"(d[50]), "+f"(d[51]), "+f"(d[52]), "+f"(d[53]), "+f"(d[54]), "+f"(d[55]), "+f"(d[56]), "+f"(d[57]), "+f"(d[58]), "+f"(d[59]), "+f"(d[60]), "+f"(d[61]), "+f"(d[62]), "+f"(d[63]), "+f"(d[64]), "+f"(d[65]), "+f"(d[66]), "+f"(d[67]), "+f"(d[68]), "+f"(d[69]), "+f"(d[70]), "+f"(d[71]), "+f"(d[72]), "+f"(d[73]), "+f"(d[74]), "+f"(d[75]), "+f"(d[76]), "+f"(d[77]), "+f"(d[78]), "+f"(d[79])
               : "l"(a), "l"(b), "r"(1) : "memory");
}

__device__ __forceinline__ void wgmma_tf32_rs_n32(float (&d)[16], const uint32_t (&a)[4], uint64_t b) {
  asm volatile("{\n\t.reg .pred p;\n\tsetp.ne.b32 p, %21, 0;\n\t"
               "wgmma.mma_async.sync.aligned.m64n32k8.f32.tf32.tf32 {%0, %1, %2, %3, %4, %5, %6, %7, %8, %9, %10, %11, %12, %13, %14, %15}, {%16, %17, %18, %19}, %20, p, 1, 1;\n\t}\n"
               : "+f"(d[0]), "+f"(d[1]), "+f"(d[2]), "+f"(d[3]), "+f"(d[4]), "+f"(d[5]), "+f"(d[6]), "+f"(d[7]), "+f"(d[8]), "+f"(d[9]), "+f"(d[10]), "+f"(d[11]), "+f"(d[12]), "+f"(d[13]), "+f"(d[14]), "+f"(d[15])
               : "r"(a[0]), "r"(a[1]), "r"(a[2]), "r"(a[3]), "l"(b), "r"(1) : "memory");
}
__device__ __forceinline__ void wgmma_tf32_rs_n64(float (&d)[32], const uint32_t (&a)[4], uint64_t b) {
  asm volatile("{\n\t.reg .pred p;\n\tsetp.ne.b32 p, %37, 0;\n\t"
               "wgmma.mma_async.sync.aligned.m64n64k8.f32.tf32.tf32 {%0, %1, %2, %3, %4, %5, %6, %7, %8, %9, %10, %11, %12, %13, %14, %15, %16, %17, %18, %19, %20, %21, %22, %23, %24, %25, %26, %27, %28, %29, %30, %31}, {%32, %33, %34, %35}, %36, p, 1, 1;\n\t}\n"
               : "+f"(d[0]), "+f"(d[1]), "+f"(d[2]), "+f"(d[3]), "+f"(d[4]), "+f"(d[5]), "+f"(d[6]), "+f"(d[7]), "+f"(d[8]), "+f"(d[9]), "+f"(d[10]), "+f"(d[11]), "+f"(d[12]), "+f"(d[13]), "+f"(d[14]), "+f"(d[15]), "+f"(d[16]), "+f"(d[17]), "+f"(d[18]), "+f"(d[19]), "+f"(d[20]), "+f"(d[21]), "+f"(d[22]), "+f"(d[23]), "+f"(d[24]), "+f"(d[25]), "+f"(d[26]), "+f"(d[27]), "+f"(d[28]), "+f"(d[29]), "+f"(d[30]), "+f"(d[31])
               : "r"(a[0]), "r"(a[1]), "r"(a[2]), "r"(a[3]), "l"(b), "r"(1) : "memory");
}
__device__ __forceinline__ void wgmma_tf32_rs_n96(float (&d)[48], const uint32_t (&a)[4], uint64_t b) {
  asm volatile("{\n\t.reg .pred p;\n\tsetp.ne.b32 p, %53, 0;\n\t"
               "wgmma.mma_async.sync.aligned.m64n96k8.f32.tf32.tf32 {%0, %1, %2, %3, %4, %5, %6, %7, %8, %9, %10, %11, %12, %13, %14, %15, %16, %17, %18, %19, %20, %21, %22, %23, %24, %25, %26, %27, %28, %29, %30, %31, %32, %33, %34, %35, %36, %37, %38, %39, %40, %41, %42, %43, %44, %45, %46, %47}, {%48, %49, %50, %51}, %52, p, 1, 1;\n\t}\n"
               : "+f"(d[0]), "+f"(d[1]), "+f"(d[2]), "+f"(d[3]), "+f"(d[4]), "+f"(d[5]), "+f"(d[6]), "+f"(d[7]), "+f"(d[8]), "+f"(d[9]), "+f"(d[10]), "+f"(d[11]), "+f"(d[12]), "+f"(d[13]), "+f"(d[14]), "+f"(d[15]), "+f"(d[16]), "+f"(d[17]), "+f"(d[18]), "+f"(d[19]), "+f"(d[20]), "+f"(d[21]), "+f"(d[22]), "+f"(d[23]), "+f"(d[24]), "+f"(d[25]), "+f"(d[26]), "+f"(d[27]), "+f"(d[28]), "+f"(d[29]), "+f"(d[30]), "+f"(d[31]), "+f"(d[32]), "+f"(d[33]), "+f"(d[34]), "+f"(d[35]), "+f"(d[36]), "+f"(d[37]), "+f"(d[38]), "+f"(d[39]), "+f"(d[40]), "+f"(d[41]), "+f"(d[42]), "+f"(d[43]), "+f"(d[44]), "+f"(d[45]), "+f"(d[46]), "+f"(d[47])
               : "r"(a[0]), "r"(a[1]), "r"(a[2]), "r"(a[3]), "l"(b), "r"(1) : "memory");
}
__device__ __forceinline__ void wgmma_tf32_rs_n128(float (&d)[64], const uint32_t (&a)[4], uint64_t b) {
  asm volatile("{\n\t.reg .pred p;\n\tsetp.ne.b32 p, %69, 0;\n\t"
               "wgmma.mma_async.sync.aligned.m64n128k8.f32.tf32.tf32 {%0, %1, %2, %3, %4, %5, %6, %7, %8, %9, %10, %11, %12, %13, %14, %15, %16, %17, %18, %19, %20, %21, %22, %23, %24, %25, %26, %27, %28, %29, %30, %31, %32, %33, %34, %35, %36, %37, %38, %39, %40, %41, %42, %43, %44, %45, %46, %47, %48, %49, %50, %51, %52, %53, %54, %55, %56, %57, %58, %59, %60, %61, %62, %63}, {%64, %65, %66, %67}, %68, p, 1, 1;\n\t}\n"
               : "+f"(d[0]), "+f"(d[1]), "+f"(d[2]), "+f"(d[3]), "+f"(d[4]), "+f"(d[5]), "+f"(d[6]), "+f"(d[7]), "+f"(d[8]), "+f"(d[9]), "+f"(d[10]), "+f"(d[11]), "+f"(d[12]), "+f"(d[13]), "+f"(d[14]), "+f"(d[15]), "+f"(d[16]), "+f"(d[17]), "+f"(d[18]), "+f"(d[19]), "+f"(d[20]), "+f"(d[21]), "+f"(d[22]), "+f"(d[23]), "+f"(d[24]), "+f"(d[25]), "+f"(d[26]), "+f"(d[27]), "+f"(d[28]), "+f"(d[29]), "+f"(d[30]), "+f"(d[31]), "+f"(d[32]), "+f"(d[33]), "+f"(d[34]), "+f"(d[35]), "+f"(d[36]), "+f"(d[37]), "+f"(d[38]), "+f"(d[39]), "+f"(d[40]), "+f"(d[41]), "+f"(d[42]), "+f"(d[43]), "+f"(d[44]), "+f"(d[45]), "+f"(d[46]), "+f"(d[47]), "+f"(d[48]), "+f"(d[49]), "+f"(d[50]), "+f"(d[51]), "+f"(d[52]), "+f"(d[53]), "+f"(d[54]), "+f"(d[55]), "+f"(d[56]), "+f"(d[57]), "+f"(d[58]), "+f"(d[59]), "+f"(d[60]), "+f"(d[61]), "+f"(d[62]), "+f"(d[63])
               : "r"(a[0]), "r"(a[1]), "r"(a[2]), "r"(a[3]), "l"(b), "r"(1) : "memory");
}
__device__ __forceinline__ void wgmma_tf32_rs_n136(float (&d)[68], const uint32_t (&a)[4], uint64_t b) {
  asm volatile("{\n\t.reg .pred p;\n\tsetp.ne.b32 p, %73, 0;\n\t"
               "wgmma.mma_async.sync.aligned.m64n136k8.f32.tf32.tf32 {%0, %1, %2, %3, %4, %5, %6, %7, %8, %9, %10, %11, %12, %13, %14, %15, %16, %17, %18, %19, %20, %21, %22, %23, %24, %25, %26, %27, %28, %29, %30, %31, %32, %33, %34, %35, %36, %37, %38, %39, %40, %41, %42, %43, %44, %45, %46, %47, %48, %49, %50, %51, %52, %53, %54, %55, %56, %57, %58, %59, %60, %61, %62, %63, %64, %65, %66, %67}, {%68, %69, %70, %71}, %72, p, 1, 1;\n\t}\n"
               : "+f"(d[0]), "+f"(d[1]), "+f"(d[2]), "+f"(d[3]), "+f"(d[4]), "+f"(d[5]), "+f"(d[6]), "+f"(d[7]), "+f"(d[8]), "+f"(d[9]), "+f"(d[10]), "+f"(d[11]), "+f"(d[12]), "+f"(d[13]), "+f"(d[14]), "+f"(d[15]), "+f"(d[16]), "+f"(d[17]), "+f"(d[18]), "+f"(d[19]), "+f"(d[20]), "+f"(d[21]), "+f"(d[22]), "+f"(d[23]), "+f"(d[24]), "+f"(d[25]), "+f"(d[26]), "+f"(d[27]), "+f"(d[28]), "+f"(d[29]), "+f"(d[30]), "+f"(d[31]), "+f"(d[32]), "+f"(d[33]), "+f"(d[34]), "+f"(d[35]), "+f"(d[36]), "+f"(d[37]), "+f"(d[38]), "+f"(d[39]), "+f"(d[40]), "+f"(d[41]), "+f"(d[42]), "+f"(d[43]), "+f"(d[44]), "+f"(d[45]), "+f"(d[46]), "+f"(d[47]), "+f"(d[48]), "+f"(d[49]), "+f"(d[50]), "+f"(d[51]), "+f"(d[52]), "+f"(d[53]), "+f"(d[54]), "+f"(d[55]), "+f"(d[56]), "+f"(d[57]), "+f"(d[58]), "+f"(d[59]), "+f"(d[60]), "+f"(d[61]), "+f"(d[62]), "+f"(d[63]), "+f"(d[64]), "+f"(d[65]), "+f"(d[66]), "+f"(d[67])
               : "r"(a[0]), "r"(a[1]), "r"(a[2]), "r"(a[3]), "l"(b), "r"(1) : "memory");
}
__device__ __forceinline__ void wgmma_tf32_rs_n160(float (&d)[80], const uint32_t (&a)[4], uint64_t b) {
  asm volatile("{\n\t.reg .pred p;\n\tsetp.ne.b32 p, %85, 0;\n\t"
               "wgmma.mma_async.sync.aligned.m64n160k8.f32.tf32.tf32 {%0, %1, %2, %3, %4, %5, %6, %7, %8, %9, %10, %11, %12, %13, %14, %15, %16, %17, %18, %19, %20, %21, %22, %23, %24, %25, %26, %27, %28, %29, %30, %31, %32, %33, %34, %35, %36, %37, %38, %39, %40, %41, %42, %43, %44, %45, %46, %47, %48, %49, %50, %51, %52, %53, %54, %55, %56, %57, %58, %59, %60, %61, %62, %63, %64, %65, %66, %67, %68, %69, %70, %71, %72, %73, %74, %75, %76, %77, %78, %79}, {%80, %81, %82, %83}, %84, p, 1, 1;\n\t}\n"
               : "+f"(d[0]), "+f"(d[1]), "+f"(d[2]), "+f"(d[3]), "+f"(d[4]), "+f"(d[5]), "+f"(d[6]), "+f"(d[7]), "+f"(d[8]), "+f"(d[9]), "+f"(d[10]), "+f"(d[11]), "+f"(d[12]), "+f"(d[13]), "+f"(d[14]), "+f"(d[15]), "+f"(d[16]), "+f"(d[17]), "+f"(d[18]), "+f"(d[19]), "+f"(d[20]), "+f"(d[21]), "+f"(d[22]), "+f"(d[23]), "+f"(d[24]), "+f"(d[25]), "+f"(d[26]), "+f"(d[27]), "+f"(d[28]), "+f"(d[29]), "+f"(d[30]), "+f"(d[31]), "+f"(d[32]), "+f"(d[33]), "+f"(d[34]), "+f"(d[35]), "+f"(d[36]), "+f"(d[37]), "+f"(d[38]), "+f"(d[39]), "+f"(d[40]), "+f"(d[41]), "+f"(d[42]), "+f"(d[43]), "+f"(d[44]), "+f"(d[45]), "+f"(d[46]), "+f"(d[47]), "+f"(d[48]), "+f"(d[49]), "+f"(d[50]), "+f"(d[51]), "+f"(d[52]), "+f"(d[53]), "+f"(d[54]), "+f"(d[55]), "+f"(d[56]), "+f"(d[57]), "+f"(d[58]), "+f"(d[59]), "+f"(d[60]), "+f"(d[61]), "+f"(d[62]), "+f"(d[63]), "+f"(d[64]), "+f"(d[65]), "+f"(d[66]), "+f"(d[67]), "+f"(d[68]), "+f"(d[69]), "+f"(d[70]), "+f"(d[71]), "+f"(d[72]), "+f"(d[73]), "+f"(d[74]), "+f"(d[75]), "+f"(d[76]), "+f"(d[77]), "+f"(d[78]), "+f"(d[79])
               : "r"(a[0]), "r"(a[1]), "r"(a[2]), "r"(a[3]), "l"(b), "r"(1) : "memory");
}

template <int N, bool BF16>
__device__ __forceinline__ void wgmma_ss(float (&d)[N / 2], uint64_t a, uint64_t b) {
  static_assert(N == 32 || N == 64 || N == 96 || N == 128 || (N == 136 && BF16) || N == 144 || N == 160, "wgmma N");
  if constexpr (BF16) {
    if constexpr (N == 32) wgmma_bf16_n32(d, a, b);
    else if constexpr (N == 64) wgmma_bf16_n64(d, a, b);
    else if constexpr (N == 96) wgmma_bf16_n96(d, a, b);
    else if constexpr (N == 128) wgmma_bf16_n128(d, a, b);
    else if constexpr (N == 136) wgmma_bf16_n136(d, a, b);
    else if constexpr (N == 144) wgmma_bf16_n144(d, a, b);
    else wgmma_bf16_n160(d, a, b);
  } else {
    if constexpr (N == 32) wgmma_tf32_n32(d, a, b);
    else if constexpr (N == 64) wgmma_tf32_n64(d, a, b);
    else if constexpr (N == 96) wgmma_tf32_n96(d, a, b);
    else if constexpr (N == 128) wgmma_tf32_n128(d, a, b);
    else if constexpr (N == 144) wgmma_tf32_n144(d, a, b);
    else wgmma_tf32_n160(d, a, b);
  }
}

template <int N>
__device__ __forceinline__ void wgmma_rs(float (&d)[N / 2], const uint32_t (&a)[4], uint64_t b) {
  static_assert(N == 32 || N == 64 || N == 96 || N == 128 || N == 136 || N == 160, "wgmma N");
  if constexpr (N == 32) wgmma_tf32_rs_n32(d, a, b);
  else if constexpr (N == 64) wgmma_tf32_rs_n64(d, a, b);
  else if constexpr (N == 96) wgmma_tf32_rs_n96(d, a, b);
  else if constexpr (N == 128) wgmma_tf32_rs_n128(d, a, b);
  else if constexpr (N == 136) wgmma_tf32_rs_n136(d, a, b);
  else wgmma_tf32_rs_n160(d, a, b);
}

}
```

Baseline: 203.5.

## Skip padded K-steps in the last channel block and add an N=136 wgmma path

Adds a ktail parameter so the final K block of each conv only issues as many k8 wgmma steps as there are real channels. It loads a correspondingly smaller weight and patch slice through new non-swizzled tail tensor maps. It also adds a tf32 m64n136 wgmma and lets 129-136 output rows use N=136 instead of padding to 160. The aim is to cut wasted tensor-core work and TMA traffic on zero-padded channels, at the cost of extra tensor maps, a switch on the tail path and more template instantiations.

```diff
diff --git a/deep-image-prior_b200/csrc/conv_tc.cu b/deep-image-prior_b200/csrc/conv_tc.cu
--- a/deep-image-prior_b200/csrc/conv_tc.cu
+++ b/deep-image-prior_b200/csrc/conv_tc.cu
@@ -25,6 +25,29 @@
                                                  float (&acc)[2][NT / 2], int x0, int y0, int opx, int opy, int n_off,
                                                  double& stat_s1, double& stat_s2, bool col_halves = false);
 __device__ __forceinline__ void tc_conv_stats_flush(const TcConvParams& p, int n_off, double stat_s1, double stat_s2);
+
+template <int NT, bool BF16, int KS>
+__device__ __forceinline__ void wgmma_ksteps(float (&acc)[2][NT / 2], uint64_t a0, uint64_t a1, uint32_t da, uint64_t b,
+                                             uint32_t db) {
+  wgmma_fence();
+#pragma unroll
+  for (int k = 0; k < KS; ++k) {
+    wgmma_ss<NT, BF16>(acc[0], a0 + k * da, b + k * db);
+    wgmma_ss<NT, BF16>(acc[1], a1 + k * da, b + k * db);
+  }
+  wgmma_commit();
+}
+template <int NT, bool BF16>
+__device__ __forceinline__ void wgmma_block(bool tail, int ktail, float (&acc)[2][NT / 2], uint64_t a0, uint64_t a1,
+                                            uint32_t da, uint64_t b_sw, uint64_t b_tail, uint32_t db_tail) {
+  switch (tail ? ktail : 4) {
+    case 1: wgmma_ksteps<NT, BF16, 1>(acc, a0, a1, da, b_tail, db_tail); break;
+    case 2: wgmma_ksteps<NT, BF16, 2>(acc, a0, a1, da, b_tail, db_tail); break;
+    case 3: wgmma_ksteps<NT, BF16, 3>(acc, a0, a1, da, b_tail, db_tail); break;
+    default: wgmma_ksteps<NT, BF16, 4>(acc, a0, a1, da, b_sw, 2); break;
+  }
+}
+__host__ __device__ constexpr int tail_b_bytes(int ktail, int n_mma) { return 2 * ktail * n_mma * 16; }
 
 template <bool BF16, int NT>
 __device__ __forceinline__ void tc_conv_consumer(const TcConvParams& p, SmemCtl* ctl,
@@ -56,17 +79,14 @@
 #pragma unroll
     for (int i = 0; i < NT / 2; ++i) { acc[0][i] = 0.f; acc[1][i] = 0.f; }
     int prev = -1;
+    int kb = 0;
     for (int kbt = 0; kbt < kb_per_tile; ++kbt) {
       mbar_wait(&ctl->full[stage], phase);
       const uint32_t a_lo = base_lo + stage * stage_step;
       const uint32_t b_lo = a_lo + kBOff;
-      wgmma_fence();
-#pragma unroll
-      for (int k = 0; k < 4; ++k) {
-        wgmma_ss<NT, BF16>(acc[0], desc_of(a_lo + 2 * k), desc_of(b_lo + 2 * k));
-        wgmma_ss<NT, BF16>(acc[1], desc_of(a_lo + kHalfOff + 2 * k), desc_of(b_lo + 2 * k));
-      }
-      wgmma_commit();
+      wgmma_block<NT, BF16>(kb == p.kblocks - 1 && p.ktail < 4, p.ktail, acc, desc_of(a_lo), desc_of(a_lo + kHalfOff), 2,
+                            desc_of(b_lo), desc_noswz(b_lo & 0x3FFFu, p.n_mma, 8), 2 * p.n_mma);
+      if (++kb == p.kblocks) kb = 0;
       if (prev >= 0) {
         wgmma_wait<1>();
         if (lane == 0) mbar_arrive(&ctl->empty[prev]);
@@ -161,6 +181,7 @@
 template <bool BF16>
 __device__ __forceinline__ void tc_conv_body(const TcConvParams& p, uint8_t* smem_raw) {
   constexpr int KE = BF16 ? 64 : 32;
+  constexpr int KG = BF16 ? 8 : 4;
   uint8_t* smem = reinterpret_cast<uint8_t*>((reinterpret_cast<uintptr_t>(smem_raw) + 1023) & ~uintptr_t(1023));
   const int nt = round32(p.n_mma);
   const int b_bytes = p.n_mma * 128;
@@ -185,6 +206,7 @@
   if (warp == 0 && lane == 0) {
     tma_prefetch_desc(&p.tmA);
     tma_prefetch_desc(&p.tmB);
+    tma_prefetch_desc(&p.tmBt);
     tma_prefetch_desc(&p.tmD);
   }
   if (warp == 1 && lane == 0) {
@@ -229,9 +251,13 @@
             mbar_wait(&ctl->empty[stage], phase ^ 1);
             uint8_t* sa = stage_base + stage * stage_bytes;
             if (elect_one()) {
-              mbar_expect_tx(&ctl->full[stage], kABytes + b_bytes);
+              const bool tail = kb == p.kblocks - 1 && p.ktail < 4;
+              mbar_expect_tx(&ctl->full[stage], kABytes + (tail ? tail_b_bytes(p.ktail, p.n_mma) : b_bytes));
               tma_load_5d(sa, &p.tmA, &ctl->full[stage], kb * KE, cpx, cx, cpy, cy);
-              tma_load_2d(sa + kABytes, &p.tmB, &ctl->full[stage], kb * KE, tap * n_total + n_off);
+              if (tail)
+                tma_load_3d(sa + kABytes, &p.tmBt, &ctl->full[stage], 0, tap * n_total + n_off, kb * (KE / KG));
+              else
+                tma_load_2d(sa + kABytes, &p.tmB, &ctl->full[stage], kb * KE, tap * n_total + n_off);
             }
             __syncwarp();
             if (++stage == p.stages) { stage = 0; phase ^= 1; }
@@ -259,7 +285,7 @@
   tc_conv_body<true>(p, smem_raw);
 }
 
-__host__ __device__ constexpr int patch_nt(int n_mma) { return n_mma == 144 ? 144 : round32(n_mma); }
+__host__ __device__ constexpr int patch_nt(int n_mma) { return n_mma == 136 || n_mma == 144 ? n_mma : round32(n_mma); }
 struct PatchCtl {
   uint64_t pfull[kPatchMaxKb];
   uint64_t pempty[kPatchMaxKb];
@@ -312,13 +338,9 @@
         mbar_wait(&ctl->full[stage], phase);
         const uint32_t b_lo = b_lo0 + stage * b_step;
         const uint32_t a16 = patch16 + kb * kSlot16 + r * row16 + s;
-        wgmma_fence();
-#pragma unroll
-        for (int k = 0; k < 4; ++k) {
-          wgmma_ss<NT, BF16>(acc[0], desc_noswz(a16 + 2 * k * kPlane16, kPlane16, row16), desc_of(b_lo + 2 * k));
-          wgmma_ss<NT, BF16>(acc[1], desc_noswz(a16 + half16 + 2 * k * kPlane16, kPlane16, row16), desc_of(b_lo + 2 * k));
-        }
-        wgmma_commit();
+        wgmma_block<NT, BF16>(kb == p.kblocks - 1 && p.ktail < 4, p.ktail, acc, desc_noswz(a16, kPlane16, row16),
+                              desc_noswz(a16 + half16, kPlane16, row16), 2 * kPlane16, desc_of(b_lo),
+                              desc_noswz(b_lo & 0x3FFFu, p.n_mma, 8), 2 * p.n_mma);
         if (prev >= 0) {
           wgmma_wait<1>();
           if (lane == 0) {
@@ -353,7 +375,7 @@
   uint8_t* b_base = smem;
   uint8_t* staging = b_base + p.stages * b_stage_bytes;
   uint8_t* patch_base = staging + p.n_chunks * kChunkBytes;
-  SmemCtl* ctl = reinterpret_cast<SmemCtl*>(patch_base + p.kblocks * kPatchBytes);
+  SmemCtl* ctl = reinterpret_cast<SmemCtl*>(patch_base + patch_area_bytes(p.kblocks, p.ktail));
   PatchCtl* pc = reinterpret_cast<PatchCtl*>(ctl + 1);
 
   const int warp = threadIdx.x >> 5;
@@ -363,7 +385,9 @@
   pdl_trigger();
   if (warp == 0 && lane == 0) {
     tma_prefetch_desc(&p.tmA);
+    tma_prefetch_desc(&p.tmAt);
     tma_prefetch_desc(&p.tmB);
+    tma_prefetch_desc(&p.tmBt);
     tma_prefetch_desc(&p.tmD);
   }
   if (warp == 1 && lane == 0) {
@@ -395,15 +419,23 @@
           if (tap == 0) {
             mbar_wait(&pc->pempty[kb], pphase ^ 1);
             if (elect_one()) {
-              mbar_expect_tx(&pc->pfull[kb], kPatchBytes);
-              tma_load_4d(patch_base + kb * kPatchBytes, &p.tmA, &pc->pfull[kb], 0, x0 + p.offx, y0 + p.offy, kb * (KE / KG));
+              const bool tail = kb == p.kblocks - 1;
+              mbar_expect_tx(&pc->pfull[kb], tail ? patch_tail_bytes(p.ktail) : kPatchBytes);
+              tma_load_4d(patch_base + kb * kPatchBytes, tail ? &p.tmAt : &p.tmA, &pc->pfull[kb], 0, x0 + p.offx, y0 + p.offy,
+                          kb * (KE / KG));
             }
             __syncwarp();
           }
           mbar_wait(&ctl->empty[stage], phase ^ 1);
           if (elect_one()) {
-            mbar_expect_tx(&ctl->full[stage], b_bytes);
-            tma_load_2d(b_base + stage * b_stage_bytes, &p.tmB, &ctl->full[stage], kb * KE, tap * wk.n_total + wk.n_off);
+            uint8_t* sb = b_base + stage * b_stage_bytes;
+            if (kb == p.kblocks - 1 && p.ktail < 4) {
+              mbar_expect_tx(&ctl->full[stage], tail_b_bytes(p.ktail, p.n_mma));
+              tma_load_3d(sb, &p.tmBt, &ctl->full[stage], 0, tap * wk.n_total + wk.n_off, kb * (KE / KG));
+            } else {
+              mbar_expect_tx(&ctl->full[stage], b_bytes);
+              tma_load_2d(sb, &p.tmB, &ctl->full[stage], kb * KE, tap * wk.n_total + wk.n_off);
+            }
           }
           __syncwarp();
           if (++stage == p.stages) { stage = 0; phase ^= 1; }
@@ -417,6 +449,7 @@
       case 64: tc_conv_patch_consumer<BF16, 64>(p, ctl, pc, patch_base, b_base, b_stage_bytes, staging, wk); break;
       case 96: tc_conv_patch_consumer<BF16, 96>(p, ctl, pc, patch_base, b_base, b_stage_bytes, staging, wk); break;
       case 128: tc_conv_patch_consumer<BF16, 128>(p, ctl, pc, patch_base, b_base, b_stage_bytes, staging, wk); break;
+      case 136: tc_conv_patch_consumer<BF16, 136>(p, ctl, pc, patch_base, b_base, b_stage_bytes, staging, wk); break;
       case 144: tc_conv_patch_consumer<BF16, 144>(p, ctl, pc, patch_base, b_base, b_stage_bytes, staging, wk); break;
       default: tc_conv_patch_consumer<BF16, 160>(p, ctl, pc, patch_base, b_base, b_stage_bytes, staging, wk); break;
     }
@@ -770,7 +803,7 @@
   const size_t b_bytes = round1024((p.patch ? patch_nt(p.n_mma) : round32(p.n_mma)) * 128);
   if (p.patch)
     return 1024 + p.stages * b_bytes + static_cast<size_t>(p.n_chunks) * kChunkBytes +
-           static_cast<size_t>(p.kblocks) * kPatchBytes + sizeof(SmemCtl) + sizeof(PatchCtl);
+           static_cast<size_t>(patch_area_bytes(p.kblocks, p.ktail)) + sizeof(SmemCtl) + sizeof(PatchCtl);
   return 1024 + p.stages * (kABytes + b_bytes) + static_cast<size_t>(p.n_chunks) * kChunkBytes + sizeof(SmemCtl);
 }
 size_t tc_wgrad_smem_bytes(const TcWgradParams& p) {
@@ -795,7 +828,7 @@
 
 static bool conv_params_ok(const TcConvParams& p) {
   return p.n_mma >= 1 && p.n_mma <= 160 && p.n_chunks == (p.n_mma + 31) / 32 && p.stages >= 1 && p.stages <= 8 &&
-         p.kblocks >= 1 && p.nphase >= 0 && p.nphase <= 4 &&
+         p.kblocks >= 1 && p.ktail >= 1 && p.ktail <= 4 && p.nphase >= 0 && p.nphase <= 4 &&
          (p.bw & (p.bw - 1)) == 0 && p.bw * p.bh == kTileM &&
          (!p.patch || (((p.bw == 8 && p.bh == 16) || (p.bw == 16 && p.bh == 8)) && p.kblocks <= kPatchMaxKb && p.kh == 3 && p.kw == 3 && p.stride == 1 && p.nphase == 0));
 }
diff --git a/deep-image-prior_b200/csrc/conv_tc.cuh b/deep-image-prior_b200/csrc/conv_tc.cuh
--- a/deep-image-prior_b200/csrc/conv_tc.cuh
+++ b/deep-image-prior_b200/csrc/conv_tc.cuh
@@ -17,6 +17,7 @@
   int offx, offy;
   int bf16;
   int kblocks;
+  int ktail;
   int n_mma;
   int n_chunks;
   int stages;
@@ -28,10 +29,16 @@
   double* stats;
   int stats_ld;
   int patch;
+  CUtensorMap tmAt;
+  CUtensorMap tmBt;
 };
 static constexpr int kPatchPlane = 180 * 16;
 static constexpr int kPatchMaxKb = 8;
 static constexpr int kPatchBytes = 8 * kPatchPlane;
+__host__ __device__ constexpr int patch_tail_bytes(int ktail) { return 2 * ktail * kPatchPlane; }
+__host__ __device__ constexpr int patch_area_bytes(int kblocks, int ktail) {
+  return (kblocks - 1) * kPatchBytes + patch_tail_bytes(ktail);
+}
 
 static constexpr int kWgradKp = 32;
 struct TcWgradParams {
diff --git a/deep-image-prior_b200/csrc/engine.cu b/deep-image-prior_b200/csrc/engine.cu
--- a/deep-image-prior_b200/csrc/engine.cu
+++ b/deep-image-prior_b200/csrc/engine.cu
@@ -100,12 +100,13 @@
   cuuint32_t box[3] = {bf16 ? 64u : 32u, (cuuint32_t)bw, (cuuint32_t)bh};
   return encode_map(m, base, 3, dims, str, box, bf16);
 }
-static int map_patch(CUtensorMap* m, const void* base, int rows, int cols, int ld, int c, int bw, int bh, bool bf16) {
+static int map_patch(CUtensorMap* m, const void* base, int rows, int cols, int ld, int c, int bw, int bh, bool bf16,
+                     int groups = 8) {
   const cuuint64_t e = bf16 ? 2 : sizeof(float);
   const cuuint64_t g = 16 / e;
   cuuint64_t dims[4] = {g, (cuuint64_t)cols, (cuuint64_t)rows, (cuuint64_t)c / g};
   cuuint64_t str[3] = {ld * e, (cuuint64_t)cols * ld * e, 16};
-  cuuint32_t box[4] = {(cuuint32_t)g, (cuuint32_t)bw + 2, (cuuint32_t)bh + 2, 8};
+  cuuint32_t box[4] = {(cuuint32_t)g, (cuuint32_t)bw + 2, (cuuint32_t)bh + 2, (cuuint32_t)groups};
   return encode_map(m, base, 4, dims, str, box, bf16, false);
 }
 static int map_w2(CUtensorMap* m, const void* base, int rows_total, int kcols, int box_rows, bool bf16 = false) {
@@ -114,6 +115,15 @@
   cuuint64_t str[1] = {kcols * e};
   cuuint32_t box[2] = {bf16 ? 64u : 32u, (cuuint32_t)box_rows};
   return encode_map(m, base, 2, dims, str, box, bf16);
+}
+
+static int map_w_groups(CUtensorMap* m, const void* base, int rows_total, int kcols, int box_rows, int groups, bool bf16) {
+  const cuuint64_t e = bf16 ? 2 : sizeof(float);
+  const cuuint64_t g = 16 / e;
+  cuuint64_t dims[3] = {g, (cuuint64_t)rows_total, (cuuint64_t)kcols / g};
+  cuuint64_t str[2] = {kcols * e, 16};
+  cuuint32_t box[3] = {(cuuint32_t)g, (cuuint32_t)box_rows, (cuuint32_t)groups};
+  return encode_map(m, base, 3, dims, str, box, bf16, false);
 }
 
 static void pick_tile(int w, int h, int* bw, int* bh) {
@@ -224,6 +234,10 @@
   while (sp * 2 <= 4 && tiles * sp * 2 <= g_num_sms && n_rows % (32 * sp * 2) == 0) sp *= 2;
   return sp;
 }
+static int k_tail(int kc, int kblocks, bool bf16) {
+  const int ke = bf16 ? 64 : 32;
+  return (kc - ke * (kblocks - 1) + ke / 4 - 1) / (ke / 4);
+}
 static void fit_stages(TcConvParams& p) {
   p.stages = p.patch ? 8 : 6;
   while (tc_conv_smem_bytes(p) > 232448 && p.stages > 2) p.stages--;
@@ -261,7 +275,7 @@
   void set_shapes() {
     c_pad = round_up(C, 32);
     c_pad16 = round_up(C, 64);
-    crows = round_up(C, 16);
+    crows = C > 128 && C <= 136 ? 136 : round_up(C, 16);
     Np = round_up(N, 16); n_pad = round_up(N, 32); n_pad16 = round_up(N, 64);
     if (Ctot == 0) Ctot = C;
     if (dg_ld == 0) dg_ld = C;
@@ -298,6 +312,7 @@
     fit_stages(t);
     if (tc_conv_smem_bytes(t) > 232448) return 0;
     DIP_CHECK(map_patch(&t.tmA, act, rows, cols, ld, kc, g.bw, g.bh, bf16));
+    DIP_CHECK(map_patch(&t.tmAt, act, rows, cols, ld, kc, g.bw, g.bh, bf16, 2 * t.ktail));
     g = t;
     return 0;
   }
@@ -316,6 +331,8 @@
       fp.kh = fp.kw = k; fp.stride = stride; fp.offx = offx; fp.offy = offy;
       fp.bf16 = bf16 ? 1 : 0;
       fp.kblocks = bf16 ? c_pad16 / 64 : c_pad / 32;
+      fp.ktail = k_tail(C, fp.kblocks, bf16);
+      DIP_CHECK(map_w_groups(&fp.tmBt, wp_f, k * k * Np, bf16 ? c_pad16 : c_pad, Np / fp.n_split, 2 * fp.ktail, bf16));
       fp.n_mma = Np / fp.n_split; fp.n_chunks = (fp.n_mma + 31) / 32;
       fp.n_valid = N;
       fp.bias = nullptr; fp.stats = stats; fp.stats_ld = N;
@@ -351,6 +368,8 @@
       }
       dg.bf16 = bf16 ? 1 : 0;
       dg.kblocks = bf16 ? n_pad16 / 64 : n_pad / 32;
+      dg.ktail = k_tail(N, dg.kblocks, bf16);
+      DIP_CHECK(map_w_groups(&dg.tmBt, wp_d, k * k * crows, bf16 ? n_pad16 : n_pad, crows / dg.n_split, 2 * dg.ktail, bf16));
       dg.n_mma = crows / dg.n_split; dg.n_chunks = (dg.n_mma + 31) / 32;
       fit_stages(dg);
       if (!dg_s2 && k == 3)
diff --git a/deep-image-prior_b200/csrc/wgmma.cuh b/deep-image-prior_b200/csrc/wgmma.cuh
--- a/deep-image-prior_b200/csrc/wgmma.cuh
+++ b/deep-image-prior_b200/csrc/wgmma.cuh
@@ -25,6 +25,12 @@
   asm volatile("{\n\t.reg .pred p;\n\tsetp.ne.b32 p, %66, 0;\n\t"
                "wgmma.mma_async.sync.aligned.m64n128k8.f32.tf32.tf32 {%0, %1, %2, %3, %4, %5, %6, %7, %8, %9, %10, %11, %12, %13, %14, %15, %16, %17, %18, %19, %20, %21, %22, %23, %24, %25, %26, %27, %28, %29, %30, %31, %32, %33, %34, %35, %36, %37, %38, %39, %40, %41, %42, %43, %44, %45, %46, %47, %48, %49, %50, %51, %52, %53, %54, %55, %56, %57, %58, %59, %60, %61, %62, %63}, %64, %65, p, 1, 1;\n\t}\n"
                : "+f"(d[0]), "+f"(d[1]), "+f"(d[2]), "+f"(d[3]), "+f"(d[4]), "+f"(d[5]), "+f"(d[6]), "+f"(d[7]), "+f"(d[8]), "+f"(d[9]), "+f"(d[10]), "+f"(d[11]), "+f"(d[12]), "+f"(d[13]), "+f"(d[14]), "+f"(d[15]), "+f"(d[16]), "+f"(d[17]), "+f"(d[18]), "+f"(d[19]), "+f"(d[20]), "+f"(d[21]), "+f"(d[22]), "+f"(d[23]), "+f"(d[24]), "+f"(d[25]), "+f"(d[26]), "+f"(d[27]), "+f"(d[28]), "+f"(d[29]), "+f"(d[30]), "+f"(d[31]), "+f"(d[32]), "+f"(d[33]), "+f"(d[34]), "+f"(d[35]), "+f"(d[36]), "+f"(d[37]), "+f"(d[38]), "+f"(d[39]), "+f"(d[40]), "+f"(d[41]), "+f"(d[42]), "+f"(d[43]), "+f"(d[44]), "+f"(d[45]), "+f"(d[46]), "+f"(d[47]), "+f"(d[48]), "+f"(d[49]), "+f"(d[50]), "+f"(d[51]), "+f"(d[52]), "+f"(d[53]), "+f"(d[54]), "+f"(d[55]), "+f"(d[56]), "+f"(d[57]), "+f"(d[58]), "+f"(d[59]), "+f"(d[60]), "+f"(d[61]), "+f"(d[62]), "+f"(d[63])
+               : "l"(a), "l"(b), "r"(1) : "memory");
+}
+__device__ __forceinline__ void wgmma_tf32_n136(float (&d)[68], uint64_t a, uint64_t b) {
+  asm volatile("{\n\t.reg .pred p;\n\tsetp.ne.b32 p, %70, 0;\n\t"
+               "wgmma.mma_async.sync.aligned.m64n136k8.f32.tf32.tf32 {%0, %1, %2, %3, %4, %5, %6, %7, %8, %9, %10, %11, %12, %13, %14, %15, %16, %17, %18, %19, %20, %21, %22, %23, %24, %25, %26, %27, %28, %29, %30, %31, %32, %33, %34, %35, %36, %37, %38, %39, %40, %41, %42, %43, %44, %45, %46, %47, %48, %49, %50, %51, %52, %53, %54, %55, %56, %57, %58, %59, %60, %61, %62, %63, %64, %65, %66, %67}, %68, %69, p, 1, 1;\n\t}\n"
+               : "+f"(d[0]), "+f"(d[1]), "+f"(d[2]), "+f"(d[3]), "+f"(d[4]), "+f"(d[5]), "+f"(d[6]), "+f"(d[7]), "+f"(d[8]), "+f"(d[9]), "+f"(d[10]), "+f"(d[11]), "+f"(d[12]), "+f"(d[13]), "+f"(d[14]), "+f"(d[15]), "+f"(d[16]), "+f"(d[17]), "+f"(d[18]), "+f"(d[19]), "+f"(d[20]), "+f"(d[21]), "+f"(d[22]), "+f"(d[23]), "+f"(d[24]), "+f"(d[25]), "+f"(d[26]), "+f"(d[27]), "+f"(d[28]), "+f"(d[29]), "+f"(d[30]), "+f"(d[31]), "+f"(d[32]), "+f"(d[33]), "+f"(d[34]), "+f"(d[35]), "+f"(d[36]), "+f"(d[37]), "+f"(d[38]), "+f"(d[39]), "+f"(d[40]), "+f"(d[41]), "+f"(d[42]), "+f"(d[43]), "+f"(d[44]), "+f"(d[45]), "+f"(d[46]), "+f"(d[47]), "+f"(d[48]), "+f"(d[49]), "+f"(d[50]), "+f"(d[51]), "+f"(d[52]), "+f"(d[53]), "+f"(d[54]), "+f"(d[55]), "+f"(d[56]), "+f"(d[57]), "+f"(d[58]), "+f"(d[59]), "+f"(d[60]), "+f"(d[61]), "+f"(d[62]), "+f"(d[63]), "+f"(d[64]), "+f"(d[65]), "+f"(d[66]), "+f"(d[67])
                : "l"(a), "l"(b), "r"(1) : "memory");
 }
 __device__ __forceinline__ void wgmma_tf32_n144(float (&d)[72], uint64_t a, uint64_t b) {
@@ -121,7 +127,7 @@
 
 template <int N, bool BF16>
 __device__ __forceinline__ void wgmma_ss(float (&d)[N / 2], uint64_t a, uint64_t b) {
-  static_assert(N == 32 || N == 64 || N == 96 || N == 128 || (N == 136 && BF16) || N == 144 || N == 160, "wgmma N");
+  static_assert(N == 32 || N == 64 || N == 96 || N == 128 || N == 136 || N == 144 || N == 160, "wgmma N");
   if constexpr (BF16) {
     if constexpr (N == 32) wgmma_bf16_n32(d, a, b);
     else if constexpr (N == 64) wgmma_bf16_n64(d, a, b);
@@ -135,6 +141,7 @@
     else if constexpr (N == 64) wgmma_tf32_n64(d, a, b);
     else if constexpr (N == 96) wgmma_tf32_n96(d, a, b);
     else if constexpr (N == 128) wgmma_tf32_n128(d, a, b);
+    else if constexpr (N == 136) wgmma_tf32_n136(d, a, b);
     else if constexpr (N == 144) wgmma_tf32_n144(d, a, b);
     else wgmma_tf32_n160(d, a, b);
   }
```

Result: slower. 195.2, median of 6 (-4.1%).
